# icameling/lidar_camera_calibration

Hardware: AMD Instinct MI355X
Metric: chessboard-corner frames/sec + max corner error (mm), VLP-16 cloud (higher is better)
Workload: dtype f32

## Files before the change

### include/ilcc_hip.h

```cpp
#ifndef ILCC_HIP_H_
#define ILCC_HIP_H_

#include <stdint.h>

#ifdef __cplusplus
extern "C" {
#endif

#define ILCC_MAX_CORNERS 256
#define ILCC_ABI_VERSION 5

enum {
  ILCC_OK = 0,
  ILCC_NO_ROI_POINTS = 1,
  ILCC_NO_CLUSTER = 2,
  ILCC_NO_PLANE = 3,
  ILCC_DEGENERATE_HIST = 4,
  ILCC_TOO_FEW_POINTS = 5,
  ILCC_BAD_ARGUMENT = 6,
  ILCC_CAPACITY = 7,
  ILCC_HIP_ERROR = 8,
  ILCC_IO_ERROR = 9,
  ILCC_BOARD_NOT_FOUND = 10,
  ILCC_AMBIGUOUS = 11
// ... 89 lines not shown
  uint64_t grid_cost_box_evals_sum;
  double grid_cost_kernel_ms_sum;
  double grid_cost_full_ms_sum;
  double walk_order_ms_sum;
  double grid_cost_prepass_ms_sum;
  double grid_cost_locate_ms_sum;
  uint64_t batches;
  double stage_ms_sum[7];
  double roi_count_ms_sum;
  uint64_t online_second_tier_frames;
} ilcc_timing;

int32_t ilcc_abi_version(void);
const char* ilcc_strerror(int32_t status);
const char* ilcc_last_error(const ilcc_handle* h);

void ilcc_default_params(ilcc_params* p);

int32_t ilcc_set_chessboard_param(ilcc_params* p, const char* cam_yaml);

ilcc_handle* ilcc_create(int32_t device, const ilcc_params* p, uint32_t max_frames,
                         uint64_t max_total_points);
void ilcc_destroy(ilcc_handle* h);
int32_t ilcc_set_params(ilcc_handle* h, const ilcc_params* p);
int32_t ilcc_reserve(ilcc_handle* h, uint32_t labelled_points_per_frame, uint32_t roi_points_per_frame);

int32_t ilcc_extract(ilcc_handle* h, const float* xyzi, uint32_t n, const float click[3],
                     ilcc_result* out);

int32_t ilcc_extract_batch(ilcc_handle* h, const float* xyzi, const uint64_t* offsets,
                           uint32_t n_frames, const float* clicks, ilcc_result* out);

int32_t ilcc_extract_batch_device(ilcc_handle* h, const float* d_xyzi, const uint64_t* offsets,
                                  uint32_t n_frames, const float* d_clicks, ilcc_result* out);

int32_t ilcc_submit_batch_device(ilcc_handle* h, const float* d_xyzi, const uint64_t* offsets,
                                 uint32_t n_frames, const float* d_clicks, int32_t* ticket);
int32_t ilcc_submit_batch(ilcc_handle* h, const float* xyzi, const uint64_t* offsets, uint32_t n_frames,
                          const float* clicks, int32_t* ticket);
int32_t ilcc_wait(ilcc_handle* h, int32_t ticket, ilcc_result* out);
#define ILCC_RECORD_HEADER 20
int32_t ilcc_wait_records_device(ilcc_handle* h, int32_t ticket, ilcc_result* out, void* d_records, uint32_t n_corners,
                                 uint32_t tag_base);

enum { ILCC_RESULTS_FULL = 0, ILCC_RESULTS_COMPACT = 1 };
int32_t ilcc_set_result_mode(ilcc_handle* h, int32_t mode);
int32_t ilcc_wait_compact(ilcc_handle* h, int32_t ticket, float* records, uint64_t capacity_floats);
uint32_t ilcc_record_floats(const ilcc_handle* h, int32_t ticket);
int32_t ilcc_fetch_results(ilcc_handle* h, uint32_t first, uint32_t n, ilcc_result* out);

int32_t ilcc_chessboard_by_point_batch(ilcc_handle* h, const float* xyzi, const uint64_t* offsets,
                                       uint32_t n_frames, const float* points, int32_t min_plane_points,
                                       ilcc_result* out);
int32_t ilcc_submit_chessboard_by_point(ilcc_handle* h, const float* xyzi, const uint64_t* offsets, uint32_t n_frames,
                                        const float* points, int32_t* ticket);
int32_t ilcc_wait_chessboard_by_point(ilcc_handle* h, int32_t ticket, int32_t min_plane_points, ilcc_result* out);
int64_t ilcc_fetch_classes(ilcc_handle* h, uint32_t frame, uint8_t* out_class, uint64_t cap_points);

int64_t ilcc_fetch_cloud(ilcc_handle* h, uint32_t frame, int32_t which, float* out_xyzi,
                         uint64_t cap_points);
int64_t ilcc_fetch_labelled(ilcc_handle* h, uint32_t frame, float* out_yz, uint8_t* out_label,
                            uint64_t cap_points);
int64_t ilcc_fetch_walk(ilcc_handle* h, uint32_t frame, float* out_yz, uint8_t* out_label, uint64_t cap_points,
                        uint32_t counts[2]);

int32_t ilcc_grid_cost(ilcc_handle* h, const float* yz, const uint8_t* label, uint32_t m,
                       int32_t use_oob, float* cost_out, int32_t* best_index, float* best_cost);

int32_t ilcc_grid_solve(ilcc_handle* h, const float* yz, const uint8_t* label, uint32_t m, int32_t* grid_index, float* grid_cost,
                        int32_t lat[3], int32_t* phase, int64_t* cost_q, int64_t* alt_cost_q, int32_t* rounds, int32_t* hops,
                        int32_t* flags, int32_t* ties);

int32_t ilcc_pattern_refine(ilcc_handle* h, const float* yz, const uint8_t* label, uint32_t m, int32_t lat[3],
                            int32_t* phase, int64_t* cost_q, int64_t* alt_cost_q, int32_t* rounds, int32_t* hops);

int32_t ilcc_get_theta_t(ilcc_handle* h, const float* yz, const uint8_t* label, uint32_t m,
                         int32_t topleft_white, int32_t use_oob, double theta_t[3], double* cost,
                         int32_t* iterations);

#define ILCC_TIMELINE_COLS 15
int32_t ilcc_debug_timeline_enable(ilcc_handle* h, int32_t on);
int32_t ilcc_debug_timeline_fetch(ilcc_handle* h, double* rows, uint32_t cap_rows);

void ilcc_get_timing(const ilcc_handle* h, ilcc_timing* t);
void ilcc_reset_timing(ilcc_handle* h);

int32_t ilcc_save_corners2txt(const float* corners_xyz, uint32_t n_corners, const char* filename);
int32_t ilcc_read_lidar_corners(const char* filename, uint32_t num, double* out_xyz);

#ifdef __cplusplus
}
#endif
#endif
```

### lidar_camera_calibration_amd/_native.py

```python
from __future__ import annotations

import ctypes as C
import os

import numpy as np

_HERE = os.path.dirname(os.path.abspath(__file__))
LIB_PATH = os.environ.get("ILCC_HIP_LIB") or os.path.join(_HERE, "libilcc_hip.so")
MAX_CORNERS = 256

OK, NO_ROI_POINTS, NO_CLUSTER, NO_PLANE, DEGENERATE_HIST, TOO_FEW_POINTS, BAD_ARGUMENT, CAPACITY, \
    HIP_ERROR, IO_ERROR, BOARD_NOT_FOUND, AMBIGUOUS = range(12)
FLAG_TIE_OVERFLOW, FLAG_REFINE_CAPPED, FLAG_LOW_COVERAGE, FLAG_BORDER_RISK = 1, 2, 4, 8
FLAGS_FP32_ONLY = FLAG_TIE_OVERFLOW | FLAG_BORDER_RISK
RECORD_HEADER = 20
TIMELINE_COLS = 15
COST_Q_ONE = float(1 << 40)
SOLVER_REFERENCE_LOCAL, SOLVER_GRID = 0, 1
CLOUD_ROI, CLOUD_CLUSTER, CLOUD_CHESSBOARD, CLOUD_PCA, CLOUD_OPTIM = range(5)

EXPORTS = [
    "ilcc_abi_version", "ilcc_strerror", "ilcc_last_error", "ilcc_default_params",
    "ilcc_set_chessboard_param", "ilcc_create", "ilcc_destroy", "ilcc_set_params", "ilcc_reserve", "ilcc_extract",
    "ilcc_extract_batch", "ilcc_extract_batch_device", "ilcc_submit_batch_device", "ilcc_submit_batch", "ilcc_wait", "ilcc_wait_records_device", "ilcc_fetch_cloud", "ilcc_fetch_labelled", "ilcc_fetch_walk", "ilcc_chessboard_by_point_batch", "ilcc_submit_chessboard_by_point", "ilcc_wait_chessboard_by_point", "ilcc_fetch_classes",
    "ilcc_grid_cost", "ilcc_grid_solve", "ilcc_pattern_refine", "ilcc_get_theta_t", "ilcc_get_timing", "ilcc_reset_timing",
    "ilcc_save_corners2txt", "ilcc_read_lidar_corners",
    "ilcc_set_result_mode", "ilcc_wait_compact", "ilcc_record_floats", "ilcc_fetch_results",
    "ilcc_debug_timeline_enable", "ilcc_debug_timeline_fetch",
]
ABI_VERSION = 5
RESULTS_FULL, RESULTS_COMPACT = 0, 1


class Params(C.Structure):
    _fields_ = [
        ("roi_half", C.c_double * 3),
        ("cluster_tol", C.c_double),
        ("cluster_min", C.c_int32),
        ("cluster_max", C.c_int32),
        ("ransac_thresh", C.c_double),
        ("ransac_hyp", C.c_int32),
        ("ransac_seed", C.c_uint32),
        ("hist_bins", C.c_int32),
        ("gray_rate", C.c_double),
        ("huber_delta", C.c_double),
        ("grid_length", C.c_double),
        ("board_w", C.c_int32),
        ("board_h", C.c_int32),
        ("solver", C.c_int32),
        ("phase_mode", C.c_int32),
        ("max_iterations", C.c_int32),
        ("grid_prune", C.c_int32),
        ("n_th", C.c_int32), ("n_ty", C.c_int32), ("n_tz", C.c_int32),
        ("th_min", C.c_double), ("th_step", C.c_double),
        ("ty_min", C.c_double), ("ty_step", C.c_double),
        ("tz_min", C.c_double), ("tz_step", C.c_double),
        ("refine_div", C.c_int32), ("refine_max_rounds", C.c_int32),
        ("refine_th_margin", C.c_int32), ("reserved0", C.c_int32),
        ("ambiguity_eps", C.c_double),
        ("online_cluster_tol", C.c_double),
        ("min_cell_coverage", C.c_double),
        ("ransac_probability", C.c_double),
    ]


class Result(C.Structure):
    _fields_ = [
        ("status", C.c_int32),
        ("n_points", C.c_int32),
        ("n_roi", C.c_int32), ("n_cluster", C.c_int32), ("n_plane", C.c_int32),
        ("n_black", C.c_int32), ("n_gray", C.c_int32), ("n_white", C.c_int32),
        ("n_corners", C.c_int32),
        ("phase", C.c_int32),
        ("iters_a", C.c_int32), ("iters_b", C.c_int32),
        ("grid_index", C.c_int32),
        ("found_board", C.c_int32),
        ("grid_cost", C.c_float),
        ("plane", C.c_float * 4),
        ("pca", C.c_float * 16),
        ("gray_zone", C.c_double * 2),
        ("theta_t", C.c_double * 3),
        ("cost_a", C.c_double), ("cost_b", C.c_double),
        ("sel_cost", C.c_double),
        ("basin_margin", C.c_double),
        ("flags", C.c_int32),
        ("grid_ties", C.c_int32),
        ("cells_hit", C.c_int32),
        ("n_oob", C.c_int32),
        ("corners", C.c_float * (MAX_CORNERS * 3)),
    ]

    def corners_array(self) -> np.ndarray:
        return np.ctypeslib.as_array(self.corners)[:3 * self.n_corners].reshape(-1, 3).copy()


class Timing(C.Structure):
    _fields_ = [
        ("roi_crop", C.c_float), ("cluster", C.c_float), ("ransac_plane", C.c_float),
        ("plane_frame_hist", C.c_float), ("grid_cost", C.c_float), ("refine_corners", C.c_float),
        ("total", C.c_float),
        ("grid_cost_launches", C.c_uint32),
        ("grid_cost_ms_sum", C.c_double),
        ("grid_cost_evals_sum", C.c_uint64),
        ("grid_cost_evals_nominal_sum", C.c_uint64),
        ("grid_cost_evals_interior_sum", C.c_uint64),
        ("grid_cost_box_evals_sum", C.c_uint64),
        ("grid_cost_kernel_ms_sum", C.c_double),
        ("grid_cost_full_ms_sum", C.c_double),
        ("walk_order_ms_sum", C.c_double),
        ("grid_cost_prepass_ms_sum", C.c_double),
        ("grid_cost_locate_ms_sum", C.c_double),
# ... 13 lines not shown
        if not os.path.exists(LIB_PATH):
            raise OSError(f"{LIB_PATH} not found: build it with `python -c 'import __graft_entry__ as g; "
                          "g.build()'` (hipcc --offload-arch=gfx950); there is no CPU fallback")
        L = C.CDLL(LIB_PATH)
        vp, fp = C.c_void_p, C.POINTER(C.c_float)
        pp, rp = C.POINTER(Params), C.POINTER(Result)
        L.ilcc_abi_version.restype = C.c_int32
        got = L.ilcc_abi_version()
        if got != ABI_VERSION:
            raise OSError(f"{LIB_PATH} implements ABI {got}, this package declares ABI {ABI_VERSION}: rebuild it "
                          "(python -c 'import __graft_entry__ as g; g.build()')")
        L.ilcc_strerror.argtypes = [C.c_int32]
        L.ilcc_strerror.restype = C.c_char_p
        L.ilcc_last_error.argtypes = [vp]
        L.ilcc_last_error.restype = C.c_char_p
        L.ilcc_default_params.argtypes = [pp]
        L.ilcc_set_chessboard_param.argtypes = [pp, C.c_char_p]
        L.ilcc_set_chessboard_param.restype = C.c_int32
        L.ilcc_create.argtypes = [C.c_int32, pp, C.c_uint32, C.c_uint64]
        L.ilcc_create.restype = vp
        L.ilcc_destroy.argtypes = [vp]
        L.ilcc_set_params.argtypes = [vp, pp]
        L.ilcc_set_params.restype = C.c_int32
        L.ilcc_reserve.argtypes = [vp, C.c_uint32, C.c_uint32]
        L.ilcc_reserve.restype = C.c_int32
        L.ilcc_extract.argtypes = [vp, fp, C.c_uint32, fp, rp]
        L.ilcc_extract.restype = C.c_int32
        L.ilcc_extract_batch.argtypes = [vp, fp, C.POINTER(C.c_uint64), C.c_uint32, fp, rp]
        L.ilcc_extract_batch.restype = C.c_int32
        L.ilcc_extract_batch_device.argtypes = [vp, vp, C.POINTER(C.c_uint64), C.c_uint32, vp, rp]
        L.ilcc_extract_batch_device.restype = C.c_int32
        L.ilcc_submit_batch_device.argtypes = [vp, vp, C.POINTER(C.c_uint64), C.c_uint32, vp, C.POINTER(C.c_int32)]
        L.ilcc_submit_batch_device.restype = C.c_int32
        L.ilcc_submit_batch.argtypes = [vp, vp, C.POINTER(C.c_uint64), C.c_uint32, vp, C.POINTER(C.c_int32)]
        L.ilcc_submit_batch.restype = C.c_int32
        L.ilcc_wait.argtypes = [vp, C.c_int32, rp]
        L.ilcc_wait.restype = C.c_int32
        L.ilcc_wait_records_device.argtypes = [vp, C.c_int32, rp, vp, C.c_uint32, C.c_uint32]
        L.ilcc_wait_records_device.restype = C.c_int32
        L.ilcc_chessboard_by_point_batch.argtypes = [vp, fp, C.POINTER(C.c_uint64), C.c_uint32, fp, C.c_int32, rp]
        L.ilcc_chessboard_by_point_batch.restype = C.c_int32
        L.ilcc_submit_chessboard_by_point.argtypes = [vp, C.c_void_p, C.POINTER(C.c_uint64), C.c_uint32, C.c_void_p, C.POINTER(C.c_int32)]
        L.ilcc_submit_chessboard_by_point.restype = C.c_int32
        L.ilcc_wait_chessboard_by_point.argtypes = [vp, C.c_int32, C.c_int32, rp]
        L.ilcc_wait_chessboard_by_point.restype = C.c_int32
        L.ilcc_fetch_classes.argtypes = [vp, C.c_uint32, C.POINTER(C.c_uint8), C.c_uint64]
        L.ilcc_fetch_classes.restype = C.c_int64
        L.ilcc_fetch_cloud.argtypes = [vp, C.c_uint32, C.c_int32, fp, C.c_uint64]
        L.ilcc_fetch_cloud.restype = C.c_int64
        L.ilcc_fetch_labelled.argtypes = [vp, C.c_uint32, fp, C.POINTER(C.c_uint8), C.c_uint64]
        L.ilcc_fetch_labelled.restype = C.c_int64
        L.ilcc_fetch_walk.argtypes = [vp, C.c_uint32, fp, C.POINTER(C.c_uint8), C.c_uint64, C.POINTER(C.c_uint32)]
        L.ilcc_fetch_walk.restype = C.c_int64
        L.ilcc_grid_cost.argtypes = [vp, fp, C.POINTER(C.c_uint8), C.c_uint32, C.c_int32, fp,
                                     C.POINTER(C.c_int32), fp]
        L.ilcc_grid_cost.restype = C.c_int32
        L.ilcc_grid_solve.argtypes = [vp, fp, C.POINTER(C.c_uint8), C.c_uint32, C.POINTER(C.c_int32), fp, C.POINTER(C.c_int32),
                                      C.POINTER(C.c_int32), C.POINTER(C.c_int64), C.POINTER(C.c_int64), C.POINTER(C.c_int32),
                                      C.POINTER(C.c_int32), C.POINTER(C.c_int32), C.POINTER(C.c_int32)]
        L.ilcc_grid_solve.restype = C.c_int32
        L.ilcc_pattern_refine.argtypes = [vp, fp, C.POINTER(C.c_uint8), C.c_uint32, C.POINTER(C.c_int32),
                                          C.POINTER(C.c_int32), C.POINTER(C.c_int64), C.POINTER(C.c_int64),
                                          C.POINTER(C.c_int32), C.POINTER(C.c_int32)]
        L.ilcc_pattern_refine.restype = C.c_int32
        L.ilcc_get_theta_t.argtypes = [vp, fp, C.POINTER(C.c_uint8), C.c_uint32, C.c_int32, C.c_int32,
                                       C.POINTER(C.c_double), C.POINTER(C.c_double), C.POINTER(C.c_int32)]
        L.ilcc_get_theta_t.restype = C.c_int32
        L.ilcc_get_timing.argtypes = [vp, C.POINTER(Timing)]
        L.ilcc_reset_timing.argtypes = [vp]
        L.ilcc_save_corners2txt.argtypes = [fp, C.c_uint32, C.c_char_p]
        L.ilcc_save_corners2txt.restype = C.c_int32
        L.ilcc_read_lidar_corners.argtypes = [C.c_char_p, C.c_uint32, C.POINTER(C.c_double)]
        L.ilcc_read_lidar_corners.restype = C.c_int32
        L.ilcc_set_result_mode.argtypes = [vp, C.c_int32]
        L.ilcc_set_result_mode.restype = C.c_int32
        L.ilcc_wait_compact.argtypes = [vp, C.c_int32, fp, C.c_uint64]
        L.ilcc_wait_compact.restype = C.c_int32
        L.ilcc_record_floats.argtypes = [vp, C.c_int32]
        L.ilcc_record_floats.restype = C.c_uint32
        L.ilcc_debug_timeline_enable.argtypes = [vp, C.c_int32]
        L.ilcc_debug_timeline_enable.restype = C.c_int32
        L.ilcc_debug_timeline_fetch.argtypes = [vp, C.POINTER(C.c_double), C.c_uint32]
        L.ilcc_debug_timeline_fetch.restype = C.c_int32
        L.ilcc_fetch_results.argtypes = [vp, C.c_uint32, C.c_uint32, rp]
        L.ilcc_fetch_results.restype = C.c_int32
        _lib = L
    return _lib


def default_params() -> Params:
    p = Params()
    lib().ilcc_default_params(C.byref(p))
    return p


def strerror(status: int) -> str:
    return lib().ilcc_strerror(int(status)).decode()


def fptr(a: np.ndarray):
    return a.ctypes.data_as(C.POINTER(C.c_float))
```

### lidar_camera_calibration_amd/csrc/ilcc_api.cpp

```cpp
#include <hip/hip_runtime.h>

#include <cmath>
#include <cstdio>
#include <cstdlib>
#include <cstring>
#include <fstream>
#include <mutex>
#include <new>
#include <sstream>
#include <string>
#include <vector>

#include "ilcc_internal.h"

using namespace ilcc;

#ifndef ILCC_SLOTS
#define ILCC_SLOTS 4
#endif
constexpr int kSlots = ILCC_SLOTS;
constexpr int kStreams = 3;

enum BatchEvent {
  kEvStart,
// ... 13 lines not shown
  kEvCount
};
static_assert(kEvCount == ILCC_TIMELINE_COLS - 1, "a timeline row is the slot and one time per event");

struct Slot {
  hipEvent_t ev[kEvCount]{};
  hipEvent_t done = nullptr;
  hipEvent_t late = nullptr;
  hipEvent_t k6_done = nullptr;
  bool allocated = false;
  float4* d_xyzi = nullptr;
  float* d_clicks = nullptr;
  uint64_t* d_off = nullptr;
  ilcc_result* d_res = nullptr;
  float4 *d_roi = nullptr, *d_cluster = nullptr, *d_board = nullptr, *d_pca = nullptr, *d_optim = nullptr;
  float2 *d_yz = nullptr, *d_walk_yz = nullptr;
  uint8_t* d_walk_lab = nullptr;
  uint32_t *d_walk_mi = nullptr, *d_walk_nrim = nullptr;
  uint8_t *d_lab = nullptr, *d_cls = nullptr;
  uint32_t *d_nlab = nullptr, *d_walk = nullptr, *d_counts = nullptr, *d_parent = nullptr, *d_count = nullptr;
  unsigned long long* d_masks = nullptr;
  uint32_t *d_hash_head = nullptr, *d_hash_next = nullptr;
  uint32_t *d_flags = nullptr, *d_nfinite = nullptr, *d_counts_fin = nullptr;
  uint32_t* h_online = nullptr;
  uint32_t* d_list = nullptr;
  void* d_list_frames = nullptr;
  GridPartial *d_partial = nullptr, *d_partial2 = nullptr, *d_partial3 = nullptr, *d_partial4 = nullptr;
  SolveRec* d_solverec = nullptr;
  uint32_t *d_bound = nullptr, *d_bound_sub = nullptr;
  uint32_t* d_tie_count = nullptr;
  GridPartial* d_tie_list = nullptr;
  unsigned long long* d_iters = nullptr;
  uint32_t *d_grp_alive = nullptr, *d_grp_mask = nullptr;
  size_t grp_alive_cap = 0, grp_mask_cap = 0;
  float* h_rec_dev = nullptr;
  unsigned long long* h_iters_dev = nullptr;
  float* h_rec = nullptr;
  ilcc_result* h_res = nullptr;
  unsigned long long* h_iters = nullptr;
  uint64_t* h_off = nullptr;
  std::vector<uint64_t> off;
  uint32_t n_frames = 0;
  bool busy = false, grid = false;
  bool online = false;
  bool h_res_valid = false;
  bool compact = false;
  uint32_t rec_corners = 0;
};

struct ilcc_handle {
  int device = 0;
  ilcc_params p{};
  uint32_t max_frames = 0;
  uint64_t max_points = 0;
  uint32_t max_theta = 0;
  uint32_t crop_chunks_cap = 0;
  Slot slots[kSlots];
  hipStream_t stream[kStreams]{};
  uint64_t seq = 0;
  uint64_t stream_last[kStreams]{};
  hipEvent_t entry_done = nullptr;
  int next_slot = 0;
  int last_slot = -1;
  int k6_last = -1;
  float *d_cth = nullptr, *d_sth = nullptr, *d_ay = nullptr, *d_az = nullptr;
  float *d_cth2 = nullptr, *d_sth2 = nullptr, *d_ay2 = nullptr, *d_az2 = nullptr;
  GridTables grid{}, seed_grid{};
  SeedMap seed_map{2, 12, 6};
  double2* d_th_lattice = nullptr;
  size_t th_lattice_cap = 0;
  int32_t th_lat_lo = 0, th_lat_hi = 0, hop_y = 0, hop_z = 0;
  double* d_solve = nullptr;
  RefineOut* d_refine_io = nullptr;
  uint32_t grid_lds_points = 1024;
  uint64_t group_prepass_skipped = 0;
  uint32_t cluster_lds_points = 2048;
  uint32_t cluster_cells_cap = kClusterCellsMin;
  uint32_t list_grid = 1024;
  bool poisoned = false;
  int32_t result_mode = ILCC_RESULTS_FULL;
  ilcc_timing timing{};
  hipEvent_t tl_ref = nullptr;
  bool tl_on = false;
  std::vector<double> tl_rows;
  std::string err;
};

namespace {

thread_local std::string g_err;

#define HIP_TRY(h, expr)                                                                   \
  do {                                                                                     \
    hipError_t e_ = (expr);                                                                \
    if (e_ != hipSuccess) {                                                                \
      (h)->err = std::string(#expr) + ": " + hipGetErrorString(e_);                        \
      return ILCC_HIP_ERROR;                                                               \
    }                                                                                      \
  } while (0)

int32_t near_zero_index(double vmin, double step, int32_t n) {
  long c = std::lround(-vmin / step);
  if (c < 0) c = 0;
  if (c > n - 1) c = n - 1;
  return (int32_t)c;
}

bool params_ok(const ilcc_params& p, std::string& why) {
  auto bad = [&](const char* m) {
    why = m;
    return false;
  };
  if (!(p.grid_length > 0)) return bad("grid_length must be > 0");
  if (p.board_w < 2 || p.board_h < 2 || p.board_w > p.board_h) return bad("board_w/board_h: need 2 <= w <= h");
  if ((p.board_w - 1) * (p.board_h - 1) > ILCC_MAX_CORNERS) return bad("too many corners");
  if (p.hist_bins < 1 || p.hist_bins > 4096) return bad("hist_bins out of range");
  if (!(p.gray_rate > 0) || !(p.huber_delta > 0)) return bad("gray_rate / huber_delta must be > 0");
  if (p.ransac_hyp < 1 || p.ransac_hyp > 65536) return bad("ransac_hyp out of range");
  if (!(p.ransac_probability == p.ransac_probability) || p.ransac_probability >= 1.0) return bad("ransac_probability must be < 1");
  if (!(p.cluster_tol > 0) || p.cluster_min < 1 || p.cluster_max < p.cluster_min) return bad("cluster params");
  if (p.solver != ILCC_SOLVER_REFERENCE_LOCAL && p.solver != ILCC_SOLVER_GRID) return bad("solver");
  if (p.phase_mode < 0 || p.phase_mode > 2) return bad("phase_mode");
  if (p.grid_prune != 0 && p.grid_prune != 1) return bad("grid_prune must be 0 or 1");
  if (p.max_iterations < 0 || p.max_iterations > 100000) return bad("max_iterations");
  if (p.n_th < 1 || p.n_ty < 1 || p.n_tz < 1) return bad("grid sizes must be >= 1");
  if (p.n_th > 4096 || p.n_ty > 4096 || p.n_tz > 4096) return bad("grid axes are limited to 4096 candidates");
  if (p.n_ty + p.n_tz > kGridTableMax) return bad("n_ty + n_tz exceeds the LDS table capacity of the grid kernel");
  if (p.refine_div < 0 || p.refine_div > 64 || (p.refine_div & (p.refine_div - 1)) != 0)
    return bad("refine_div must be 0 or a power of two <= 64");
  if (p.refine_max_rounds < 0 || p.refine_max_rounds > 4096) return bad("refine_max_rounds");
  if (p.refine_th_margin < 0 || p.refine_th_margin > 4096) return bad("refine_th_margin");
  if (!(p.online_cluster_tol > 0)) return bad("online_cluster_tol must be > 0");
  if (!(p.ambiguity_eps == p.ambiguity_eps)) return bad("ambiguity_eps is NaN");
  if (!(p.min_cell_coverage == p.min_cell_coverage) || p.min_cell_coverage > 1.0) return bad("min_cell_coverage must be <= 1");
  if (p.board_w * p.board_h > kCoverageCellsMax) return bad("board has more squares than the coverage mask holds");
  if ((uint64_t)p.n_th * p.n_ty * p.n_tz * 2ull >= 0xFFFFFFFFull) return bad("grid too large");
  if (!(p.th_step > 0) || !(p.ty_step > 0) || !(p.tz_step > 0)) return bad("grid steps must be > 0");
  {
    const double div = (double)(p.refine_div > 0 ? p.refine_div : 1);
    if (std::lround(p.grid_length / (p.ty_step / div)) < 1 || std::lround(p.grid_length / (p.tz_step / div)) < 1)
      return bad("ty_step / tz_step too coarse: one board square is less than half a refinement-lattice step");
  }
  return true;
}

int32_t sync_own(ilcc_handle* h, hipStream_t s) {
  HIP_TRY(h, hipEventRecord(h->entry_done, s));
  HIP_TRY(h, hipEventSynchronize(h->entry_done));
  return ILCC_OK;
}

int32_t sync_all(ilcc_handle* h) {
  for (hipStream_t s : h->stream)
    if (s) HIP_TRY(h, hipStreamSynchronize(s));
  return ILCC_OK;
}

int32_t upload_tables(ilcc_handle* h) {
  const ilcc_params& p = h->p;
  if ((uint32_t)p.n_th > h->max_theta || (uint32_t)p.n_ty > h->max_theta || (uint32_t)p.n_tz > h->max_theta) {
    h->err = "grid axis longer than the handle's table capacity";
    return ILCC_CAPACITY;
  }
  hipStream_t st = h->stream[0];
  std::vector<float> cth(p.n_th), sth(p.n_th), ay(p.n_ty), az(p.n_tz);
  const double g = p.grid_length;
// ... 339 lines not shown
#endif
#ifndef ILCC_BOX_POINTS
#define ILCC_BOX_POINTS 48
#endif
constexpr int kAnchorRadius = 1;
#ifndef ILCC_ANCHOR_ROUNDS
#define ILCC_ANCHOR_ROUNDS 2
#endif
constexpr int kAnchorRounds = ILCC_ANCHOR_ROUNDS;


GridPass whole_grid_pass(const Ctx& c, const GridTables& t, GridPartial* out) {
  GridPass g{};
  g.t = t;
  g.out = out;
  g.blocks = (uint32_t)t.n_th;
  g.bound = c.grid_bound;
  return g;
}

GridSeed full_table_records(const GridPartial* records, uint32_t blocks) { return GridSeed{records, blocks, SeedMap{1, 1, 0}}; }

GridPass seed_pass(const ilcc_handle* h, const Slot& sl, const Ctx& c) {
  GridPass g = whole_grid_pass(c, h->seed_grid, sl.d_partial2);
  g.walk_limit = (uint32_t)ILCC_SEED_POINTS;
  g.bound = c.grid_bound_sub;
  return g;
}

GridPass refine_pass(const ilcc_handle* h, const Slot& sl, const Ctx& c, int32_t refine_radius) {
  GridPass g = whole_grid_pass(c, h->grid, sl.d_partial3);
  g.seed = GridSeed{sl.d_partial2, (uint32_t)h->seed_grid.n_th, h->seed_map};
  g.window_tiles = h->seed_map.stride_t > 2 * kTileA ? 4 : 2;
  g.radius_th = (refine_radius / kRefineThetaStride) * kRefineThetaStride;
  g.step_th = kRefineThetaStride;
  g.blocks = std::min((uint32_t)(2 * (g.radius_th / kRefineThetaStride) + 1), h->max_theta);
  g.walk_limit = (uint32_t)ILCC_SEED_POINTS;
  g.bound = c.grid_bound_sub;
  return g;
}

GridPass anchor_pass(const ilcc_handle* h, const Ctx& c, const GridSeed& seed, GridPartial* out) {
  GridPass g = whole_grid_pass(c, h->grid, out);
  g.seed = seed;
  g.radius_th = kAnchorRadius;
  g.blocks = 2 * kAnchorRadius + 1;
  return g;
}

GridPass full_pass(const ilcc_handle* h, const Ctx& c, const GridSeed& seed) {
  GridPass g = whole_grid_pass(c, h->grid, c.partial);
  g.seed = seed;
  g.collect_ties = 1u;
  return g;
}

LocatePlan locate_plan(const ilcc_handle* h, const Slot& sl, const Ctx& c) {
  LocatePlan lp{};
  lp.seed = h->seed_grid;
  lp.map = h->seed_map;
  lp.refine_radius = std::max(1, h->seed_map.stride_th / ILCC_REFINE_RADIUS_DIV);
  lp.sample_min = (uint32_t)ILCC_SEED_POINTS;
  lp.sample_cap = std::max((uint32_t)ILCC_SEED_POINTS, ((c.grid_lds_points >> 3) + 63u) & ~63u);
  lp.out = sl.d_partial4;
  return lp;
}

int32_t enqueue_locate_launches(ilcc_handle* h, Slot& sl, const Ctx& c, hipStream_t s, int32_t refine_radius, GridSeed& located) {
  launch_grid_cost(c, seed_pass(h, sl, c), s, 1, nullptr, true);
  HIP_TRY(h, hipEventRecord(sl.ev[kEvSeeded], s));
  const GridPass refine = refine_pass(h, sl, c, refine_radius);
  launch_grid_cost(c, refine, s, 1, nullptr, true);
  HIP_TRY(h, hipEventRecord(sl.ev[kEvRefined], s));
  located = full_table_records(refine.out, refine.blocks);
  GridPartial* const ping[2] = {sl.d_partial4, sl.d_partial2};
  for (int round = 0; round < kAnchorRounds; ++round) {
    const GridPass anchor = anchor_pass(h, c, located, ping[round & 1]);
    launch_anchor(c, anchor, s);
    located = full_table_records(anchor.out, anchor.blocks);
  }
  return ILCC_OK;
}

int32_t enqueue_grid_search(ilcc_handle* h, Slot& sl, const Ctx& c, hipStream_t s, uint32_t n_frames, bool chain) {
  const bool prune = h->p.grid_prune != 0;
  launch_walk_order(c, s);
  HIP_TRY(h, hipEventRecord(sl.ev[kEvWalkOrdered], s));
  GridSeed located{};
  if (h->seed_grid.n_th > 0 && h->p.n_th >= 8 && h->p.n_ty >= 8 && h->p.n_tz >= 8) {
    const LocatePlan lp = locate_plan(h, sl, c);
    const bool fused = n_frames >= (uint32_t)kLocateMinFrames && lp.seed.n_th <= 16 &&
                       locate_lds_bytes(lp.sample_cap, h->grid.n_ty, h->grid.n_tz, lp.seed.n_ty, lp.seed.n_tz) <= 60u * 1024u;
    if (fused) {
      launch_locate(c, s, lp);
      HIP_TRY(h, hipEventRecord(sl.ev[kEvSeeded], s));
      HIP_TRY(h, hipEventRecord(sl.ev[kEvRefined], s));
      located = full_table_records(lp.out, 1);
    } else {
      const int32_t st = enqueue_locate_launches(h, sl, c, s, lp.refine_radius, located);
      if (st != ILCC_OK) return st;
    }
  } else {
    HIP_TRY(h, hipEventRecord(sl.ev[kEvSeeded], s));
    HIP_TRY(h, hipEventRecord(sl.ev[kEvRefined], s));
  }
  HIP_TRY(h, hipEventRecord(sl.ev[kEvAnchored], s));
  GridPass full = full_pass(h, c, located);
  const GroupPrepassPlan gp = group_prepass_plan(h->p);
  full.box_points = gp.box ? (uint32_t)ILCC_BOX_POINTS : 0u;
  if (full.box_points != 0u && gp.on && (size_t)n_frames * gp.groups <= sl.grp_alive_cap &&
      (size_t)n_frames * gp.groups * gp.words <= sl.grp_mask_cap) {
    full.grp_alive = sl.d_grp_alive;
    full.grp_mask = sl.d_grp_mask;
    full.grp_count = gp.groups;
    full.grp_words = gp.words;
    launch_group_prepass(c, full, s);
  } else if (full.box_points != 0u && gp.on) {
    if (h->group_prepass_skipped++ == 0) h->err = "note: k6_group_prepass skipped (mask buffers smaller than this batch needs): slower, results unaffected";
  }
  HIP_TRY(h, hipEventRecord(sl.ev[kEvPrepassed], s));
  const int si = (int)(&sl - h->slots);
  if (chain && h->k6_last >= 0 && h->k6_last != si && h->slots[h->k6_last].busy)
    HIP_TRY(h, hipStreamWaitEvent(s, h->slots[h->k6_last].k6_done, 0));
  HIP_TRY(h, hipEventRecord(sl.ev[kEvFullStart], s));
  launch_grid_cost(c, full, s, 1, nullptr, prune);
  if (chain) {
    HIP_TRY(h, hipEventRecord(sl.k6_done, s));
    h->k6_last = si;
  }
  return ILCC_OK;
}

int32_t enqueue_impl(ilcc_handle* h, int si, hipStream_t s, const float4* d_xyzi, const uint64_t* offsets, uint32_t n_frames,
                     const float* d_clicks, bool front_only, bool no_crop) {
  Slot& sl = h->slots[si];
  uint64_t max_n = 0;
  for (uint32_t f = 0; f < n_frames; ++f) max_n = std::max<uint64_t>(max_n, offsets[f + 1] - offsets[f]);
  uint32_t chunks = (uint32_t)((max_n + kCropChunk - 1) / kCropChunk);
  if (chunks == 0) chunks = 1;
  if ((uint64_t)chunks * n_frames > (uint64_t)h->crop_chunks_cap) {
    h->err = "crop chunk table too small for this (very ragged) batch";
    return ILCC_CAPACITY;
  }
  sl.off.assign(offsets, offsets + n_frames + 1);
  sl.n_frames = n_frames;
  std::memcpy(sl.h_off, sl.off.data(), sizeof(uint64_t) * (n_frames + 1));
  HIP_TRY(h, hipMemcpyAsync(sl.d_off, sl.h_off, sizeof(uint64_t) * (n_frames + 1), hipMemcpyHostToDevice, s));
  Ctx c = make_ctx(h, sl, d_xyzi, d_clicks, n_frames, chunks);
  HIP_TRY(h, hipEventRecord(sl.ev[kEvStart], s));
  if (!no_crop) {
    launch_roi_crop(c, s, sl.ev[kEvCropCounted]);
    HIP_TRY(h, hipEventRecord(sl.ev[kEvCropped], s));
    launch_cluster(c, s);
  } else {
    c.p.cluster_tol = c.p.online_cluster_tol;
    c.wide = 1u;
    Ctx t1 = c;
    t1.online_tier = 1u;
    t1.online_window = 1.25f;
    t1.p.roi_half[0] = t1.p.roi_half[1] = t1.p.roi_half[2] = (double)t1.online_window;
    t1.cluster_bits = cluster_bits_online();
    launch_roi_crop(t1, s, sl.ev[kEvCropCounted]);
    HIP_TRY(h, hipEventRecord(sl.ev[kEvCropped], s));
    launch_cluster(t1, s);
    Ctx t2 = c;
    t2.online_tier = 2u;
    t2.p.roi_half[0] = t2.p.roi_half[1] = t2.p.roi_half[2] = (double)INFINITY;
    launch_roi_crop(t2, s, nullptr);
    launch_cluster(t2, s);
    HIP_TRY(h, hipMemcpyAsync(sl.h_online, sl.d_flags, sizeof(uint32_t) * n_frames, hipMemcpyDeviceToHost, s));
    HIP_TRY(h, hipMemcpyAsync(sl.h_online + h->max_frames, sl.d_nfinite, sizeof(uint32_t) * n_frames, hipMemcpyDeviceToHost, s));
  }
  HIP_TRY(h, hipEventRecord(sl.ev[kEvClustered], s));
  launch_ransac_plane(c, s);
  HIP_TRY(h, hipEventRecord(sl.ev[kEvPlane], s));
  launch_plane_frame_hist(c, s);
  sl.grid = !front_only && h->p.solver == ILCC_SOLVER_GRID;
  HIP_TRY(h, hipEventRecord(sl.ev[kEvLabelled], s));
  if (sl.grid) {
    const int32_t st = enqueue_grid_search(h, sl, c, s, n_frames, true);
    if (st != ILCC_OK) return st;
  }
  HIP_TRY(h, hipEventRecord(sl.ev[kEvSearched], s));
  if (!front_only) {
    if (sl.grid) {
      launch_pattern_refine_corners(c, s);
    } else {
      launch_refine_corners(c, s);
    }
  }
  HIP_TRY(h, hipEventRecord(sl.ev[kEvEnd], s));
  HIP_TRY(h, hipGetLastError());
  sl.compact = h->result_mode == ILCC_RESULTS_COMPACT;
  sl.rec_corners = board_corners(h->p);
  if (sl.compact) {
    launch_pack_records(sl.d_res, n_frames, sl.rec_corners, 0u, sl.h_rec_dev, s);
  } else {
    HIP_TRY(h, copy_results_trimmed(sl.h_res, sl.d_res, n_frames, sl.rec_corners, s));
  }
  launch_store_to_host(sl.d_iters, sl.h_iters_dev, sizeof(unsigned long long) * kBatchWords, s);
  HIP_TRY(h, hipGetLastError());
  HIP_TRY(h, hipEventRecord(sl.done, s));
  sl.busy = true;
  sl.online = no_crop;
  return ILCC_OK;
}

int32_t run_late(ilcc_handle* h, Slot& sl, hipStream_t s) {
  HIP_TRY(h, hipEventRecord(sl.late, s));
  HIP_TRY(h, hipEventSynchronize(sl.late));
  return ILCC_OK;
}

int32_t ensure_full(ilcc_handle* h, Slot& sl) {
  if (sl.h_res_valid) return ILCC_OK;
  const hipStream_t s = late_stream(h);
  HIP_TRY(h, copy_results_trimmed(sl.h_res, sl.d_res, sl.n_frames, sl.rec_corners, s));
  const int32_t st = run_late(h, sl, s);
  if (st != ILCC_OK) return st;
  sl.h_res_valid = true;
  return ILCC_OK;
}

int32_t finish(ilcc_handle* h, int si, ilcc_result* out, float* out_compact = nullptr, float* d_records = nullptr,
               uint32_t n_corners = 0, uint32_t tag_base = 0) {
  Slot& sl = h->slots[si];
  HIP_TRY(h, hipEventSynchronize(sl.done));
  const uint32_t n_frames = sl.n_frames;
  const size_t rec_w = (size_t)ILCC_RECORD_HEADER + 3 * (size_t)sl.rec_corners;
  const bool pack_now = out_compact && !sl.compact;
  const hipStream_t ls = late_stream(h);
  if (d_records) launch_pack_records(sl.d_res, n_frames, n_corners, tag_base, d_records, ls);
  if (pack_now) launch_pack_records(sl.d_res, n_frames, sl.rec_corners, 0u, sl.h_rec_dev, ls);
  if (d_records || pack_now) {
    const int32_t st = run_late(h, sl, ls);
    if (st != ILCC_OK) return st;
  }
  sl.busy = false;
  sl.h_res_valid = !sl.compact;
  h->last_slot = si;
  if (out) {
    const int32_t st = ensure_full(h, sl);
    if (st != ILCC_OK) return st;
    const size_t row = trimmed_bytes(sl.rec_corners);
    for (uint32_t f = 0; f < n_frames; ++f) std::memcpy(&out[f], &sl.h_res[f], row);
  }
  if (out_compact) std::memcpy(out_compact, sl.h_rec, sizeof(float) * n_frames * rec_w);
  auto span = [&](BatchEvent from, BatchEvent to, float& ms_out) { return hipEventElapsedTime(&ms_out, sl.ev[from], sl.ev[to]); };
  float ms[6];
  HIP_TRY(h, span(kEvStart, kEvCropped, ms[0]));
  HIP_TRY(h, span(kEvCropped, kEvClustered, ms[1]));
  HIP_TRY(h, span(kEvClustered, kEvPlane, ms[2]));
  HIP_TRY(h, span(kEvPlane, kEvLabelled, ms[3]));
  HIP_TRY(h, span(kEvLabelled, kEvSearched, ms[4]));
  HIP_TRY(h, span(kEvSearched, kEvEnd, ms[5]));
  float k6k[6] = {0.f, 0.f, 0.f, 0.f, 0.f, 0.f};
  if (sl.grid) {
    float pre = 0.f;
    HIP_TRY(h, span(kEvLabelled, kEvPrepassed, pre));
    HIP_TRY(h, span(kEvLabelled, kEvWalkOrdered, k6k[0]));
    HIP_TRY(h, span(kEvWalkOrdered, kEvSeeded, k6k[1]));
    HIP_TRY(h, span(kEvSeeded, kEvRefined, k6k[2]));
    HIP_TRY(h, span(kEvRefined, kEvAnchored, k6k[3]));
// ... 767 lines not shown
  if (cost_q) *cost_q = (int64_t)std::llround(rec.sel * 1099511627776.0);
  if (alt_cost_q) *alt_cost_q = (int64_t)std::llround(rec.cost_b * 1099511627776.0);
  if (rounds) *rounds = rec.iters_a;
  if (hops) *hops = rec.iters_b;
  if (flags) *flags = rec.flags;
  if (ties) *ties = rec.ties;
  return ILCC_OK;
}

int32_t ilcc_get_theta_t(ilcc_handle* h, const float* yz, const uint8_t* label, uint32_t m, int32_t topleft_white,
                         int32_t use_oob, double theta_t[3], double* cost, int32_t* iterations) {
  if (!h || !theta_t) return ILCC_BAD_ARGUMENT;
  const hipStream_t s = h->stream[take_stream(h)];
  int32_t st = stage_labelled(h, s, yz, label, m);
  if (st != ILCC_OK) return st;
  Slot& sl = h->slots[0];
  HIP_TRY(h, hipMemcpyAsync(h->d_solve, theta_t, sizeof(double) * 3, hipMemcpyHostToDevice, s));
  const Ctx c = make_ctx(h, sl, nullptr, nullptr, 1, 1);
  launch_local_solve(c, s, topleft_white, use_oob, h->d_solve, h->d_solve + 3);
  HIP_TRY(h, hipGetLastError());
  double back[5];
  HIP_TRY(h, hipMemcpyAsync(back, h->d_solve, sizeof(back), hipMemcpyDeviceToHost, s));
  {
    const int32_t sst = sync_own(h, s);
    if (sst != ILCC_OK) return sst;
  }
  theta_t[0] = back[0];
  theta_t[1] = back[1];
  theta_t[2] = back[2];
  if (cost) *cost = back[3];
  if (iterations) *iterations = (int32_t)back[4];
  return ILCC_OK;
}

int32_t ilcc_pattern_refine(ilcc_handle* h, const float* yz, const uint8_t* label, uint32_t m, int32_t lat[3],
                            int32_t* phase, int64_t* cost_q, int64_t* alt_cost_q, int32_t* rounds, int32_t* hops) {
  if (!h || !lat || !phase) return ILCC_BAD_ARGUMENT;
  if (lat[0] < h->th_lat_lo || lat[0] > h->th_lat_hi || (*phase != 0 && *phase != 1)) {
    h->err = "ilcc_pattern_refine: theta lattice coordinate outside [th_min - refine_th_margin, th_max + refine_th_margin] steps";
    return ILCC_BAD_ARGUMENT;
  }
  const hipStream_t s = h->stream[take_stream(h)];
  int32_t st = stage_labelled(h, s, yz, label, m);
  if (st != ILCC_OK) return st;
  Slot& sl = h->slots[0];
  RefineOut io{};
  io.lat[0] = lat[0];
  io.lat[1] = lat[1];
  io.lat[2] = lat[2];
  io.phase = *phase;
  HIP_TRY(h, hipMemcpyAsync(h->d_refine_io, &io, sizeof(io), hipMemcpyHostToDevice, s));
  const Ctx c = make_ctx(h, sl, nullptr, nullptr, 1, 1);
  launch_pattern_refine_test(c, s, h->d_refine_io);
  HIP_TRY(h, hipGetLastError());
  HIP_TRY(h, hipMemcpyAsync(&io, h->d_refine_io, sizeof(io), hipMemcpyDeviceToHost, s));
  {
    const int32_t sst = sync_own(h, s);
    if (sst != ILCC_OK) return sst;
  }
  lat[0] = io.lat[0];
  lat[1] = io.lat[1];
  lat[2] = io.lat[2];
  *phase = io.phase;
  if (cost_q) *cost_q = io.cost_q;
  if (alt_cost_q) *alt_cost_q = io.alt_q;
  if (rounds) *rounds = io.rounds;
  if (hops) *hops = io.hops;
  return ILCC_OK;
}

int32_t ilcc_debug_timeline_enable(ilcc_handle* h, int32_t on) {
  if (!h) return ILCC_BAD_ARGUMENT;
  HIP_TRY(h, hipSetDevice(h->device));
  h->tl_rows.clear();
  h->tl_on = on != 0;
  if (h->tl_on) {
    if (!h->tl_ref) HIP_TRY(h, hipEventCreate(&h->tl_ref));
    HIP_TRY(h, hipEventRecord(h->tl_ref, h->stream[0]));
    HIP_TRY(h, hipEventSynchronize(h->tl_ref));
  }
  return ILCC_OK;
}

int32_t ilcc_debug_timeline_fetch(ilcc_handle* h, double* rows, uint32_t cap_rows) {
  if (!h || (!rows && cap_rows)) return -ILCC_BAD_ARGUMENT;
  const size_t have = h->tl_rows.size() / ILCC_TIMELINE_COLS;
  const size_t n = std::min<size_t>(have, cap_rows);
  if (n) std::memcpy(rows, h->tl_rows.data(), sizeof(double) * n * ILCC_TIMELINE_COLS);
  h->tl_rows.clear();
  return (int32_t)n;
}

void ilcc_get_timing(const ilcc_handle* h, ilcc_timing* t) {
  if (h && t) *t = h->timing;
}
void ilcc_reset_timing(ilcc_handle* h) {
  if (h) h->timing = ilcc_timing{};
}

int32_t ilcc_save_corners2txt(const float* corners_xyz, uint32_t n_corners, const char* filename) {
  if (!corners_xyz || !filename) return ILCC_BAD_ARGUMENT;
  std::ofstream outfile(filename, std::ios_base::trunc);
  if (!outfile.is_open()) return ILCC_IO_ERROR;
  for (uint32_t i = 0; i < n_corners; ++i)
    outfile << corners_xyz[3 * i] << " " << corners_xyz[3 * i + 1] << " " << corners_xyz[3 * i + 2] << std::endl;
  outfile.close();
  return outfile.fail() ? ILCC_IO_ERROR : ILCC_OK;
}

int32_t ilcc_read_lidar_corners(const char* filename, uint32_t num, double* out_xyz) {
  if (!filename || !out_xyz) return -ILCC_BAD_ARGUMENT;
  std::ifstream infile(filename);
  if (!infile.is_open()) return -ILCC_IO_ERROR;
  uint32_t counter = 0;
  while (!infile.eof() && counter < num) {
    float x = 0, y = 0, z = 0;
    infile >> x >> y >> z;
    if (infile.fail()) break;
    out_xyz[3 * counter] = x;
    out_xyz[3 * counter + 1] = y;
    out_xyz[3 * counter + 2] = z;
    ++counter;
  }
  return (int32_t)counter;
}

}
```

### lidar_camera_calibration_amd/csrc/ilcc_internal.h

```cpp
#pragma once

#include <hip/hip_runtime.h>
#include <stdint.h>

#include "ilcc_hip.h"

#define ILCC_WAVE 64

namespace ilcc {

constexpr int kCropThreads = 256;
constexpr int kCropChunk = 4096;
#ifndef ILCC_K2_THREADS
#define ILCC_K2_THREADS 256
#endif
constexpr int kFrameThreads = ILCC_K2_THREADS;
#ifndef ILCC_K3_THREADS
#define ILCC_K3_THREADS 256
#endif
#ifndef ILCC_K45_THREADS
#define ILCC_K45_THREADS 256
#endif
constexpr int kPlaneThreads = ILCC_K3_THREADS;
constexpr int kPlaneThreadsSmallBatch = 1024;
#ifndef ILCC_SMALL_BATCH
#define ILCC_SMALL_BATCH 64
#endif
constexpr int kSmallBatchFrames = ILCC_SMALL_BATCH;
constexpr int kHistThreads = ILCC_K45_THREADS;
#ifndef ILCC_K6_THREADS
#define ILCC_K6_THREADS 256
#endif
constexpr int kGridThreads = ILCC_K6_THREADS;
#ifndef ILCC_K6_THREADS_LARGE
#define ILCC_K6_THREADS_LARGE 512
#endif
constexpr int kGridThreadsLarge = ILCC_K6_THREADS_LARGE;
#ifndef ILCC_K6_LARGE_FROM
#define ILCC_K6_LARGE_FROM 2048
#endif
constexpr int kGridLargeFrom = ILCC_K6_LARGE_FROM;
constexpr int kTileA = 4;
#ifndef ILCC_TILE_B
#define ILCC_TILE_B 4
#endif
constexpr int kTileB = ILCC_TILE_B;
#ifndef ILCC_K6_GROUP
#define ILCC_K6_GROUP 7
#endif
constexpr int kThetaGroup = ILCC_K6_GROUP;
constexpr int kGridLdsPointsMax = 8192;
constexpr int kGridTableMax = 8192;
#ifndef ILCC_K7_THREADS
#define ILCC_K7_THREADS 256
#endif
constexpr int kSolveThreads = ILCC_K7_THREADS;
#ifndef ILCC_K7R_THREADS
#define ILCC_K7R_THREADS 192
#endif
constexpr int kRefineThreads = ILCC_K7R_THREADS;
constexpr int kRefineThreadsSmallBatch = 768;
constexpr int kRefineList = 32;
constexpr int kTieCap = 256;
constexpr float kTieEps = 2e-5f;
constexpr int kCoverageCellsMax = 1024;
constexpr int kIterSlots = 64;
constexpr int kBatchWords = 3 * kIterSlots + 2;
constexpr int kClusterHashSize = 1 << 17;
constexpr int kClusterLdsPointsMax = 4096;
constexpr int kClusterLdsPointsMin = 1024;
constexpr int kClusterCellsMin = 512;
constexpr int kClusterCellsMax = 6144;

struct GridPartial {
  float cost;
  uint32_t d2;
  uint32_t flat;
  uint32_t pad;
};

struct SolveRec {
  double x[3];
  double cost_a, cost_b, sel;
  double margin;
  int32_t iters_a, iters_b, phase, valid;
  int32_t flags, ties;
};

struct RefineOut {
  long long cost_q, alt_q;
  int32_t lat[3];
  int32_t phase, rounds, hops;
};

struct GridTables {
  const float* cth;
  const float* sth;
  const float* ay;
  const float* az;
  int32_t n_th, n_ty, n_tz;
  int32_t c_th, c_ty, c_tz;
};

struct SeedMap {
  int32_t stride_t, stride_th, off_th;
};

struct GridSeed {
  const GridPartial* records;
  uint32_t blocks;
  SeedMap map;
};
// ... 80 lines not shown
    }
    if (a == 1u) break;
  }
  return S >= M ? 1u : S;
}

__device__ __forceinline__ int lane_id() { return threadIdx.x & (ILCC_WAVE - 1); }
__device__ __forceinline__ int wave_id() { return threadIdx.x >> 6; }

template <typename T>
__device__ __forceinline__ T wave_sum(T v) {
#pragma unroll
  for (int o = ILCC_WAVE / 2; o > 0; o >>= 1) v += __shfl_down(v, o, ILCC_WAVE);
  return v;
}

template <typename T>
__device__ __forceinline__ T block_sum(T v, T* scratch) {
  v = wave_sum(v);
  const int nw = (blockDim.x + ILCC_WAVE - 1) / ILCC_WAVE;
  __syncthreads();
  if (lane_id() == 0) scratch[wave_id()] = v;
  __syncthreads();
  if (threadIdx.x == 0) {
    T s = scratch[0];
    for (int w = 1; w < nw; ++w) s += scratch[w];
    scratch[16] = s;
  }
  __syncthreads();
  return scratch[16];
}

template <int NV>
__device__ __forceinline__ void block_sum_n(double (&v)[NV], double* scratch ) {
#pragma unroll
  for (int k = 0; k < NV; ++k) v[k] = wave_sum(v[k]);
  const int kW = (blockDim.x + ILCC_WAVE - 1) / ILCC_WAVE;
  __syncthreads();
  if (lane_id() == 0) {
#pragma unroll
    for (int k = 0; k < NV; ++k) scratch[wave_id() * NV + k] = v[k];
  }
  __syncthreads();
#pragma unroll
  for (int k = 0; k < NV; ++k) {
    double t = scratch[k];
    for (int w = 1; w < kW; ++w) t += scratch[w * NV + k];
    v[k] = t;
  }
}

__device__ __forceinline__ uint32_t block_rank(bool flag, uint32_t* scratch, uint32_t& total) {
  const unsigned long long m = __ballot(flag);
  const int lane = lane_id();
  const uint32_t in_wave = __popcll(m & ((1ull << lane) - 1ull));
  const int nw = (blockDim.x + ILCC_WAVE - 1) / ILCC_WAVE;
  __syncthreads();
  if (lane == 0) scratch[wave_id()] = __popcll(m);
  __syncthreads();
  uint32_t base = 0, tot = 0;
  for (int w = 0; w < nw; ++w) {
    const uint32_t c = scratch[w];
    if (w < wave_id()) base += c;
    tot += c;
  }
  total = tot;
  return base + in_wave;
}

struct LocatePlan {
  GridTables seed;
  SeedMap map;
  int32_t refine_radius;
  uint32_t sample_min, sample_cap;
  GridPartial* out;
};

size_t locate_lds_bytes(uint32_t sample_cap, int n_ty, int n_tz, int n_ty2, int n_tz2);
void launch_locate(const Ctx& c, hipStream_t s, const LocatePlan& lp);
void launch_anchor(const Ctx& c, const GridPass& pass, hipStream_t s);
constexpr int kRefineThetaStride = 2;
constexpr int kLocateMinFrames = 512;

void launch_roi_crop(const Ctx& c, hipStream_t s, hipEvent_t after_count = nullptr);
void launch_cluster(const Ctx& c, hipStream_t s);
void launch_ransac_plane(const Ctx& c, hipStream_t s);
void launch_plane_frame_hist(const Ctx& c, hipStream_t s);
void launch_walk_order(const Ctx& c, hipStream_t s);
void launch_grid_cost(const Ctx& c, const GridPass& pass, hipStream_t s, int32_t use_oob, float* cost_volume , bool prune);
void launch_group_prepass(const Ctx& c, const GridPass& full, hipStream_t s);
uint32_t grid_cost_evals_per_count();
void launch_refine_corners(const Ctx& c, hipStream_t s);
void launch_pack_records(const ilcc_result* d_res, uint32_t n_frames, uint32_t n_corners, uint32_t tag_base, float* d_out,
                         hipStream_t s);
void launch_store_to_host(const void* d_src, void* h_dst, size_t bytes, hipStream_t s);
void launch_pattern_refine_corners(const Ctx& c, hipStream_t s);
void launch_pattern_refine_test(const Ctx& c, hipStream_t s, RefineOut* d_io);
hipError_t set_kernel_attributes_k2();
size_t cluster_lds_bytes(uint32_t pts_cap, uint32_t cells_cap, uint32_t bits);
uint32_t cluster_bits_default();
uint32_t cluster_bits_online();
hipError_t set_kernel_attributes_k6();
hipError_t set_kernel_attributes_k7();
void launch_local_solve(const Ctx& c, hipStream_t s, int32_t tlw, int32_t use_oob, double* theta_t,
                        double* cost_iters );

}
```

### lidar_camera_calibration_amd/csrc/k1_roi_crop.hip

```cpp
#include "ilcc_internal.h"

namespace ilcc {

typedef float f32x4 __attribute__((ext_vector_type(4)));

struct Box {
  float lo[3], hi[3];
};

__device__ __forceinline__ Box make_box(const Ctx& c, uint32_t f) {
  Box b;
#pragma unroll
  for (int a = 0; a < 3; ++a) {
    const double cl = (double)c.clicks[3 * f + a];
    b.lo[a] = (float)(cl - c.p.roi_half[a]);
    b.hi[a] = (float)(cl + c.p.roi_half[a]);
  }
  return b;
}

template <bool FINITE_BOX>
__device__ __forceinline__ bool keep_point(const float4 q, const Box& b) {
  if (FINITE_BOX)
    return q.z >= b.lo[2] && q.z <= b.hi[2] && q.x >= b.lo[0] && q.x <= b.hi[0] && q.y >= b.lo[1] && q.y <= b.hi[1];
  const bool fin = isfinite(q.x) && isfinite(q.y) && isfinite(q.z);
  const bool in = !(q.z < b.lo[2] || q.z > b.hi[2]) && !(q.x < b.lo[0] || q.x > b.hi[0]) &&
                  !(q.y < b.lo[1] || q.y > b.hi[1]);
  return fin && in;
}

__global__ __launch_bounds__(kCropThreads) void k1_roi_count(Ctx c) {
  const uint32_t f = blockIdx.y, s = blockIdx.x;
  if (c.online_tier == 2u && c.frame_flags[f] == 0u) return;
  const uint64_t beg = c.off[f], end = c.off[f + 1];
  const uint64_t n = end - beg;
  if (s == 0) {
    uint32_t* w = reinterpret_cast<uint32_t*>(&c.res[f]);
    for (uint32_t k = threadIdx.x; k < sizeof(ilcc_result) / 4; k += kCropThreads) w[k] = 0u;
    if (f == 0 && threadIdx.x < kBatchWords && c.online_tier != 2u) c.grid_iters[threadIdx.x] = 0ull;
    __syncthreads();
  }
  if (s == 0 && threadIdx.x == 0) {
    if (c.tie_count) c.tie_count[f] = 0u;
    ilcc_result* r = &c.res[f];
    r->status = ILCC_OK;
    r->n_points = (int32_t)n;
    r->n_roi = r->n_cluster = r->n_plane = 0;
    r->n_black = r->n_gray = r->n_white = 0;
    r->n_corners = 0;
    r->phase = 0;
    r->iters_a = r->iters_b = 0;
    r->grid_index = -1;
    r->cells_hit = r->n_oob = 0;
    r->grid_cost = 0.f;
    r->cost_a = r->cost_b = r->sel_cost = 0.0;
    r->theta_t[0] = r->theta_t[1] = r->theta_t[2] = 0.0;
    c.n_lab[f] = 0;
    c.grid_bound[f] = 0x7f800000u;
    c.grid_bound_sub[f] = 0x7f800000u;
    if (c.online_tier == 1u) c.frame_flags[f] = 0u;
  }
  const uint64_t cbeg = (uint64_t)s * kCropChunk;
  uint32_t cnt = 0, fin = 0;
  unsigned long long* masks = c.crop_masks + ((uint64_t)f * c.crop_chunks + s) * (kCropChunk / ILCC_WAVE);
  if (cbeg < n) {
    const Box b = make_box(c, f);
    const uint64_t cend = (cbeg + kCropChunk < n) ? cbeg + kCropChunk : n;
    const float4* __restrict__ src = c.xyzi + beg;
    constexpr int kTrips = kCropChunk / kCropThreads;
    float4 q[kTrips];
#pragma unroll
    for (int k = 0; k < kTrips; ++k) {
      const uint64_t i = cbeg + (uint64_t)k * kCropThreads + threadIdx.x;
      if (i < cend) {
        const f32x4 v = __builtin_nontemporal_load(reinterpret_cast<const f32x4*>(src + i));
        q[k] = make_float4(v.x, v.y, v.z, v.w);
      } else {
        q[k] = make_float4(0.f, 0.f, 0.f, 0.f);
      }
    }
    const bool finite_box = isfinite(b.lo[0]) && isfinite(b.hi[0]) && isfinite(b.lo[1]) && isfinite(b.hi[1]) && isfinite(b.lo[2]) && isfinite(b.hi[2]);
    const uint32_t left = (uint32_t)(cend - cbeg);
    if (finite_box && c.online_tier != 1u) {
#pragma unroll
      for (int k = 0; k < kTrips; ++k) {
        const bool keep = ((uint32_t)k * kCropThreads + threadIdx.x < left) && keep_point<true>(q[k], b);
        const unsigned long long m = __ballot(keep);
        if (lane_id() == 0) masks[k * (kCropThreads / ILCC_WAVE) + wave_id()] = m;
        cnt += keep ? 1u : 0u;
      }
    } else {
#pragma unroll
      for (int k = 0; k < kTrips; ++k) {
        const bool mine = (uint32_t)k * kCropThreads + threadIdx.x < left;
        const bool keep = mine && keep_point<false>(q[k], b);
        const unsigned long long m = __ballot(keep);
        if (lane_id() == 0) masks[k * (kCropThreads / ILCC_WAVE) + wave_id()] = m;
        cnt += keep ? 1u : 0u;
        fin += (mine && isfinite(q[k].x) && isfinite(q[k].y) && isfinite(q[k].z)) ? 1u : 0u;
      }
    }
  }
  __shared__ uint32_t sc[17];
  const uint32_t total = block_sum<uint32_t>(cnt, sc);
  if (threadIdx.x == 0) c.crop_counts[(uint64_t)f * c.crop_chunks + s] = total;
  if (c.online_tier == 1u) {
    const uint32_t total_fin = block_sum<uint32_t>(fin, sc);
    if (threadIdx.x == 0) c.crop_fin[(uint64_t)f * c.crop_chunks + s] = total_fin;
  }
}

__global__ __launch_bounds__(kCropThreads) void k1_roi_scatter(Ctx c) {
  const uint32_t f = blockIdx.y, s = blockIdx.x;
  if (c.online_tier == 2u && c.frame_flags[f] == 0u) return;
  const uint64_t beg = c.off[f], end = c.off[f + 1];
  const uint64_t n = end - beg;
  const uint32_t* counts = c.crop_counts + (uint64_t)f * c.crop_chunks;
  uint32_t base = 0, all = 0;
  for (uint32_t k = 0; k < c.crop_chunks; ++k) {
    const uint32_t v = counts[k];
    if (k < s) base += v;
    all += v;
  }
  if (s == 0 && threadIdx.x == 0 && c.online_tier == 1u) {
    uint32_t nf = 0;
    for (uint32_t k = 0; k < c.crop_chunks; ++k) nf += c.crop_fin[(uint64_t)f * c.crop_chunks + k];
    c.n_finite[f] = nf;
  }
  if (s == 0 && threadIdx.x == 0) {
    c.res[f].n_roi = (int32_t)all;
    if (all == 0) {
      if (c.online_tier == 1u)
        c.frame_flags[f] = 1u;
      else
        c.res[f].status = ILCC_NO_ROI_POINTS;
    }
  }
  const uint64_t cbeg = (uint64_t)s * kCropChunk;
  if (cbeg >= n || counts[s] == 0) return;
  const float4* __restrict__ src = c.xyzi + beg;
  float4* __restrict__ dst = c.roi + beg;
  const unsigned long long* masks = c.crop_masks + ((uint64_t)f * c.crop_chunks + s) * (kCropChunk / ILCC_WAVE);
  constexpr int kWaves = kCropThreads / ILCC_WAVE, kMasks = kCropChunk / ILCC_WAVE;
  static_assert(kMasks == ILCC_WAVE, "one keep-mask per lane of the first wavefront");
  const int lane = lane_id(), w = wave_id();
  __shared__ unsigned long long s_mask[kMasks];
  __shared__ uint32_t s_before[kMasks];
  if (w == 0) {
    const unsigned long long mk = masks[lane];
    uint32_t incl = (uint32_t)__popcll(mk);
    const uint32_t own = incl;
#pragma unroll
    for (int o = 1; o < ILCC_WAVE; o <<= 1) {
      const uint32_t t = __shfl_up(incl, o, ILCC_WAVE);
      if (lane >= o) incl += t;
    }
    s_mask[lane] = mk;
    s_before[lane] = base + incl - own;
  }
  __syncthreads();
#pragma unroll
  for (int k = 0; k < kCropChunk / kCropThreads; ++k) {
    const int mine = k * kWaves + w;
    const unsigned long long mk = s_mask[mine];
    if ((mk >> lane) & 1ull) {
      const uint64_t i = cbeg + (uint64_t)k * kCropThreads + threadIdx.x;
      dst[s_before[mine] + (uint32_t)__popcll(mk & ((1ull << lane) - 1ull))] = src[i];
    }
  }
}

void launch_roi_crop(const Ctx& c, hipStream_t s, hipEvent_t after_count) {
  const dim3 grid(c.crop_chunks, c.n_frames);
  hipLaunchKernelGGL(k1_roi_count, grid, dim3(kCropThreads), 0, s, c);
  if (after_count) (void)hipEventRecord(after_count, s);
  hipLaunchKernelGGL(k1_roi_scatter, grid, dim3(kCropThreads), 0, s, c);
}

}
```

### lidar_camera_calibration_amd/csrc/k3_ransac_plane.hip

```cpp
#include "eig3.h"
#include "ilcc_internal.h"

namespace ilcc {

__device__ __forceinline__ uint32_t hash_u32(uint32_t x) {
  x ^= x >> 16;
  x *= 0x7feb352dU;
  x ^= x >> 15;
  x *= 0x846ca68bU;
  x ^= x >> 16;
  return x;
}
__device__ __forceinline__ uint32_t sample_index(uint32_t seed, uint32_t h, uint32_t k, uint32_t m) {
  const uint32_t r = hash_u32(seed ^ hash_u32(h * 3u + k + 0x9E3779B9u));
  return (uint32_t)(((uint64_t)r * (uint64_t)m) >> 32);
}

__device__ __forceinline__ bool plane_from_3(const float4 p0, const float4 p1, const float4 p2,
                                             float pl[4]) {
  const float ax = p1.x - p0.x, ay = p1.y - p0.y, az = p1.z - p0.z;
  const float bx = p2.x - p0.x, by = p2.y - p0.y, bz = p2.z - p0.z;
  float nx = ay * bz - az * by;
  float ny = az * bx - ax * bz;
  float nz = ax * by - ay * bx;
  float n2 = nx * nx;
  n2 = n2 + ny * ny;
  n2 = n2 + nz * nz;
  if (!(n2 > 1e-12f)) return false;
  const float nrm = sqrtf(n2);
  nx = nx / nrm;
  ny = ny / nrm;
  nz = nz / nrm;
  float d = nx * p0.x;
  d = d + ny * p0.y;
  d = d + nz * p0.z;
  pl[0] = nx;
  pl[1] = ny;
  pl[2] = nz;
  pl[3] = -d;
  return true;
}

__device__ __forceinline__ float plane_dist(const float pl[4], const float4 q) {
  float s = pl[0] * q.x;
  s = s + pl[1] * q.y;
  s = s + pl[2] * q.z;
  s = s + pl[3];
  return fabsf(s);
}

constexpr int kRansacLdsPoints = 2048;

__global__ __launch_bounds__(kPlaneThreadsSmallBatch) void k3_ransac_plane(Ctx c) {
  const uint32_t kThreads = blockDim.x;
  __shared__ float4 s_P[kRansacLdsPoints];
  __shared__ uint32_t sc[64];
  __shared__ double scd[16 * 6 + 8];
  __shared__ float s_plane[4];
  const uint32_t f = blockIdx.x;
  ilcc_result* r = &c.res[f];
  if (r->status != ILCC_OK) return;
  const uint32_t M = (uint32_t)r->n_cluster;
  const uint64_t beg = c.off[f];
  const float4* __restrict__ G = c.cluster + beg;
  const uint32_t tid = threadIdx.x;
  const int lane = lane_id(), wid = wave_id();
  const float thr = (float)c.p.ransac_thresh;
  if (M < 3) {
    if (tid == 0) r->status = ILCC_NO_PLANE;
    return;
  }
  const float4* P = G;
  if (M <= (uint32_t)kRansacLdsPoints) {
    for (uint32_t i = tid; i < M; i += kThreads) s_P[i] = G[i];
    __syncthreads();
    P = s_P;
  }

  const uint32_t n_waves = kThreads / ILCC_WAVE;
  auto score = [&](uint32_t h, uint32_t beat, uint32_t& cnt) -> bool {
    const uint32_t i0 = sample_index(c.p.ransac_seed, h, 0, M);
    const uint32_t i1 = sample_index(c.p.ransac_seed, h, 1, M);
    const uint32_t i2 = sample_index(c.p.ransac_seed, h, 2, M);
    float pl[4];
    cnt = 0;
    if (i0 == i1 || i0 == i2 || i1 == i2) return false;
    if (!plane_from_3(P[i0], P[i1], P[i2], pl)) return false;
    for (uint32_t base = 0; base < M; base += ILCC_WAVE) {
      const uint32_t i = base + lane;
      const bool in = (i < M) && plane_dist(pl, P[i]) < thr;
      cnt += (uint32_t)__popcll(__ballot(in));
      if (cnt + (M - min(M, base + (uint32_t)ILCC_WAVE)) <= beat) break;
    }
    return true;
  };
  if (c.p.ransac_probability > 0.0) {
    __shared__ uint32_t s_state[5];
    __shared__ double s_k;
    if (tid == 0) {
      s_state[0] = 0u;
      s_state[1] = 0xFFFFFFFFu;
      s_state[2] = s_state[3] = s_state[4] = 0u;
      s_k = 1.0;
    }
    __syncthreads();
    const double log_probability = log(1.0 - c.p.ransac_probability);
    const double one_over_indices = 1.0 / (double)M;
    const uint32_t max_it = (uint32_t)c.p.ransac_hyp, max_skip = max_it * 10u;
    for (uint32_t h0 = 0;; h0 += n_waves) {
      uint32_t cnt;
      const bool valid = score(h0 + (uint32_t)wid, s_state[0], cnt);
      if (lane == 0) sc[wid] = valid ? cnt : 0xFFFFFFFFu;
      __syncthreads();
      if (tid == 0) {
        uint32_t best = s_state[0], best_h = s_state[1], it = s_state[2], skip = s_state[3], stop = 0u;
        double k = s_k;
        for (uint32_t j = 0; j < n_waves; ++j) {
          if (!((double)it < k && skip < max_skip)) {
            stop = 1u;
            break;
          }
          const uint32_t v = sc[j];
          if (v == 0xFFFFFFFFu) {
            ++skip;
            continue;
          }
          if (v > best) {
            best = v;
            best_h = h0 + j;
            const double w = (double)best * one_over_indices;
            double p_no_outliers = 1.0 - w * w * w;
            p_no_outliers = fmax(2.220446049250313e-16, p_no_outliers);
            p_no_outliers = fmin(1.0 - 2.220446049250313e-16, p_no_outliers);
            k = log_probability / log(p_no_outliers);
          }
          ++it;
          if (it > max_it) {
            stop = 1u;
            break;
          }
        }
        if (!((double)it < k && skip < max_skip)) stop = 1u;
        s_state[0] = best;
        s_state[1] = best_h;
        s_state[2] = it;
        s_state[3] = skip;
        s_state[4] = stop;
        s_k = k;
      }
      __syncthreads();
      if (s_state[4] != 0u) break;
    }
    if (tid == 0) {
      sc[32] = s_state[0];
      sc[33] = s_state[1];
    }
  } else {
    uint32_t best_cnt = 0, best_h = 0xFFFFFFFFu;
    for (uint32_t h = (uint32_t)wid; h < (uint32_t)c.p.ransac_hyp; h += n_waves) {
      uint32_t cnt;
      if (!score(h, best_cnt, cnt)) continue;
      if (cnt > best_cnt) {
        best_cnt = cnt;
        best_h = h;
      }
    }
    if (lane == 0) {
      sc[wid] = best_cnt;
      sc[16 + wid] = best_h;
    }
    __syncthreads();
    if (tid == 0) {
      uint32_t bc = 0, bh = 0xFFFFFFFFu;
      for (int w = 0; w < (int)n_waves; ++w)
        if (sc[w] > bc || (sc[w] == bc && sc[w] > 0 && sc[16 + w] < bh)) {
          bc = sc[w];
          bh = sc[16 + w];
        }
      sc[32] = bc;
      sc[33] = bh;
    }
  }
  if (tid == 0 && sc[32] > 0u) {
    const uint32_t bh = sc[33];
    float pl[4];
    plane_from_3(P[sample_index(c.p.ransac_seed, bh, 0, M)], P[sample_index(c.p.ransac_seed, bh, 1, M)],
                 P[sample_index(c.p.ransac_seed, bh, 2, M)], pl);
    for (int k = 0; k < 4; ++k) s_plane[k] = pl[k];
  }
  __syncthreads();
  const uint32_t bc = sc[32];
  if (bc == 0) {
    if (tid == 0) r->status = ILCC_NO_PLANE;
    return;
  }
  float pl[4] = {s_plane[0], s_plane[1], s_plane[2], s_plane[3]};

  if (bc > 3) {
    double sx = 0, sy = 0, sz = 0;
    for (uint32_t i = tid; i < M; i += kThreads) {
      const float4 q = P[i];
      if (plane_dist(pl, q) < thr) {
        sx += q.x;
        sy += q.y;
        sz += q.z;
      }
    }
    double sums3[3] = {sx, sy, sz};
    block_sum_n<3>(sums3, scd);
    const double cx = sums3[0] / bc, cy = sums3[1] / bc, cz = sums3[2] / bc;
    double cv[6] = {0, 0, 0, 0, 0, 0};
    for (uint32_t i = tid; i < M; i += kThreads) {
      const float4 q = P[i];
      if (plane_dist(pl, q) < thr) {
        const double dx = q.x - cx, dy = q.y - cy, dz = q.z - cz;
        cv[0] += dx * dx;
        cv[1] += dx * dy;
        cv[2] += dx * dz;
        cv[3] += dy * dy;
        cv[4] += dy * dz;
        cv[5] += dz * dz;
      }
    }
    __syncthreads();
    block_sum_n<6>(cv, scd);
    double cs[6];
    for (int k = 0; k < 6; ++k) cs[k] = cv[k] / bc;
    if (tid == 0) {
      const double cov[9] = {cs[0], cs[1], cs[2], cs[1], cs[3], cs[4], cs[2], cs[4], cs[5]};
      double w[3], v[3][3];
      eig3_sym(cov, w, v);
      double n[3] = {v[0][0], v[0][1], v[0][2]};
      if (n[0] * pl[0] + n[1] * pl[1] + n[2] * pl[2] < 0) {
        n[0] = -n[0];
        n[1] = -n[1];
        n[2] = -n[2];
      }
      s_plane[0] = (float)n[0];
      s_plane[1] = (float)n[1];
      s_plane[2] = (float)n[2];
      s_plane[3] = (float)(-(n[0] * cx + n[1] * cy + n[2] * cz));
    }
    __syncthreads();
    for (int k = 0; k < 4; ++k) pl[k] = s_plane[k];
  }

  float4* __restrict__ dst = c.board + beg;
  uint32_t running = 0;
  for (uint32_t base = 0; base < M; base += kThreads) {
    const uint32_t i = base + tid;
    float4 q = make_float4(0.f, 0.f, 0.f, 0.f);
    bool keep = false;
    if (i < M) {
      q = P[i];
      keep = plane_dist(pl, q) < thr;
    }
    uint32_t tot;
    const uint32_t rank = block_rank(keep, sc + 40, tot);
    if (keep) dst[running + rank] = q;
    running += tot;
  }
  if (tid == 0) {
    r->n_plane = (int32_t)running;
    for (int k = 0; k < 4; ++k) r->plane[k] = pl[k];
    if (running < 3) r->status = ILCC_NO_PLANE;
  }
}

void launch_ransac_plane(const Ctx& c, hipStream_t s) {
  const int threads = (c.n_frames <= (uint32_t)kSmallBatchFrames || c.wide) ? kPlaneThreadsSmallBatch : kPlaneThreads;
  hipLaunchKernelGGL(k3_ransac_plane, dim3(c.n_frames), dim3(threads), 0, s, c);
}

}
```

### lidar_camera_calibration_amd/csrc/k45_plane_frame_hist.hip

```cpp
#include "eig3.h"
#include "ilcc_internal.h"

namespace ilcc {

__global__ __launch_bounds__(kHistThreads) void k45_plane_frame_hist(Ctx c) {
  __shared__ uint32_t sc[64];
  __shared__ double scd[16 * 6 + 8];
  __shared__ float s_pca[16];
  __shared__ float s_mm[34];
  __shared__ double s_gz[2];
  __shared__ int s_status;
  extern __shared__ int s_hist[];

  const uint32_t f = blockIdx.x;
  ilcc_result* r = &c.res[f];
  if (r->status != ILCC_OK) return;
  const uint32_t M = (uint32_t)r->n_plane;
  const uint64_t beg = c.off[f];
  const float4* __restrict__ P = c.board + beg;
  const uint32_t tid = threadIdx.x;
  const int lane = lane_id(), wid = wave_id();
  if (M < 3) {
    if (tid == 0) r->status = ILCC_TOO_FEW_POINTS;
    return;
  }

  double sx = 0, sy = 0, sz = 0, si = 0;
  float vmin = 3.402823466e38f, vmax = -3.402823466e38f;
  for (uint32_t i = tid; i < M; i += kHistThreads) {
    const float4 q = P[i];
    sx += q.x;
    sy += q.y;
    sz += q.z;
    si += (double)q.w;
    vmin = fminf(vmin, q.w);
    vmax = fmaxf(vmax, q.w);
  }
  double s4[4] = {sx, sy, sz, si};
  block_sum_n<4>(s4, scd);
  const double cx = (double)(float)(s4[0] / M);
  const double cy = (double)(float)(s4[1] / M);
  const double cz = (double)(float)(s4[2] / M);
  const double isum = s4[3];
  double cv[6] = {0, 0, 0, 0, 0, 0};
  for (uint32_t i = tid; i < M; i += kHistThreads) {
    const float4 q = P[i];
    const double dx = q.x - cx, dy = q.y - cy, dz = q.z - cz;
    cv[0] += dx * dx;
    cv[1] += dx * dy;
    cv[2] += dx * dz;
    cv[3] += dy * dy;
    cv[4] += dy * dz;
    cv[5] += dz * dz;
  }
  __syncthreads();
  block_sum_n<6>(cv, scd);
  double cs[6];
  for (int k = 0; k < 6; ++k) cs[k] = cv[k] / M;
#pragma unroll
  for (int o = 32; o > 0; o >>= 1) {
    vmin = fminf(vmin, __shfl_down(vmin, o, ILCC_WAVE));
    vmax = fmaxf(vmax, __shfl_down(vmax, o, ILCC_WAVE));
  }
  if (lane == 0) {
    s_mm[wid] = vmin;
    s_mm[16 + wid] = vmax;
  }
  __syncthreads();
  if (tid == 0) {
    const double cov[9] = {cs[0], cs[1], cs[2], cs[1], cs[3], cs[4], cs[2], cs[4], cs[5]};
    double w[3], v[3][3];
    eig3_sym(cov, w, v);
    double e0[3] = {v[0][0], v[0][1], v[0][2]};
    double e1[3] = {v[1][0], v[1][1], v[1][2]};
    if (e0[0] * cx + e0[1] * cy + e0[2] * cz > 0) {
      e0[0] = -e0[0];
      e0[1] = -e0[1];
      e0[2] = -e0[2];
    }
    int big = 0;
    for (int a = 1; a < 3; ++a)
      if (fabs(e1[a]) > fabs(e1[big])) big = a;
    if (e1[big] < 0) {
      e1[0] = -e1[0];
      e1[1] = -e1[1];
      e1[2] = -e1[2];
    }
    float f0[3], f1[3], f2[3];
    for (int a = 0; a < 3; ++a) {
      f0[a] = (float)e0[a];
      f1[a] = (float)e1[a];
    }
    f2[0] = f0[1] * f1[2] - f0[2] * f1[1];
    f2[1] = f0[2] * f1[0] - f0[0] * f1[2];
    f2[2] = f0[0] * f1[1] - f0[1] * f1[0];
    const float cf[3] = {(float)cx, (float)cy, (float)cz};
    const float* rows[3] = {f0, f1, f2};
    for (int rr = 0; rr < 3; ++rr) {
      for (int a = 0; a < 3; ++a) s_pca[4 * rr + a] = rows[rr][a];
      float t = rows[rr][0] * cf[0];
      t = t + rows[rr][1] * cf[1];
      t = t + rows[rr][2] * cf[2];
      s_pca[4 * rr + 3] = -1.0f * t;
    }
    s_pca[12] = s_pca[13] = s_pca[14] = 0.f;
    s_pca[15] = 1.f;
    for (int k = 0; k < 16; ++k) r->pca[k] = s_pca[k];
    float mn = s_mm[0], mx = s_mm[16];
    for (int w2 = 1; w2 < kHistThreads / ILCC_WAVE; ++w2) {
      mn = fminf(mn, s_mm[w2]);
      mx = fmaxf(mx, s_mm[16 + w2]);
    }
    s_mm[32] = mn;
    s_mm[33] = mx;
  }
  const int HL = c.p.hist_bins;
  for (int b = (int)tid; b <= HL; b += kHistThreads) s_hist[b] = 0;
  __syncthreads();

  float4* __restrict__ Q = c.pca + beg;
  const double mn = (double)s_mm[32], mx = (double)s_mm[33];
  const bool flat = !(mx > mn);
  const double factor = flat ? 0.0 : HL / (mx - mn);
  for (uint32_t i = tid; i < M; i += kHistThreads) {
    const float4 q = P[i];
    float o[3];
#pragma unroll
    for (int rr = 0; rr < 3; ++rr) {
      float s = s_pca[4 * rr] * q.x;
      s = s + s_pca[4 * rr + 1] * q.y;
      s = s + s_pca[4 * rr + 2] * q.z;
      s = s + s_pca[4 * rr + 3];
      o[rr] = s;
    }
    Q[i] = make_float4(o[0], o[1], o[2], q.w);
    if (!flat) {
      const double sample = (double)q.w - mn;
      int bin = (int)round(sample * factor);
      bin = bin < 0 ? 0 : (bin > HL ? HL : bin);
      atomicAdd(&s_hist[bin], 1);
    }
  }
  __syncthreads();

  __shared__ unsigned long long s_top[2];
  if (tid == 0) s_top[0] = s_top[1] = 0ull;
  __syncthreads();
  const bool hist_ok = !(flat || HL <= 0);
  const double mean = isum / M;
  const double bin_width = (mx - mn) / HL;
  if (hist_ok) {
    for (int bb = (int)tid; bb < HL; bb += kHistThreads) {
      const int cb = s_hist[bb];
      bool first = true;
      for (int b2 = 0; b2 < bb; ++b2) first = first && (s_hist[b2] != cb);
      if (!first) continue;
      const double edge = bin_width * (double)bb + mn;
      const int side = edge > mean ? 1 : (edge < mean ? 0 : -1);
      if (side >= 0) atomicMax(&s_top[side], ((unsigned long long)(uint32_t)(cb + 1) << 32) | (unsigned long long)(uint32_t)bb);
    }
  }
  __syncthreads();
  if (tid == 0) {
    int status = ILCC_OK;
    if (!hist_ok || s_top[0] == 0ull || s_top[1] == 0ull) {
      status = ILCC_DEGENERATE_HIST;
    } else {
      const double low = bin_width * (double)(uint32_t)(s_top[0] & 0xFFFFFFFFull) + mn;
      const double high = bin_width * (double)(uint32_t)(s_top[1] & 0xFFFFFFFFull) + mn;
      const double rate = c.p.gray_rate;
      s_gz[0] = ((rate - 1) * low + high) / rate;
      s_gz[1] = (low + (rate - 1) * high) / rate;
      r->gray_zone[0] = s_gz[0];
      r->gray_zone[1] = s_gz[1];
    }
    s_status = status;
    if (status != ILCC_OK) r->status = status;
  }
  __syncthreads();
  if (s_status != ILCC_OK) return;

  const double gz0 = s_gz[0], gz1 = s_gz[1];
  float2* __restrict__ YZ = c.yz + beg;
  uint8_t* __restrict__ LB = c.lab + beg;
  uint8_t* __restrict__ CL = c.cls + beg;
  uint32_t running = 0, nb = 0, nw = 0;
  for (uint32_t base = 0; base < M; base += kHistThreads) {
    const uint32_t i = base + tid;
    bool keep = false;
    uint8_t l = 0;
    float4 q = make_float4(0.f, 0.f, 0.f, 0.f);
    if (i < M) {
      q = Q[i];
      if ((double)q.w < gz0) {
        keep = true;
        l = 0;
      } else if ((double)q.w > gz1) {
        keep = true;
        l = 1;
      }
      CL[i] = keep ? (uint8_t)(2 * l) : (uint8_t)1;
    }
    uint32_t tot, totw;
    const uint32_t rank = block_rank(keep, sc, tot);
    (void)block_rank(keep && l == 1, sc + 20, totw);
    if (keep) {
      YZ[running + rank] = make_float2(q.y, q.z);
      LB[running + rank] = l;
    }
    running += tot;
    nw += totw;
    nb += tot - totw;
  }
  if (tid == 0) {
    r->n_black = (int32_t)nb;
    r->n_white = (int32_t)nw;
    r->n_gray = (int32_t)(M - running);
    c.n_lab[f] = running;
    c.walk_stride[f] = walk_stride(running);
  }
}

void launch_plane_frame_hist(const Ctx& c, hipStream_t s) {
  const size_t lds = sizeof(int) * (size_t)(c.p.hist_bins + 1);
  hipLaunchKernelGGL(k45_plane_frame_hist, dim3(c.n_frames), dim3(kHistThreads), lds, s, c);
}

}
```

### lidar_camera_calibration_amd/csrc/k6_grid_cost.hip

```cpp
#include "ilcc_internal.h"
#include <type_traits>
#ifdef ILCC_K6_TIMING
#include <algorithm>
#include <vector>
#endif

namespace ilcc {

#ifdef ILCC_K6_TIMING
constexpr int kProfWaves = 1 << 17, kProfWords = 16;
__device__ unsigned long long k6_prof[kProfWaves * kProfWords];
#define K6_NOW() __builtin_readcyclecounter()
#else
#define K6_NOW() 0ull
#endif
#ifndef ILCC_SEED_SHIFT
#define ILCC_SEED_SHIFT 4
#endif
constexpr int kSeedShift = ILCC_SEED_SHIFT;
constexpr int kTile = 4;
constexpr int kSlices = 4;
constexpr int kUnroll = 2;
constexpr int kStep = kSlices * kUnroll;
constexpr int kBoxShiftSmall = 3;
constexpr int kBoxShiftLarge = 2;
#ifndef ILCC_GROUP_SHIFT_SMALL
#define ILCC_GROUP_SHIFT_SMALL 2
#endif
#ifndef ILCC_GROUP_SHIFT_LARGE
#define ILCC_GROUP_SHIFT_LARGE 1
#endif
constexpr int kGroupShiftSmall = ILCC_GROUP_SHIFT_SMALL, kGroupShiftLarge = ILCC_GROUP_SHIFT_LARGE;
static_assert(kGroupShiftSmall >= 1 && kGroupShiftLarge >= 1,
              "k6_group_prepass stages M >> kGroupShift <= M / 2 points: launch_group_prepass sizes its LDS for that");
constexpr int kBoxFirstRound = 32;
constexpr int kBoxFirstRoundFrom = 8;
template <int THREADS>
constexpr int kBoxSegment = THREADS <= 256 ? 256 : 1024;
constexpr int kBoxTilesMax = 4096;
constexpr float kBoxSafety = 1.f - 0x1p-12f;
constexpr int kBoundRefresh = 256;

__device__ __forceinline__ float quad_sum(float v) {
  v += __uint_as_float(__builtin_amdgcn_update_dpp(0u, __float_as_uint(v), 0xB1 , 0xf, 0xf, false));
  v += __uint_as_float(__builtin_amdgcn_update_dpp(0u, __float_as_uint(v), 0x4E , 0xf, 0xf, false));
  return v;
}

__device__ __forceinline__ float lanes_sum(float v, uint32_t P) {
  v += __uint_as_float(__builtin_amdgcn_update_dpp(0u, __float_as_uint(v), 0xB1 , 0xf, 0xf, false));
  if (P > 2u) v += __uint_as_float(__builtin_amdgcn_update_dpp(0u, __float_as_uint(v), 0x4E , 0xf, 0xf, false));
  if (P > 4u) v += __uint_as_float(__builtin_amdgcn_update_dpp(0u, __float_as_uint(v), 0x141 , 0xf, 0xf, false));
  if (P > 8u) v += __uint_as_float(__builtin_amdgcn_update_dpp(0u, __float_as_uint(v), 0x140 , 0xf, 0xf, false));
  if (P > 16u) v += __shfl_xor(v, 16);
  if (P > 32u) v += __shfl_xor(v, 32);
  return v;
}

struct Best {
  float cost;
  uint32_t d2;
  uint32_t flat;
};
__device__ __forceinline__ bool better(float c, uint32_t d2, uint32_t flat, const Best& b) {
  return c < b.cost || (c == b.cost && (d2 < b.d2 || (d2 == b.d2 && flat < b.flat)));
}

template <bool AB>
__device__ __forceinline__ Best wave_argmin(Best best, uint32_t& ab) {
#pragma unroll
  for (int o = ILCC_WAVE / 2; o > 0; o >>= 1) {
    Best t;
    t.cost = __shfl_down(best.cost, o, ILCC_WAVE);
    t.d2 = __shfl_down(best.d2, o, ILCC_WAVE);
    t.flat = __shfl_down(best.flat, o, ILCC_WAVE);
    const uint32_t tab = AB ? __shfl_down(ab, o, ILCC_WAVE) : 0u;
    if (better(t.cost, t.d2, t.flat, best)) {
      best = t;
      if (AB) ab = tab;
    }
  }
  return best;
}
__device__ __forceinline__ Best wave_argmin(Best best) {
  uint32_t none = 0;
  return wave_argmin<false>(best, none);
}

template <int WAVES>
__device__ __forceinline__ Best block_argmin(const Best* s_best, const uint32_t* s_ab, uint32_t& ab) {
  Best b = s_best[0];
  if (s_ab) ab = s_ab[0];
  for (int w = 1; w < WAVES; ++w)
    if (better(s_best[w].cost, s_best[w].d2, s_best[w].flat, b)) {
      b = s_best[w];
      if (s_ab) ab = s_ab[w];
    }
  return b;
}

__device__ __forceinline__ float wave_min(float v) {
#pragma unroll
  for (int o = ILCC_WAVE / 2; o > 0; o >>= 1) v = fminf(v, __shfl_xor(v, o, ILCC_WAVE));
  return v;
}

__device__ __forceinline__ void score(float c0, float c1, int k, int ia, int ib, int n_ty, int n_tz, int c_th, int c_ty, int c_tz, Best& best,
                                      uint32_t& ab) {
  const uint32_t cell = ((uint32_t)k * (uint32_t)n_ty + (uint32_t)ia) * (uint32_t)n_tz + (uint32_t)ib;
  const uint32_t d2 = (uint32_t)((k - c_th) * (k - c_th) + (ia - c_ty) * (ia - c_ty) + (ib - c_tz) * (ib - c_tz));
  const uint32_t cab = ((uint32_t)ia << 16) | (uint32_t)ib;
  if (better(c0, d2, 2u * cell, best)) {
    best = Best{c0, d2, 2u * cell};
    ab = cab;
  }
  if (better(c1, d2, 2u * cell + 1u, best)) {
    best = Best{c1, d2, 2u * cell + 1u};
    ab = cab;
  }
}

__device__ __forceinline__ void no_candidate(GridPartial* out) { *out = GridPartial{__builtin_inff(), 0xFFFFFFFFu, 0xFFFFFFFFu, 0u}; }

enum EvalCounter { kEvalsAll = 0, kEvalsInterior = 1, kEvalsBox = 2 };
__device__ __forceinline__ void count_evals(unsigned long long* grid_iters, uint32_t f, EvalCounter which, unsigned long long n) {
  atomicAdd(grid_iters + (int)which * kIterSlots + (f & (kIterSlots - 1)), n);
}

__device__ __forceinline__ int window_origin(int centre, int before, int n, int width) {
  return min(max(centre - before, 0), max(n - width, 0));
}

__device__ __forceinline__ float2 rotate(float2 v, float cth, float sth) {
  return make_float2(fmaf(-sth, v.y, cth * v.x), fmaf(cth, v.y, sth * v.x));
}

__device__ __forceinline__ uint32_t walk_sample(uint32_t M, uint32_t at_least) { return min(M, max(at_least, M >> kSeedShift)); }
__device__ __forceinline__ void walk_prefix(uint32_t Ms, uint32_t M, uint32_t Mi_all, uint32_t n_rim_all, uint32_t& n_in, uint32_t& n_rm) {
  n_in = Mi_all;
  n_rm = n_rim_all;
  if (Ms < M) {
    n_in = (uint32_t)(((uint64_t)Mi_all * Ms) / M);
    n_rm = (uint32_t)(((uint64_t)n_rim_all * Ms) / M);
  }
}
__device__ __forceinline__ uint32_t layout_source(uint32_t sl, uint32_t n_in, uint32_t n_rm, uint32_t M, uint32_t Mi_all, uint32_t n_rim_all) {
  const uint32_t src = sl < n_in ? sl : sl < n_in + n_rm ? Mi_all + (sl - n_in) : Mi_all + n_rim_all + (sl - n_in - n_rm);
  return min(src, M - 1u);
}
struct FrameWalk {
  const float2* __restrict__ yz;
  const uint8_t* __restrict__ lab;
  uint32_t M, S, Mi_all, n_rim_all;
  bool layout;
  __device__ __forceinline__ FrameWalk(const Ctx& c, uint32_t f) : M(c.n_lab[f]), layout(M <= (uint32_t)kGridLdsPointsMax) {
    const uint64_t beg = c.off[f];
    yz = (layout ? c.walk_yz : c.yz) + beg;
    lab = (layout ? c.walk_lab : c.lab) + beg;
    S = (!layout && M) ? c.walk_stride[f] : 1u;
    Mi_all = layout ? c.walk_mi[f] : 0u;
    n_rim_all = layout ? c.walk_nrim[f] : 0u;
  }
  __device__ __forceinline__ uint32_t sample(uint32_t at_least) const { return walk_sample(M, at_least); }
  __device__ __forceinline__ void prefix(uint32_t Ms, uint32_t& n_in, uint32_t& n_rm) const { walk_prefix(Ms, M, Mi_all, n_rim_all, n_in, n_rm); }
  __device__ __forceinline__ uint32_t source(uint32_t sl, uint32_t n_in, uint32_t n_rm) const {
    return layout ? layout_source(sl, n_in, n_rm, M, Mi_all, n_rim_all) : (uint32_t)(((uint64_t)sl * S) % M);
  }
};

struct PointTerms {
  float pi, pj, hw;
};

template <bool OOB>
__device__ __forceinline__ void accumulate(const PointTerms& p, float ay, float az, float Wh, float Hh, float delta,
                                           float& A0, float& A1) {
  const float i = p.pi + ay, j = p.pj + az;
  const float fi = floorf(i), fj = floorf(j);
  const float ai = (i - fi) - 0.5f, aj = (j - fj) - 0.5f;
  const float Rin = 1.f - (fabsf(ai) + fabsf(aj));
  const float mf = __builtin_amdgcn_fractf(fmaf(0.5f, fi + fj, p.hw));
  const float nmf = 0.5f - mf;
  const float ui = fabsf(i - Wh) - Wh, uj = fabsf(j - Hh) - Hh;
  const bool oob = fmaxf(ui, uj) >= 0.f;
  auto sel = [&](float if_oob, float otherwise) -> float { return oob ? if_oob : otherwise; };
  float R, w0, w1;
  if (OOB) {
    R = sel(fabsf(ui) + fabsf(uj), Rin);
    w0 = sel(0.5f, mf);
    w1 = sel(0.5f, nmf);
  } else {
    R = sel(0.f, Rin);
    w0 = mf;
    w1 = nmf;
  }
  const float Q = fminf(R, delta);
  const float T = Q * fmaf(-0.5f, Q, R);
  A0 = fmaf(T, w0, A0);
  A1 = fmaf(T, w1, A1);
}

__device__ __forceinline__ void accumulate_interior(const PointTerms& p, float ay, float az, float delta, float& A0, float& A1) {
  const float i = p.pi + ay, j = p.pj + az;
  const float fi = floorf(i), fj = floorf(j);
  const float ai = (i - fi) - 0.5f, aj = (j - fj) - 0.5f;
  const float R = 1.f - (fabsf(ai) + fabsf(aj));
  const float mf = __builtin_amdgcn_fractf(fmaf(0.5f, fi + fj, p.hw));
  const float nmf = 0.5f - mf;
  const float Q = fminf(R, delta);
  const float T = Q * fmaf(-0.5f, Q, R);
  A0 = fmaf(T, mf, A0);
  A1 = fmaf(T, nmf, A1);
}


__device__ __forceinline__ void box_term(float pi_lo, float pi_hi, float pj_lo, float pj_hi, float alo, float ahi, float zlo, float zhi,
                                         float Wh, float Hh, float delta, float& lb, bool count = true) {
  const float i_lo = pi_lo + alo, i_hi = pi_hi + ahi, j_lo = pj_lo + zlo, j_hi = pj_hi + zhi;
  const float ui_lo = fabsf(i_lo - Wh) - Wh, ui_hi = fabsf(i_hi - Wh) - Wh;
// ... 991 lines not shown
    const int kr = (int)((s_pick[0] >> 1) / (uint32_t)(n_ty * n_tz));
    const int ra = min((int)(s_pick[1] >> 16), n_ty - 1), rb = min((int)(s_pick[1] & 0xFFFFu), n_tz - 1);
    const int a_org = window_origin(ra, 1, n_ty, kTile), b_org = window_origin(rb, 1, n_tz, kTile);
    const int k0 = kr - kAnchorThetas / 2;
    if (wid < kAnchorThetas * kAnchorParts) {
      const int t = wid % kAnchorThetas, part = wid / kAnchorThetas;
      anchor_walk(c.p, full, fw, min(max(k0 + t, 0), n_th - 1), a_org, b_org, s_ay, s_az, (uint32_t)part, kAnchorParts, s_part[t * kAnchorParts + part],
                  pts_done, pts_in);
    }
    __syncthreads();
    if (wid == 0) anchor_publish<kAnchorThetas, kAnchorParts>(full, c.grid_bound + f, s_part, k0, a_org, b_org, out);
  }
  if (lane == 0) {
    s_iters[wid] = pts_done;
    s_iters_in[wid] = pts_in;
  }
  __syncthreads();
  if (threadIdx.x == 0) {
    uint32_t it_sum = 0, in_sum = 0;
    for (int w = 0; w < kLocateWaves; ++w) {
      it_sum += s_iters[w];
      in_sum += s_iters_in[w];
    }
    count_evals(c.grid_iters, f, kEvalsAll, it_sum);
    count_evals(c.grid_iters, f, kEvalsInterior, in_sum);
  }
}

constexpr int kAnchorThreads = 512;
constexpr int kAnchorWaves = kAnchorThreads / ILCC_WAVE;
__global__ __launch_bounds__(kAnchorThreads) void k6_anchor(Ctx c, GridPass pass) {
  __shared__ float s_part[kAnchorWaves][16][2];
  __shared__ uint32_t s_iters[kAnchorWaves], s_iters_in[kAnchorWaves];
  const uint32_t f = blockIdx.y, kblk = blockIdx.x;
  GridPartial* out = &pass.out[(uint64_t)f * pass.blocks + kblk];
  const int lane = lane_id();
  const int wid = __builtin_amdgcn_readfirstlane(wave_id());
  uint32_t k2u = 0, ab = 0;
  Best sb{__builtin_inff(), 0xFFFFFFFFu, 0xFFFFFFFFu};
  if (c.res[f].status == ILCC_OK) sb = seed_argmin(pass.seed, f, k2u, ab);
  if (sb.flat == 0xFFFFFFFFu) {
    if (threadIdx.x == 0) no_candidate(out);
    return;
  }
  const int n_ty = pass.t.n_ty, n_tz = pass.t.n_tz;
  const int kr = (int)((sb.flat >> 1) / (uint32_t)(n_ty * n_tz));
  const int k0 = kr + (int)kblk - pass.radius_th;
  const int ra = min((int)(ab >> 16), n_ty - 1), rb = min((int)(ab & 0xFFFFu), n_tz - 1);
  const int a_org = window_origin(ra, 1, n_ty, kTile), b_org = window_origin(rb, 1, n_tz, kTile);
  uint32_t pts_done = 0, pts_in = 0;
  anchor_walk(c.p, pass.t, FrameWalk(c, f), min(max(k0, 0), pass.t.n_th - 1), a_org, b_org, pass.t.ay, pass.t.az, (uint32_t)wid, kAnchorWaves, s_part[wid], pts_done,
              pts_in);
  if (lane == 0) {
    s_iters[wid] = pts_done;
    s_iters_in[wid] = pts_in;
  }
  __syncthreads();
  if (wid == 0) anchor_publish<1, kAnchorWaves>(pass.t, pass.bound + f, s_part, k0, a_org, b_org, out);
  if (threadIdx.x == 0) {
    uint32_t it_sum = 0, in_sum = 0;
    for (int w = 0; w < kAnchorWaves; ++w) {
      it_sum += s_iters[w];
      in_sum += s_iters_in[w];
    }
    count_evals(c.grid_iters, f, kEvalsAll, it_sum);
    count_evals(c.grid_iters, f, kEvalsInterior, in_sum);
  }
}

void launch_anchor(const Ctx& c, const GridPass& pass, hipStream_t s) {
  hipLaunchKernelGGL(k6_anchor, dim3(pass.blocks, c.n_frames), dim3(kAnchorThreads), 0, s, c, pass);
}

size_t locate_lds_bytes(uint32_t sample_cap, int n_ty, int n_tz, int n_ty2, int n_tz2) {
  return (sizeof(float2) + sizeof(float)) * (size_t)sample_cap + sizeof(float2) * (size_t)kLocateThetasMax * sample_cap +
         sizeof(float) * (size_t)(n_ty + n_tz + n_ty2 + n_tz2);
}

void launch_locate(const Ctx& c, hipStream_t s, const LocatePlan& lp) {
  const size_t lds = locate_lds_bytes(lp.sample_cap, c.grid.n_ty, c.grid.n_tz, lp.seed.n_ty, lp.seed.n_tz);
  hipLaunchKernelGGL(k6_locate, dim3(c.n_frames), dim3(kLocateThreads), lds, s, c, lp);
}

constexpr int kRimMilli = 300;
constexpr int kWalkThreads = 256;
__global__ __launch_bounds__(kWalkThreads) void k5w_walk_order(Ctx c) {
  __shared__ uint8_t s_cls[kGridLdsPointsMax];
  __shared__ uint32_t s_in[kWalkThreads / ILCC_WAVE], s_rim[kWalkThreads / ILCC_WAVE], s_oth[kWalkThreads / ILCC_WAVE];
  const uint32_t f = blockIdx.x;
  if (c.res[f].status != ILCC_OK) return;
  const uint32_t M = c.n_lab[f];
  if (M == 0u || M > (uint32_t)kGridLdsPointsMax) {
    if (threadIdx.x == 0) {
      c.walk_mi[f] = 0u;
      c.walk_nrim[f] = 0u;
    }
    return;
  }
  const int lane = lane_id();
  const int wid = wave_id();
  const uint64_t beg = c.off[f];
  const float2* __restrict__ gyz = c.yz + beg;
  const uint8_t* __restrict__ glab = c.lab + beg;
  const uint32_t S = c.walk_stride[f];
  const float Wh = 0.5f * (float)c.p.board_w, Hh = 0.5f * (float)c.p.board_h;
  const GridTables& t = c.grid;
  const float ay_lo = t.ay[0], ay_hi = t.ay[t.n_ty - 1], az_lo = t.az[0], az_hi = t.az[t.n_tz - 1];
  const float ay_c = t.ay[t.c_ty], az_c = t.az[t.c_tz];
  const float rim_thr = -(float)kRimMilli * 1e-3f;
  const int n_th = t.n_th;
  float cmax = 0.f, smax = 0.f;
  for (int k = 0; k < n_th; ++k) {
    cmax = fmaxf(cmax, fabsf(t.cth[k]));
    smax = fmaxf(smax, fabsf(t.sth[k]));
  }
  const float room_i = fminf(fminf(ay_lo, ay_hi), 2.f * Wh - fmaxf(ay_lo, ay_hi)), room_j = fminf(fminf(az_lo, az_hi), 2.f * Hh - fmaxf(az_lo, az_hi));
  uint32_t cnt_in = 0, cnt_rim = 0;
  for (uint32_t sl = threadIdx.x; sl < M; sl += kWalkThreads) {
    const float2 v = gyz[(uint32_t)(((uint64_t)sl * S) % M)];
    const float bi = fmaf(fabsf(v.y), smax, fabsf(v.x) * cmax), bj = fmaf(fabsf(v.y), cmax, fabsf(v.x) * smax);
    const bool inside_always = bi + 1e-4f < room_i && bj + 1e-4f < room_j;
    int cl = 0;
    if (!inside_always) {
      const float2 p = rotate(v, t.cth[t.c_th], t.sth[t.c_th]);
      const float uc = fabsf((p.x + ay_c) - Wh) - Wh, wc = fabsf((p.y + az_c) - Hh) - Hh;
      cl = (fmaxf(uc, wc) > rim_thr) ? 2 : 1;
    }
    s_cls[sl] = (uint8_t)cl;
    cnt_in += cl == 0;
    cnt_rim += cl == 2;
  }
  cnt_in = wave_sum(cnt_in);
  cnt_rim = wave_sum(cnt_rim);
  if (lane == 0) {
    s_in[wid] = cnt_in;
    s_rim[wid] = cnt_rim;
  }
  __syncthreads();
  uint32_t Mi = 0, n_rim = 0;
  for (int w = 0; w < kWalkThreads / ILCC_WAVE; ++w) {
    Mi += s_in[w];
    n_rim += s_rim[w];
  }
  __syncthreads();
  if (threadIdx.x == 0) {
    c.walk_mi[f] = Mi;
    c.walk_nrim[f] = n_rim;
  }
  float2* __restrict__ wyz = c.walk_yz + beg;
  uint8_t* __restrict__ wlab = c.walk_lab + beg;
  uint32_t base_in = 0, base_rim = Mi, base_oth = Mi + n_rim;
  for (uint32_t c0 = 0; c0 < M; c0 += kWalkThreads) {
    const uint32_t sl = c0 + threadIdx.x;
    const int cl = sl < M ? (int)s_cls[sl] : -1;
    const unsigned long long m_in = __ballot(cl == 0), m_oth = __ballot(cl == 1), m_rim = __ballot(cl == 2);
    const unsigned long long below = (1ull << lane) - 1ull;
    if (lane == 0) {
      s_in[wid] = (uint32_t)__popcll(m_in);
      s_rim[wid] = (uint32_t)__popcll(m_rim);
      s_oth[wid] = (uint32_t)__popcll(m_oth);
    }
    __syncthreads();
    uint32_t pre_in = 0, pre_rim = 0, pre_oth = 0, tot_in = 0, tot_rim = 0, tot_oth = 0;
    for (int w = 0; w < kWalkThreads / ILCC_WAVE; ++w) {
      const uint32_t a = s_in[w], r = s_rim[w], o = s_oth[w];
      if (w < wid) {
        pre_in += a;
        pre_rim += r;
        pre_oth += o;
      }
      tot_in += a;
      tot_rim += r;
      tot_oth += o;
    }
    if (cl >= 0) {
      const uint32_t at = cl == 0   ? base_in + pre_in + (uint32_t)__popcll(m_in & below)
                          : cl == 2 ? base_rim + pre_rim + (uint32_t)__popcll(m_rim & below)
                                    : base_oth + pre_oth + (uint32_t)__popcll(m_oth & below);
      const uint32_t i = (uint32_t)(((uint64_t)sl * S) % M);
      wyz[at] = gyz[i];
      wlab[at] = glab[i];
    }
    base_in += tot_in;
    base_rim += tot_rim;
    base_oth += tot_oth;
    __syncthreads();
  }
}

void launch_walk_order(const Ctx& c, hipStream_t s) {
  hipLaunchKernelGGL(k5w_walk_order, dim3(c.n_frames), dim3(kWalkThreads), 0, s, c);
}

#ifdef ILCC_K6_ISA_PROBE
template <int N, bool BORDER>
__global__ void k6_isa_probe(const float* __restrict__ pts, float ay, float az, float Wh, float Hh, float delta, float* out) {
  float A0 = 0.f, A1 = 0.f;
  const float lay = ay + (float)threadIdx.x, laz = az - (float)threadIdx.x;
#pragma unroll
  for (int k = 0; k < N; ++k) {
    const PointTerms p{pts[3 * k], pts[3 * k + 1], pts[3 * k + 2]};
    if (BORDER)
      accumulate<true>(p, lay, laz, Wh, Hh, delta, A0, A1);
    else
      accumulate_interior(p, lay, laz, delta, A0, A1);
  }
  out[2 * threadIdx.x] = A0;
  out[2 * threadIdx.x + 1] = A1;
}
template <int N>
__global__ void k6_isa_probe_box(const float* __restrict__ pts, float alo, float ahi, float zlo, float zhi, float Wh, float Hh, float delta,
                                 float* out) {
  float lb = 0.f;
  const float t = (float)threadIdx.x;
#pragma unroll
  for (int k = 0; k < N; ++k) box_term(pts[2 * k], pts[2 * k], pts[2 * k + 1], pts[2 * k + 1], alo + t, ahi + t, zlo - t, zhi - t, Wh, Hh, delta, lb);
  out[threadIdx.x] = lb;
}
template __global__ void k6_isa_probe_box<1>(const float*, float, float, float, float, float, float, float, float*);
template __global__ void k6_isa_probe_box<3>(const float*, float, float, float, float, float, float, float, float*);
template __global__ void k6_isa_probe<1, true>(const float*, float, float, float, float, float, float*);
template __global__ void k6_isa_probe<3, true>(const float*, float, float, float, float, float, float*);
template __global__ void k6_isa_probe<1, false>(const float*, float, float, float, float, float, float*);
template __global__ void k6_isa_probe<3, false>(const float*, float, float, float, float, float, float*);
#endif

#ifdef ILCC_K6_TIMING
extern "C" int ilcc_debug_k6_profile(unsigned long long* out16, int clear) {
  static std::vector<unsigned long long> host((size_t)kProfWaves * kProfWords);
  if (hipMemcpyFromSymbol(host.data(), HIP_SYMBOL(k6_prof), host.size() * sizeof(unsigned long long)) != hipSuccess) return -1;
  for (int k = 0; k < 16; ++k) out16[k] = 0;
  for (size_t w = 0; w < (size_t)kProfWaves; ++w)
    for (int k = 0; k < kProfWords; ++k) out16[k] += host[w * kProfWords + k];
  if (clear) {
    std::fill(host.begin(), host.end(), 0ull);
    if (hipMemcpyToSymbol(HIP_SYMBOL(k6_prof), host.data(), host.size() * sizeof(unsigned long long)) != hipSuccess) return -1;
  }
  return 0;
}
#endif

uint32_t grid_cost_evals_per_count() { return kTile * kTile; }

hipError_t set_kernel_attributes_k6() {
  const void* fns[] = {(const void*)k6_grid_cost<true, true, false, kGridThreads>,  (const void*)k6_grid_cost<true, false, false, kGridThreads>,
                       (const void*)k6_grid_cost<false, true, false, kGridThreads>, (const void*)k6_grid_cost<false, false, false, kGridThreads>,
                       (const void*)k6_grid_cost<true, false, true, kGridThreads>,  (const void*)k6_grid_cost<false, false, true, kGridThreads>,
                       (const void*)k6_grid_cost<true, false, true, kGridThreadsLarge>,
                       (const void*)k6_group_prepass<kGridThreads>, (const void*)k6_group_prepass<kGridThreadsLarge>, (const void*)k6_locate};
  const int cap = (int)((sizeof(float2) + sizeof(float)) * (size_t)kGridLdsPointsMax + sizeof(float) * (size_t)kGridTableMax);
  for (const void* fn : fns) {
    const hipError_t e = hipFuncSetAttribute(fn, hipFuncAttributeMaxDynamicSharedMemorySize, cap);
    if (e != hipSuccess) return e;
  }
  return hipSuccess;
}

void launch_grid_cost(const Ctx& c, const GridPass& pass, hipStream_t s, int32_t use_oob, float* cost_volume, bool prune) {
  const dim3 grid(pass.blocks, c.n_frames), block(kGridThreads);
  const size_t lds = (sizeof(float2) + sizeof(float)) * (size_t)c.grid_lds_points + sizeof(float) * (size_t)(pass.t.n_ty + pass.t.n_tz);
  if (cost_volume) {
    if (use_oob)
      hipLaunchKernelGGL((k6_grid_cost<true, true, false, kGridThreads>), grid, block, lds, s, c, pass, cost_volume);
    else
      hipLaunchKernelGGL((k6_grid_cost<false, true, false, kGridThreads>), grid, block, lds, s, c, pass, cost_volume);
  } else if (prune) {
    if (use_oob && c.grid_lds_points > (uint32_t)kGridLargeFrom)
      hipLaunchKernelGGL((k6_grid_cost<true, false, true, kGridThreadsLarge>), grid, dim3(kGridThreadsLarge), lds, s, c, pass, cost_volume);
    else if (use_oob)
      hipLaunchKernelGGL((k6_grid_cost<true, false, true, kGridThreads>), grid, block, lds, s, c, pass, cost_volume);
// ... 12 lines not shown
```

### lidar_camera_calibration_amd/lidar_corners_est.py

```python
from __future__ import annotations

import ctypes as C
from typing import Optional, Sequence

import numpy as np

from . import _native as N


class IlccError(RuntimeError):
    def __init__(self, status: int, detail: str = ""):
        self.status = int(status)
        msg = N.strerror(status)
        super().__init__(f"{msg}: {detail}" if detail else msg)


class LidarCornersEst:

    def __init__(self, device: int = -1, max_frames: int = 1, max_points_per_frame: int = 150_000,
                 params: Optional[N.Params] = None):
        self._lib = N.lib()
        self.params = params if params is not None else N.default_params()
        self._device = device
        self._max_frames = int(max_frames)
# ... 103 lines not shown
    def color_by_gray_zone(self) -> np.ndarray:
        n = self._lib.ilcc_fetch_classes(self._h, 0, None, 0)
        if n < 0:
            raise IlccError(-n)
        cl = np.zeros(max(n, 1), dtype=np.uint8)
        self._lib.ilcc_fetch_classes(self._h, 0, cl.ctypes.data_as(C.POINTER(C.c_uint8)), n)
        lut = np.array([[10, 10, 10], [255, 0, 0], [255, 255, 255]], dtype=np.uint8)
        return lut[cl[:n]]

    def EuclideanCluster(self) -> bool:
        res = self._run()
        self.m_cloud_ROI = self._fetch(N.CLOUD_ROI)
        if res.status in (N.NO_ROI_POINTS, N.NO_CLUSTER, N.NO_PLANE):
            return False
        self.m_cloud_chessboard = self._fetch(N.CLOUD_CHESSBOARD)
        print("chessboard plane size:", len(self.m_cloud_chessboard))
        return True

    def PCA(self):
        res = self._run()
        self.m_cloud_PCA = self._fetch(N.CLOUD_PCA)
        self.pca_matrix = np.array(res.pca, dtype=np.float32).reshape(4, 4)
        self.m_gray_zone = np.array(res.gray_zone)

    def get_corners(self, corners: list) -> bool:
        res = self._run()
        if res.status == N.AMBIGUOUS and not self.accept_ambiguous:
            print("reject this scan (ambiguous: basin margin %.3g)" % res.basin_margin)
            return False
        if res.status not in (N.OK, N.AMBIGUOUS):
            print("reject this scan")
            return False
        if (res.flags & N.FLAG_LOW_COVERAGE) and not self.accept_low_coverage:
            print("reject this scan (pattern under-sampled: %d of %d squares hold points)"
                  % (res.cells_hit, self.params.board_w * self.params.board_h))
            return False
        c = res.corners_array()
        self.m_cloud_optim = self._fetch(N.CLOUD_OPTIM)
        self.m_cloud_corners = np.concatenate([c, np.full((len(c), 1), 50.0, np.float32)], 1)
        corners.extend(map(tuple, c.astype(np.float64)))
        return True

    @property
    def result(self) -> Optional[N.Result]:
        return self._result


class LidarCornersBatch:

    def __init__(self, max_frames: int, max_points_per_frame: int, params: Optional[N.Params] = None,
                 device: int = -1):
        self._lib = N.lib()
        self.params = params if params is not None else N.default_params()
        self._h = self._lib.ilcc_create(device, C.byref(self.params), int(max_frames),
                                        int(max_frames) * int(max_points_per_frame))
        if not self._h:
            raise IlccError(N.HIP_ERROR, self._lib.ilcc_last_error(None).decode())

    def close(self):
        if self._h:
            self._lib.ilcc_destroy(self._h)
            self._h = None

    def __del__(self):
        try:
            self.close()
        except Exception:
            pass

    def _err(self):
        return self._lib.ilcc_last_error(self._h).decode()

    def set_params(self, params: N.Params):
        self.params = params
        st = self._lib.ilcc_set_params(self._h, C.byref(params))
        if st != N.OK:
            raise IlccError(st, self._err())

    def set_result_mode(self, mode: int):
        st = self._lib.ilcc_set_result_mode(self._h, int(mode))
        if st != N.OK:
            raise IlccError(st, self._err())

    def wait_compact(self, ticket) -> np.ndarray:
        t, n_frames = ticket
        width = int(self._lib.ilcc_record_floats(self._h, t))
        if width == 0:
            raise IlccError(N.BAD_ARGUMENT, "wait_compact: no batch in flight under this ticket")
        rec = np.empty((n_frames, width), dtype=np.float32)
        st = self._lib.ilcc_wait_compact(self._h, t, N.fptr(rec), rec.size)
        if st != N.OK:
            raise IlccError(st, self._err())
        return rec

    def fetch_results(self, first: int, n: int):
        res = (N.Result * n)()
        st = self._lib.ilcc_fetch_results(self._h, int(first), int(n), res)
        if st != N.OK:
            raise IlccError(st, self._err())
        return res

    def reserve(self, labelled_points_per_frame: int, roi_points_per_frame: int):
        st = self._lib.ilcc_reserve(self._h, int(labelled_points_per_frame), int(roi_points_per_frame))
        if st != N.OK:
            raise IlccError(st, self._err())

    def extract(self, clouds: np.ndarray, clicks: np.ndarray, offsets: Optional[np.ndarray] = None):
        clouds = np.ascontiguousarray(clouds, dtype=np.float32)
        clicks = np.ascontiguousarray(clicks, dtype=np.float32).reshape(-1, 3)
        f = len(clicks)
        if offsets is None:
            n = clouds.shape[-2]
            offsets = np.arange(f + 1, dtype=np.uint64) * np.uint64(n)
        offsets = np.ascontiguousarray(offsets, dtype=np.uint64)
        res = (N.Result * f)()
        st = self._lib.ilcc_extract_batch(self._h, N.fptr(clouds), offsets.ctypes.data_as(C.POINTER(C.c_uint64)),
                                          f, N.fptr(clicks), res)
        if st != N.OK:
            raise IlccError(st, self._err())
        return res

    def extract_device(self, d_xyzi_ptr: int, n_frames: int, n_points: int, d_clicks_ptr: int):
        offsets = np.arange(n_frames + 1, dtype=np.uint64) * np.uint64(n_points)
        res = (N.Result * n_frames)()
        st = self._lib.ilcc_extract_batch_device(self._h, C.c_void_p(d_xyzi_ptr),
                                                 offsets.ctypes.data_as(C.POINTER(C.c_uint64)), n_frames,
                                                 C.c_void_p(d_clicks_ptr), res)
        if st != N.OK:
            raise IlccError(st, self._err())
        return res

    def submit_device(self, d_xyzi_ptr: int, n_frames: int, n_points: int, d_clicks_ptr: int):
        offsets = np.arange(n_frames + 1, dtype=np.uint64) * np.uint64(n_points)
        ticket = C.c_int32(-1)
        st = self._lib.ilcc_submit_batch_device(self._h, C.c_void_p(d_xyzi_ptr),
                                                offsets.ctypes.data_as(C.POINTER(C.c_uint64)), n_frames,
                                                C.c_void_p(d_clicks_ptr), C.byref(ticket))
        if st != N.OK:
            raise IlccError(st, self._err())
        return ticket.value, n_frames

    def submit_host(self, xyzi_ptr: int, n_frames: int, n_points: int, clicks_ptr: int):
        offsets = np.arange(n_frames + 1, dtype=np.uint64) * np.uint64(n_points)
        ticket = C.c_int32(-1)
        st = self._lib.ilcc_submit_batch(self._h, C.c_void_p(xyzi_ptr), offsets.ctypes.data_as(C.POINTER(C.c_uint64)),
                                         n_frames, C.c_void_p(clicks_ptr), C.byref(ticket))
        if st != N.OK:
            raise IlccError(st, self._err())
        return ticket.value, n_frames

    def wait(self, ticket, d_records_ptr: Optional[int] = None, n_corners: int = 0, tag_base: int = 0,
             want_results: bool = True):
        t, n_frames = ticket
        res = (N.Result * n_frames)() if (want_results or d_records_ptr is None) else None
        if d_records_ptr is not None:
            st = self._lib.ilcc_wait_records_device(self._h, t, res, C.c_void_p(d_records_ptr), n_corners,
                                                    int(tag_base) & 0xFFFFFFFF)
        else:
            st = self._lib.ilcc_wait(self._h, t, res)
        if st != N.OK:
            raise IlccError(st, self._err())
        return res

    def fetch_cloud(self, frame: int, which: int) -> np.ndarray:
        n = self._lib.ilcc_fetch_cloud(self._h, frame, which, None, 0)
        if n < 0:
# ... 141 lines not shown
```

Before: 1.278 million.

## Fuse RANSAC, histogram and walk-order into one front-end kernel; one-pass ROI crop

Merges the RANSAC plane, plane-frame histogram and walk-order kernels into a single per-frame kernel. It keeps cluster points staged in LDS across the stages so the labelled points are not reloaded from global memory, and it removes two launches. For large batches it also adds a one-block-per-frame ROI crop that counts and compacts in a single pass, replacing the count-then-scatter pair. A debug switch restores separate launches. Risks include larger LDS use and lower occupancy in the fused kernel, and one block per frame can leave the GPU underused on big frames.

```diff
diff --git a/include/ilcc_hip.h b/include/ilcc_hip.h
--- a/include/ilcc_hip.h
+++ b/include/ilcc_hip.h
@@ -195,6 +195,8 @@
 int32_t ilcc_debug_timeline_enable(ilcc_handle* h, int32_t on);
 int32_t ilcc_debug_timeline_fetch(ilcc_handle* h, double* rows, uint32_t cap_rows);
 
+int32_t ilcc_debug_separate_launches(ilcc_handle* h, int32_t on);
+
 void ilcc_get_timing(const ilcc_handle* h, ilcc_timing* t);
 void ilcc_reset_timing(ilcc_handle* h);
 
diff --git a/lidar_camera_calibration_amd/_native.py b/lidar_camera_calibration_amd/_native.py
--- a/lidar_camera_calibration_amd/_native.py
+++ b/lidar_camera_calibration_amd/_native.py
@@ -26,7 +26,7 @@
     "ilcc_grid_cost", "ilcc_grid_solve", "ilcc_pattern_refine", "ilcc_get_theta_t", "ilcc_get_timing", "ilcc_reset_timing",
     "ilcc_save_corners2txt", "ilcc_read_lidar_corners",
     "ilcc_set_result_mode", "ilcc_wait_compact", "ilcc_record_floats", "ilcc_fetch_results",
-    "ilcc_debug_timeline_enable", "ilcc_debug_timeline_fetch",
+    "ilcc_debug_timeline_enable", "ilcc_debug_timeline_fetch", "ilcc_debug_separate_launches",
 ]
 ABI_VERSION = 5
 RESULTS_FULL, RESULTS_COMPACT = 0, 1
@@ -206,6 +206,9 @@
         L.ilcc_debug_timeline_enable.restype = C.c_int32
         L.ilcc_debug_timeline_fetch.argtypes = [vp, C.POINTER(C.c_double), C.c_uint32]
         L.ilcc_debug_timeline_fetch.restype = C.c_int32
+        if hasattr(L, "ilcc_debug_separate_launches"):
+            L.ilcc_debug_separate_launches.argtypes = [vp, C.c_int32]
+            L.ilcc_debug_separate_launches.restype = C.c_int32
         L.ilcc_fetch_results.argtypes = [vp, C.c_uint32, C.c_uint32, rp]
         L.ilcc_fetch_results.restype = C.c_int32
         _lib = L
diff --git a/lidar_camera_calibration_amd/csrc/ilcc_api.cpp b/lidar_camera_calibration_amd/csrc/ilcc_api.cpp
--- a/lidar_camera_calibration_amd/csrc/ilcc_api.cpp
+++ b/lidar_camera_calibration_amd/csrc/ilcc_api.cpp
@@ -119,6 +119,7 @@
   ilcc_timing timing{};
   hipEvent_t tl_ref = nullptr;
   bool tl_on = false;
+  bool separate_launches = false;
   std::vector<double> tl_rows;
   std::string err;
 };
@@ -624,9 +625,9 @@
   return ILCC_OK;
 }
 
-int32_t enqueue_grid_search(ilcc_handle* h, Slot& sl, const Ctx& c, hipStream_t s, uint32_t n_frames, bool chain) {
+int32_t enqueue_grid_search(ilcc_handle* h, Slot& sl, const Ctx& c, hipStream_t s, uint32_t n_frames, bool chain, bool walk_laid_out = false) {
   const bool prune = h->p.grid_prune != 0;
-  launch_walk_order(c, s);
+  if (!walk_laid_out) launch_walk_order(c, s);
   HIP_TRY(h, hipEventRecord(sl.ev[kEvWalkOrdered], s));
   GridSeed located{};
   if (h->seed_grid.n_th > 0 && h->p.n_th >= 8 && h->p.n_ty >= 8 && h->p.n_tz >= 8) {
@@ -691,7 +692,7 @@
   Ctx c = make_ctx(h, sl, d_xyzi, d_clicks, n_frames, chunks);
   HIP_TRY(h, hipEventRecord(sl.ev[kEvStart], s));
   if (!no_crop) {
-    launch_roi_crop(c, s, sl.ev[kEvCropCounted]);
+    launch_roi_crop(c, s, sl.ev[kEvCropCounted], !h->separate_launches && n_frames >= (uint32_t)kCropFrameMinFrames);
     HIP_TRY(h, hipEventRecord(sl.ev[kEvCropped], s));
     launch_cluster(c, s);
   } else {
@@ -714,13 +715,19 @@
     HIP_TRY(h, hipMemcpyAsync(sl.h_online + h->max_frames, sl.d_nfinite, sizeof(uint32_t) * n_frames, hipMemcpyDeviceToHost, s));
   }
   HIP_TRY(h, hipEventRecord(sl.ev[kEvClustered], s));
-  launch_ransac_plane(c, s);
-  HIP_TRY(h, hipEventRecord(sl.ev[kEvPlane], s));
-  launch_plane_frame_hist(c, s);
   sl.grid = !front_only && h->p.solver == ILCC_SOLVER_GRID;
+  const bool one_launch = !h->separate_launches && front_end_fusable(c);
+  if (one_launch) {
+    launch_front_end(c, s, sl.grid);
+    HIP_TRY(h, hipEventRecord(sl.ev[kEvPlane], s));
+  } else {
+    launch_ransac_plane(c, s);
+    HIP_TRY(h, hipEventRecord(sl.ev[kEvPlane], s));
+    launch_plane_frame_hist(c, s);
+  }
   HIP_TRY(h, hipEventRecord(sl.ev[kEvLabelled], s));
   if (sl.grid) {
-    const int32_t st = enqueue_grid_search(h, sl, c, s, n_frames, true);
+    const int32_t st = enqueue_grid_search(h, sl, c, s, n_frames, true, one_launch);
     if (st != ILCC_OK) return st;
   }
   HIP_TRY(h, hipEventRecord(sl.ev[kEvSearched], s));
@@ -1654,6 +1661,18 @@
   return ILCC_OK;
 }
 
+int32_t ilcc_debug_separate_launches(ilcc_handle* h, int32_t on) {
+  if (!h) return ILCC_BAD_ARGUMENT;
+  for (const Slot& sl : h->slots) {
+    if (sl.busy) {
+      h->err = "ilcc_debug_separate_launches with a batch in flight: ilcc_wait first";
+      return ILCC_BAD_ARGUMENT;
+    }
+  }
+  h->separate_launches = on != 0;
+  return ILCC_OK;
+}
+
 int32_t ilcc_debug_timeline_fetch(ilcc_handle* h, double* rows, uint32_t cap_rows) {
   if (!h || (!rows && cap_rows)) return -ILCC_BAD_ARGUMENT;
   const size_t have = h->tl_rows.size() / ILCC_TIMELINE_COLS;
diff --git a/lidar_camera_calibration_amd/csrc/ilcc_internal.h b/lidar_camera_calibration_amd/csrc/ilcc_internal.h
--- a/lidar_camera_calibration_amd/csrc/ilcc_internal.h
+++ b/lidar_camera_calibration_amd/csrc/ilcc_internal.h
@@ -28,6 +28,7 @@
 #endif
 constexpr int kSmallBatchFrames = ILCC_SMALL_BATCH;
 constexpr int kHistThreads = ILCC_K45_THREADS;
+constexpr int kWalkThreads = 256;
 #ifndef ILCC_K6_THREADS
 #define ILCC_K6_THREADS 256
 #endif
@@ -274,10 +275,15 @@
 constexpr int kRefineThetaStride = 2;
 constexpr int kLocateMinFrames = 512;
 
-void launch_roi_crop(const Ctx& c, hipStream_t s, hipEvent_t after_count = nullptr);
+void launch_roi_crop(const Ctx& c, hipStream_t s, hipEvent_t after_count = nullptr, bool one_pass = false);
+constexpr int kCropFrameMinFrames = 512;
 void launch_cluster(const Ctx& c, hipStream_t s);
 void launch_ransac_plane(const Ctx& c, hipStream_t s);
 void launch_plane_frame_hist(const Ctx& c, hipStream_t s);
+void launch_front_end(const Ctx& c, hipStream_t s, bool walk_layout);
+inline bool front_end_fusable(const Ctx& c) {
+  return kPlaneThreads == kHistThreads && kHistThreads == kWalkThreads && c.n_frames > (uint32_t)kSmallBatchFrames && !c.wide;
+}
 void launch_walk_order(const Ctx& c, hipStream_t s);
 void launch_grid_cost(const Ctx& c, const GridPass& pass, hipStream_t s, int32_t use_oob, float* cost_volume , bool prune);
 void launch_group_prepass(const Ctx& c, const GridPass& full, hipStream_t s);
diff --git a/lidar_camera_calibration_amd/csrc/k1_roi_crop.hip b/lidar_camera_calibration_amd/csrc/k1_roi_crop.hip
--- a/lidar_camera_calibration_amd/csrc/k1_roi_crop.hip
+++ b/lidar_camera_calibration_amd/csrc/k1_roi_crop.hip
@@ -29,18 +29,12 @@
   return fin && in;
 }
 
-__global__ __launch_bounds__(kCropThreads) void k1_roi_count(Ctx c) {
-  const uint32_t f = blockIdx.y, s = blockIdx.x;
-  if (c.online_tier == 2u && c.frame_flags[f] == 0u) return;
-  const uint64_t beg = c.off[f], end = c.off[f + 1];
-  const uint64_t n = end - beg;
-  if (s == 0) {
-    uint32_t* w = reinterpret_cast<uint32_t*>(&c.res[f]);
-    for (uint32_t k = threadIdx.x; k < sizeof(ilcc_result) / 4; k += kCropThreads) w[k] = 0u;
-    if (f == 0 && threadIdx.x < kBatchWords && c.online_tier != 2u) c.grid_iters[threadIdx.x] = 0ull;
-    __syncthreads();
-  }
-  if (s == 0 && threadIdx.x == 0) {
+__device__ __forceinline__ void reset_frame(const Ctx& c, const uint32_t f, const uint64_t n) {
+  uint32_t* w = reinterpret_cast<uint32_t*>(&c.res[f]);
+  for (uint32_t k = threadIdx.x; k < sizeof(ilcc_result) / 4; k += kCropThreads) w[k] = 0u;
+  if (f == 0 && threadIdx.x < kBatchWords && c.online_tier != 2u) c.grid_iters[threadIdx.x] = 0ull;
+  __syncthreads();
+  if (threadIdx.x == 0) {
     if (c.tie_count) c.tie_count[f] = 0u;
     ilcc_result* r = &c.res[f];
     r->status = ILCC_OK;
@@ -60,6 +54,14 @@
     c.grid_bound_sub[f] = 0x7f800000u;
     if (c.online_tier == 1u) c.frame_flags[f] = 0u;
   }
+}
+
+__global__ __launch_bounds__(kCropThreads) void k1_roi_count(Ctx c) {
+  const uint32_t f = blockIdx.y, s = blockIdx.x;
+  if (c.online_tier == 2u && c.frame_flags[f] == 0u) return;
+  const uint64_t beg = c.off[f], end = c.off[f + 1];
+  const uint64_t n = end - beg;
+  if (s == 0) reset_frame(c, f, n);
   const uint64_t cbeg = (uint64_t)s * kCropChunk;
   uint32_t cnt = 0, fin = 0;
   unsigned long long* masks = c.crop_masks + ((uint64_t)f * c.crop_chunks + s) * (kCropChunk / ILCC_WAVE);
@@ -170,7 +172,82 @@
   }
 }
 
-void launch_roi_crop(const Ctx& c, hipStream_t s, hipEvent_t after_count) {
+constexpr int kCropFrameTrips = 8;
+constexpr int kCropFrameChunk = kCropFrameTrips * kCropThreads;
+constexpr int kCropFrameCounts = kCropFrameTrips * (kCropThreads / ILCC_WAVE);
+static_assert(kCropFrameCounts <= ILCC_WAVE, "one popcount per lane");
+
+template <bool FINITE_BOX>
+__device__ __forceinline__ uint32_t crop_frame(const float4* __restrict__ src, float4* __restrict__ dst, const uint64_t n, const Box& b,
+                                               uint32_t (*s_cnt)[kCropFrameCounts]) {
+  const int lane = lane_id(), w = wave_id();
+  constexpr int kWaves = kCropThreads / ILCC_WAVE;
+  if (n == 0) return 0u;
+  auto load_chunk = [&](float4 (&q)[kCropFrameTrips], const uint64_t cbeg) {
+#pragma unroll
+    for (int k = 0; k < kCropFrameTrips; ++k) {
+      const uint64_t i = cbeg + (uint64_t)k * kCropThreads + threadIdx.x;
+      const f32x4 v = __builtin_nontemporal_load(reinterpret_cast<const f32x4*>(src + (i < n ? i : n - 1)));
+      q[k] = make_float4(v.x, v.y, v.z, v.w);
+    }
+  };
+  uint32_t running = 0;
+  auto chunk = [&](float4 (&cur)[kCropFrameTrips], float4 (&nxt)[kCropFrameTrips], const uint64_t cbeg, const int pb) {
+    load_chunk(nxt, cbeg + kCropFrameChunk);
+    unsigned long long mk[kCropFrameTrips];
+#pragma unroll
+    for (int k = 0; k < kCropFrameTrips; ++k) {
+      const bool keep = (cbeg + (uint64_t)k * kCropThreads + threadIdx.x < n) && keep_point<FINITE_BOX>(cur[k], b);
+      mk[k] = __ballot(keep);
+      if (lane == 0) s_cnt[pb][k * kWaves + w] = (uint32_t)__popcll(mk[k]);
+    }
+    __syncthreads();
+    uint32_t incl = lane < kCropFrameCounts ? s_cnt[pb][lane] : 0u;
+    const uint32_t own = incl;
+#pragma unroll
+    for (int o = 1; o < ILCC_WAVE; o <<= 1) {
+      const uint32_t t = __shfl_up(incl, o, ILCC_WAVE);
+      if (lane >= o) incl += t;
+    }
+    const uint32_t excl = incl - own;
+#pragma unroll
+    for (int k = 0; k < kCropFrameTrips; ++k) {
+      const uint32_t before = __shfl(excl, k * kWaves + w, ILCC_WAVE);
+      if ((mk[k] >> lane) & 1ull) dst[running + before + (uint32_t)__popcll(mk[k] & ((1ull << lane) - 1ull))] = cur[k];
+    }
+    running += __shfl(incl, ILCC_WAVE - 1, ILCC_WAVE);
+  };
+  float4 qa[kCropFrameTrips], qb[kCropFrameTrips];
+  load_chunk(qa, 0);
+  for (uint64_t cbeg = 0; cbeg < n; cbeg += 2 * kCropFrameChunk) {
+    chunk(qa, qb, cbeg, 0);
+    if (cbeg + kCropFrameChunk >= n) break;
+    chunk(qb, qa, cbeg + kCropFrameChunk, 1);
+  }
+  return running;
+}
+
+__global__ __launch_bounds__(kCropThreads, 4) void k1_roi_crop_frame(Ctx c) {
+  const uint32_t f = blockIdx.x;
+  const uint64_t beg = c.off[f], end = c.off[f + 1];
+  const uint64_t n = end - beg;
+  reset_frame(c, f, n);
+  __shared__ uint32_t s_cnt[2][kCropFrameCounts];
+  const Box b = make_box(c, f);
+  const bool finite_box = isfinite(b.lo[0]) && isfinite(b.hi[0]) && isfinite(b.lo[1]) && isfinite(b.hi[1]) && isfinite(b.lo[2]) && isfinite(b.hi[2]);
+  const uint32_t all = finite_box ? crop_frame<true>(c.xyzi + beg, c.roi + beg, n, b, s_cnt) : crop_frame<false>(c.xyzi + beg, c.roi + beg, n, b, s_cnt);
+  if (threadIdx.x == 0) {
+    c.res[f].n_roi = (int32_t)all;
+    if (all == 0) c.res[f].status = ILCC_NO_ROI_POINTS;
+  }
+}
+
+void launch_roi_crop(const Ctx& c, hipStream_t s, hipEvent_t after_count, bool one_pass) {
+  if (one_pass && c.online_tier == 0u) {
+    hipLaunchKernelGGL(k1_roi_crop_frame, dim3(c.n_frames), dim3(kCropThreads), 0, s, c);
+    if (after_count) (void)hipEventRecord(after_count, s);
+    return;
+  }
   const dim3 grid(c.crop_chunks, c.n_frames);
   hipLaunchKernelGGL(k1_roi_count, grid, dim3(kCropThreads), 0, s, c);
   if (after_count) (void)hipEventRecord(after_count, s);
diff --git a/lidar_camera_calibration_amd/csrc/k345_front_end.hip b/lidar_camera_calibration_amd/csrc/k345_front_end.hip
--- /dev/null
+++ b/lidar_camera_calibration_amd/csrc/k345_front_end.hip
@@ -0,0 +1,37 @@
+#include "k3_ransac_plane.h"
+#include "k45_plane_frame_hist.h"
+#include "k5w_walk_order.h"
+
+namespace ilcc {
+
+constexpr int kFrontThreads = kPlaneThreads;
+static_assert(kRansacLdsPoints * sizeof(float4) >= (size_t)kGridLdsPointsMax, "K5w's classes fit the unused staging");
+
+__global__ __launch_bounds__(kFrontThreads) void k345_front_end(Ctx c, uint32_t walk_layout) {
+  __shared__ float4 s_P[kRansacLdsPoints];
+  __shared__ uint32_t sc[64];
+  __shared__ double scd[16 * 6 + 8];
+  extern __shared__ int s_hist[];
+  const uint32_t f = blockIdx.x;
+  if (c.res[f].status != ILCC_OK) return;
+  const uint64_t beg = c.off[f];
+  uint32_t n_plane, n_lab, S;
+  bool staged;
+  if (!ransac_plane_frame(c, f, s_P, sc, scd, true, n_plane, staged)) return;
+  if (staged) {
+    if (!plane_frame_hist_frame(c, f, s_P, n_plane, sc, scd, s_hist, s_P, n_lab, S) || !walk_layout) return;
+    uint8_t* bytes = reinterpret_cast<uint8_t*>(s_P);
+    walk_order_frame(c, f, n_lab, S, WalkSource{reinterpret_cast<const float*>(s_P), 4u, bytes + 8, 16u}, bytes + 12, 16u, sc);
+  } else {
+    if (!plane_frame_hist_frame(c, f, c.board + beg, n_plane, sc, scd, s_hist, nullptr, n_lab, S) || !walk_layout) return;
+    walk_order_frame(c, f, n_lab, S, WalkSource{reinterpret_cast<const float*>(c.yz + beg), 2u, c.lab + beg, 1u},
+                     reinterpret_cast<uint8_t*>(s_P), 1u, sc);
+  }
+}
+
+void launch_front_end(const Ctx& c, hipStream_t s, bool walk_layout) {
+  const size_t lds = sizeof(int) * (size_t)(c.p.hist_bins + 1);
+  hipLaunchKernelGGL(k345_front_end, dim3(c.n_frames), dim3(kFrontThreads), lds, s, c, walk_layout ? 1u : 0u);
+}
+
+}
diff --git a/lidar_camera_calibration_amd/csrc/k3_ransac_plane.h b/lidar_camera_calibration_amd/csrc/k3_ransac_plane.h
--- /dev/null
+++ b/lidar_camera_calibration_amd/csrc/k3_ransac_plane.h
@@ -0,0 +1,278 @@
+#pragma once
+
+#include "eig3.h"
+#include "ilcc_internal.h"
+
+namespace ilcc {
+
+__device__ __forceinline__ uint32_t hash_u32(uint32_t x) {
+  x ^= x >> 16;
+  x *= 0x7feb352dU;
+  x ^= x >> 15;
+  x *= 0x846ca68bU;
+  x ^= x >> 16;
+  return x;
+}
+__device__ __forceinline__ uint32_t sample_index(uint32_t seed, uint32_t h, uint32_t k, uint32_t m) {
+  const uint32_t r = hash_u32(seed ^ hash_u32(h * 3u + k + 0x9E3779B9u));
+  return (uint32_t)(((uint64_t)r * (uint64_t)m) >> 32);
+}
+
+__device__ __forceinline__ bool plane_from_3(const float4 p0, const float4 p1, const float4 p2,
+                                             float pl[4]) {
+  const float ax = p1.x - p0.x, ay = p1.y - p0.y, az = p1.z - p0.z;
+  const float bx = p2.x - p0.x, by = p2.y - p0.y, bz = p2.z - p0.z;
+  float nx = ay * bz - az * by;
+  float ny = az * bx - ax * bz;
+  float nz = ax * by - ay * bx;
+  float n2 = nx * nx;
+  n2 = n2 + ny * ny;
+  n2 = n2 + nz * nz;
+  if (!(n2 > 1e-12f)) return false;
+  const float nrm = sqrtf(n2);
+  nx = nx / nrm;
+  ny = ny / nrm;
+  nz = nz / nrm;
+  float d = nx * p0.x;
+  d = d + ny * p0.y;
+  d = d + nz * p0.z;
+  pl[0] = nx;
+  pl[1] = ny;
+  pl[2] = nz;
+  pl[3] = -d;
+  return true;
+}
+
+__device__ __forceinline__ float plane_dist(const float pl[4], const float4 q) {
+  float s = pl[0] * q.x;
+  s = s + pl[1] * q.y;
+  s = s + pl[2] * q.z;
+  s = s + pl[3];
+  return fabsf(s);
+}
+
+constexpr int kRansacLdsPoints = 2048;
+
+__device__ __forceinline__ bool ransac_plane_frame(const Ctx& c, const uint32_t f, float4* s_P, uint32_t* sc, double* scd,
+                                                   const bool keep_in_lds, uint32_t& n_plane, bool& staged) {
+  const uint32_t kThreads = blockDim.x;
+  __shared__ float s_plane[4];
+  ilcc_result* r = &c.res[f];
+  n_plane = 0u;
+  staged = false;
+  const uint32_t M = (uint32_t)r->n_cluster;
+  const uint64_t beg = c.off[f];
+  const float4* __restrict__ G = c.cluster + beg;
+  const uint32_t tid = threadIdx.x;
+  const int lane = lane_id(), wid = wave_id();
+  const float thr = (float)c.p.ransac_thresh;
+  if (M < 3) {
+    if (tid == 0) r->status = ILCC_NO_PLANE;
+    return false;
+  }
+  const float4* P = G;
+  if (M <= (uint32_t)kRansacLdsPoints) {
+    for (uint32_t i = tid; i < M; i += kThreads) s_P[i] = G[i];
+    __syncthreads();
+    P = s_P;
+    staged = true;
+  }
+
+  const uint32_t n_waves = kThreads / ILCC_WAVE;
+  auto score = [&](uint32_t h, uint32_t beat, uint32_t& cnt) -> bool {
+    const uint32_t i0 = sample_index(c.p.ransac_seed, h, 0, M);
+    const uint32_t i1 = sample_index(c.p.ransac_seed, h, 1, M);
+    const uint32_t i2 = sample_index(c.p.ransac_seed, h, 2, M);
+    float pl[4];
+    cnt = 0;
+    if (i0 == i1 || i0 == i2 || i1 == i2) return false;
+    if (!plane_from_3(P[i0], P[i1], P[i2], pl)) return false;
+    for (uint32_t base = 0; base < M; base += ILCC_WAVE) {
+      const uint32_t i = base + lane;
+      const bool in = (i < M) && plane_dist(pl, P[i]) < thr;
+      cnt += (uint32_t)__popcll(__ballot(in));
+      if (cnt + (M - min(M, base + (uint32_t)ILCC_WAVE)) <= beat) break;
+    }
+    return true;
+  };
+  if (c.p.ransac_probability > 0.0) {
+    __shared__ uint32_t s_state[5];
+    __shared__ double s_k;
+    if (tid == 0) {
+      s_state[0] = 0u;
+      s_state[1] = 0xFFFFFFFFu;
+      s_state[2] = s_state[3] = s_state[4] = 0u;
+      s_k = 1.0;
+    }
+    __syncthreads();
+    const double log_probability = log(1.0 - c.p.ransac_probability);
+    const double one_over_indices = 1.0 / (double)M;
+    const uint32_t max_it = (uint32_t)c.p.ransac_hyp, max_skip = max_it * 10u;
+    for (uint32_t h0 = 0;; h0 += n_waves) {
+      uint32_t cnt;
+      const bool valid = score(h0 + (uint32_t)wid, s_state[0], cnt);
+      if (lane == 0) sc[wid] = valid ? cnt : 0xFFFFFFFFu;
+      __syncthreads();
+      if (tid == 0) {
+        uint32_t best = s_state[0], best_h = s_state[1], it = s_state[2], skip = s_state[3], stop = 0u;
+        double k = s_k;
+        for (uint32_t j = 0; j < n_waves; ++j) {
+          if (!((double)it < k && skip < max_skip)) {
+            stop = 1u;
+            break;
+          }
+          const uint32_t v = sc[j];
+          if (v == 0xFFFFFFFFu) {
+            ++skip;
+            continue;
+          }
+          if (v > best) {
+            best = v;
+            best_h = h0 + j;
+            const double w = (double)best * one_over_indices;
+            double p_no_outliers = 1.0 - w * w * w;
+            p_no_outliers = fmax(2.220446049250313e-16, p_no_outliers);
+            p_no_outliers = fmin(1.0 - 2.220446049250313e-16, p_no_outliers);
+            k = log_probability / log(p_no_outliers);
+          }
+          ++it;
+          if (it > max_it) {
+            stop = 1u;
+            break;
+          }
+        }
+        if (!((double)it < k && skip < max_skip)) stop = 1u;
+        s_state[0] = best;
+        s_state[1] = best_h;
+        s_state[2] = it;
+        s_state[3] = skip;
+        s_state[4] = stop;
+        s_k = k;
+      }
+      __syncthreads();
+      if (s_state[4] != 0u) break;
+    }
+    if (tid == 0) {
+      sc[32] = s_state[0];
+      sc[33] = s_state[1];
+    }
+  } else {
+    uint32_t best_cnt = 0, best_h = 0xFFFFFFFFu;
+    for (uint32_t h = (uint32_t)wid; h < (uint32_t)c.p.ransac_hyp; h += n_waves) {
+      uint32_t cnt;
+      if (!score(h, best_cnt, cnt)) continue;
+      if (cnt > best_cnt) {
+        best_cnt = cnt;
+        best_h = h;
+      }
+    }
+    if (lane == 0) {
+      sc[wid] = best_cnt;
+      sc[16 + wid] = best_h;
+    }
+    __syncthreads();
+    if (tid == 0) {
+      uint32_t bc = 0, bh = 0xFFFFFFFFu;
+      for (int w = 0; w < (int)n_waves; ++w)
+        if (sc[w] > bc || (sc[w] == bc && sc[w] > 0 && sc[16 + w] < bh)) {
+          bc = sc[w];
+          bh = sc[16 + w];
+        }
+      sc[32] = bc;
+      sc[33] = bh;
+    }
+  }
+  if (tid == 0 && sc[32] > 0u) {
+    const uint32_t bh = sc[33];
+    float pl[4];
+    plane_from_3(P[sample_index(c.p.ransac_seed, bh, 0, M)], P[sample_index(c.p.ransac_seed, bh, 1, M)],
+                 P[sample_index(c.p.ransac_seed, bh, 2, M)], pl);
+    for (int k = 0; k < 4; ++k) s_plane[k] = pl[k];
+  }
+  __syncthreads();
+  const uint32_t bc = sc[32];
+  if (bc == 0) {
+    if (tid == 0) r->status = ILCC_NO_PLANE;
+    return false;
+  }
+  float pl[4] = {s_plane[0], s_plane[1], s_plane[2], s_plane[3]};
+
+  if (bc > 3) {
+    double sx = 0, sy = 0, sz = 0;
+    for (uint32_t i = tid; i < M; i += kThreads) {
+      const float4 q = P[i];
+      if (plane_dist(pl, q) < thr) {
+        sx += q.x;
+        sy += q.y;
+        sz += q.z;
+      }
+    }
+    double sums3[3] = {sx, sy, sz};
+    block_sum_n<3>(sums3, scd);
+    const double cx = sums3[0] / bc, cy = sums3[1] / bc, cz = sums3[2] / bc;
+    double cv[6] = {0, 0, 0, 0, 0, 0};
+    for (uint32_t i = tid; i < M; i += kThreads) {
+      const float4 q = P[i];
+      if (plane_dist(pl, q) < thr) {
+        const double dx = q.x - cx, dy = q.y - cy, dz = q.z - cz;
+        cv[0] += dx * dx;
+        cv[1] += dx * dy;
+        cv[2] += dx * dz;
+        cv[3] += dy * dy;
+        cv[4] += dy * dz;
+        cv[5] += dz * dz;
+      }
+    }
+    __syncthreads();
+    block_sum_n<6>(cv, scd);
+    double cs[6];
+    for (int k = 0; k < 6; ++k) cs[k] = cv[k] / bc;
+    if (tid == 0) {
+      const double cov[9] = {cs[0], cs[1], cs[2], cs[1], cs[3], cs[4], cs[2], cs[4], cs[5]};
+      double w[3], v[3][3];
+      eig3_sym(cov, w, v);
+      double n[3] = {v[0][0], v[0][1], v[0][2]};
+      if (n[0] * pl[0] + n[1] * pl[1] + n[2] * pl[2] < 0) {
+        n[0] = -n[0];
+        n[1] = -n[1];
+        n[2] = -n[2];
+      }
+      s_plane[0] = (float)n[0];
+      s_plane[1] = (float)n[1];
+      s_plane[2] = (float)n[2];
+      s_plane[3] = (float)(-(n[0] * cx + n[1] * cy + n[2] * cz));
+    }
+    __syncthreads();
+    for (int k = 0; k < 4; ++k) pl[k] = s_plane[k];
+  }
+
+  const bool compact = keep_in_lds && staged;
+  float4* __restrict__ dst = c.board + beg;
+  uint32_t running = 0;
+  for (uint32_t base = 0; base < M; base += kThreads) {
+    const uint32_t i = base + tid;
+    float4 q = make_float4(0.f, 0.f, 0.f, 0.f);
+    bool keep = false;
+    if (i < M) {
+      q = P[i];
+      keep = plane_dist(pl, q) < thr;
+    }
+    uint32_t tot;
+    const uint32_t rank = block_rank(keep, sc + 40, tot);
+    if (keep) {
+      dst[running + rank] = q;
+      if (compact) s_P[running + rank] = q;
+    }
+    running += tot;
+  }
+  if (tid == 0) {
+    r->n_plane = (int32_t)running;
+    for (int k = 0; k < 4; ++k) r->plane[k] = pl[k];
+    if (running < 3) r->status = ILCC_NO_PLANE;
+  }
+  __syncthreads();
+  n_plane = running;
+  return running >= 3;
+}
+
+}
diff --git a/lidar_camera_calibration_amd/csrc/k3_ransac_plane.hip b/lidar_camera_calibration_amd/csrc/k3_ransac_plane.hip
--- a/lidar_camera_calibration_amd/csrc/k3_ransac_plane.hip
+++ b/lidar_camera_calibration_amd/csrc/k3_ransac_plane.hip
@@ -1,270 +1,16 @@
-#include "eig3.h"
-#include "ilcc_internal.h"
+#include "k3_ransac_plane.h"
 
 namespace ilcc {
 
-__device__ __forceinline__ uint32_t hash_u32(uint32_t x) {
-  x ^= x >> 16;
-  x *= 0x7feb352dU;
-  x ^= x >> 15;
-  x *= 0x846ca68bU;
-  x ^= x >> 16;
-  return x;
-}
-__device__ __forceinline__ uint32_t sample_index(uint32_t seed, uint32_t h, uint32_t k, uint32_t m) {
-  const uint32_t r = hash_u32(seed ^ hash_u32(h * 3u + k + 0x9E3779B9u));
-  return (uint32_t)(((uint64_t)r * (uint64_t)m) >> 32);
-}
-
-__device__ __forceinline__ bool plane_from_3(const float4 p0, const float4 p1, const float4 p2,
-                                             float pl[4]) {
-  const float ax = p1.x - p0.x, ay = p1.y - p0.y, az = p1.z - p0.z;
-  const float bx = p2.x - p0.x, by = p2.y - p0.y, bz = p2.z - p0.z;
-  float nx = ay * bz - az * by;
-  float ny = az * bx - ax * bz;
-  float nz = ax * by - ay * bx;
-  float n2 = nx * nx;
-  n2 = n2 + ny * ny;
-  n2 = n2 + nz * nz;
-  if (!(n2 > 1e-12f)) return false;
-  const float nrm = sqrtf(n2);
-  nx = nx / nrm;
-  ny = ny / nrm;
-  nz = nz / nrm;
-  float d = nx * p0.x;
-  d = d + ny * p0.y;
-  d = d + nz * p0.z;
-  pl[0] = nx;
-  pl[1] = ny;
-  pl[2] = nz;
-  pl[3] = -d;
-  return true;
-}
-
-__device__ __forceinline__ float plane_dist(const float pl[4], const float4 q) {
-  float s = pl[0] * q.x;
-  s = s + pl[1] * q.y;
-  s = s + pl[2] * q.z;
-  s = s + pl[3];
-  return fabsf(s);
-}
-
-constexpr int kRansacLdsPoints = 2048;
-
 __global__ __launch_bounds__(kPlaneThreadsSmallBatch) void k3_ransac_plane(Ctx c) {
-  const uint32_t kThreads = blockDim.x;
   __shared__ float4 s_P[kRansacLdsPoints];
   __shared__ uint32_t sc[64];
   __shared__ double scd[16 * 6 + 8];
-  __shared__ float s_plane[4];
   const uint32_t f = blockIdx.x;
-  ilcc_result* r = &c.res[f];
-  if (r->status != ILCC_OK) return;
-  const uint32_t M = (uint32_t)r->n_cluster;
-  const uint64_t beg = c.off[f];
-  const float4* __restrict__ G = c.cluster + beg;
-  const uint32_t tid = threadIdx.x;
-  const int lane = lane_id(), wid = wave_id();
-  const float thr = (float)c.p.ransac_thresh;
-  if (M < 3) {
-    if (tid == 0) r->status = ILCC_NO_PLANE;
-    return;
-  }
-  const float4* P = G;
-  if (M <= (uint32_t)kRansacLdsPoints) {
-    for (uint32_t i = tid; i < M; i += kThreads) s_P[i] = G[i];
-    __syncthreads();
-    P = s_P;
-  }
-
-  const uint32_t n_waves = kThreads / ILCC_WAVE;
-  auto score = [&](uint32_t h, uint32_t beat, uint32_t& cnt) -> bool {
-    const uint32_t i0 = sample_index(c.p.ransac_seed, h, 0, M);
-    const uint32_t i1 = sample_index(c.p.ransac_seed, h, 1, M);
-    const uint32_t i2 = sample_index(c.p.ransac_seed, h, 2, M);
-    float pl[4];
-    cnt = 0;
-    if (i0 == i1 || i0 == i2 || i1 == i2) return false;
-    if (!plane_from_3(P[i0], P[i1], P[i2], pl)) return false;
-    for (uint32_t base = 0; base < M; base += ILCC_WAVE) {
-      const uint32_t i = base + lane;
-      const bool in = (i < M) && plane_dist(pl, P[i]) < thr;
-      cnt += (uint32_t)__popcll(__ballot(in));
-      if (cnt + (M - min(M, base + (uint32_t)ILCC_WAVE)) <= beat) break;
-    }
-    return true;
-  };
-  if (c.p.ransac_probability > 0.0) {
-    __shared__ uint32_t s_state[5];
-    __shared__ double s_k;
-    if (tid == 0) {
-      s_state[0] = 0u;
-      s_state[1] = 0xFFFFFFFFu;
-      s_state[2] = s_state[3] = s_state[4] = 0u;
-      s_k = 1.0;
-    }
-    __syncthreads();
-    const double log_probability = log(1.0 - c.p.ransac_probability);
-    const double one_over_indices = 1.0 / (double)M;
-    const uint32_t max_it = (uint32_t)c.p.ransac_hyp, max_skip = max_it * 10u;
-    for (uint32_t h0 = 0;; h0 += n_waves) {
-      uint32_t cnt;
-      const bool valid = score(h0 + (uint32_t)wid, s_state[0], cnt);
-      if (lane == 0) sc[wid] = valid ? cnt : 0xFFFFFFFFu;
-      __syncthreads();
-      if (tid == 0) {
-        uint32_t best = s_state[0], best_h = s_state[1], it = s_state[2], skip = s_state[3], stop = 0u;
-        double k = s_k;
-        for (uint32_t j = 0; j < n_waves; ++j) {
-          if (!((double)it < k && skip < max_skip)) {
-            stop = 1u;
-            break;
-          }
-          const uint32_t v = sc[j];
-          if (v == 0xFFFFFFFFu) {
-            ++skip;
-            continue;
-          }
-          if (v > best) {
-            best = v;
-            best_h = h0 + j;
-            const double w = (double)best * one_over_indices;
-            double p_no_outliers = 1.0 - w * w * w;
-            p_no_outliers = fmax(2.220446049250313e-16, p_no_outliers);
-            p_no_outliers = fmin(1.0 - 2.220446049250313e-16, p_no_outliers);
-            k = log_probability / log(p_no_outliers);
-          }
-          ++it;
-          if (it > max_it) {
-            stop = 1u;
-            break;
-          }
-        }
-        if (!((double)it < k && skip < max_skip)) stop = 1u;
-        s_state[0] = best;
-        s_state[1] = best_h;
-        s_state[2] = it;
-        s_state[3] = skip;
-        s_state[4] = stop;
-        s_k = k;
-      }
-      __syncthreads();
-      if (s_state[4] != 0u) break;
-    }
-    if (tid == 0) {
-      sc[32] = s_state[0];
-      sc[33] = s_state[1];
-    }
-  } else {
-    uint32_t best_cnt = 0, best_h = 0xFFFFFFFFu;
-    for (uint32_t h = (uint32_t)wid; h < (uint32_t)c.p.ransac_hyp; h += n_waves) {
-      uint32_t cnt;
-      if (!score(h, best_cnt, cnt)) continue;
-      if (cnt > best_cnt) {
-        best_cnt = cnt;
-        best_h = h;
-      }
-    }
-    if (lane == 0) {
-      sc[wid] = best_cnt;
-      sc[16 + wid] = best_h;
-    }
-    __syncthreads();
-    if (tid == 0) {
-      uint32_t bc = 0, bh = 0xFFFFFFFFu;
-      for (int w = 0; w < (int)n_waves; ++w)
-        if (sc[w] > bc || (sc[w] == bc && sc[w] > 0 && sc[16 + w] < bh)) {
-          bc = sc[w];
-          bh = sc[16 + w];
-        }
-      sc[32] = bc;
-      sc[33] = bh;
-    }
-  }
-  if (tid == 0 && sc[32] > 0u) {
-    const uint32_t bh = sc[33];
-    float pl[4];
-    plane_from_3(P[sample_index(c.p.ransac_seed, bh, 0, M)], P[sample_index(c.p.ransac_seed, bh, 1, M)],
-                 P[sample_index(c.p.ransac_seed, bh, 2, M)], pl);
-    for (int k = 0; k < 4; ++k) s_plane[k] = pl[k];
-  }
-  __syncthreads();
-  const uint32_t bc = sc[32];
-  if (bc == 0) {
-    if (tid == 0) r->status = ILCC_NO_PLANE;
-    return;
-  }
-  float pl[4] = {s_plane[0], s_plane[1], s_plane[2], s_plane[3]};
-
-  if (bc > 3) {
-    double sx = 0, sy = 0, sz = 0;
-    for (uint32_t i = tid; i < M; i += kThreads) {
-      const float4 q = P[i];
-      if (plane_dist(pl, q) < thr) {
-        sx += q.x;
-        sy += q.y;
-        sz += q.z;
-      }
-    }
-    double sums3[3] = {sx, sy, sz};
-    block_sum_n<3>(sums3, scd);
-    const double cx = sums3[0] / bc, cy = sums3[1] / bc, cz = sums3[2] / bc;
-    double cv[6] = {0, 0, 0, 0, 0, 0};
-    for (uint32_t i = tid; i < M; i += kThreads) {
-      const float4 q = P[i];
-      if (plane_dist(pl, q) < thr) {
-        const double dx = q.x - cx, dy = q.y - cy, dz = q.z - cz;
-        cv[0] += dx * dx;
-        cv[1] += dx * dy;
-        cv[2] += dx * dz;
-        cv[3] += dy * dy;
-        cv[4] += dy * dz;
-        cv[5] += dz * dz;
-      }
-    }
-    __syncthreads();
-    block_sum_n<6>(cv, scd);
-    double cs[6];
-    for (int k = 0; k < 6; ++k) cs[k] = cv[k] / bc;
-    if (tid == 0) {
-      const double cov[9] = {cs[0], cs[1], cs[2], cs[1], cs[3], cs[4], cs[2], cs[4], cs[5]};
-      double w[3], v[3][3];
-      eig3_sym(cov, w, v);
-      double n[3] = {v[0][0], v[0][1], v[0][2]};
-      if (n[0] * pl[0] + n[1] * pl[1] + n[2] * pl[2] < 0) {
-        n[0] = -n[0];
-        n[1] = -n[1];
-        n[2] = -n[2];
-      }
-      s_plane[0] = (float)n[0];
-      s_plane[1] = (float)n[1];
-      s_plane[2] = (float)n[2];
-      s_plane[3] = (float)(-(n[0] * cx + n[1] * cy + n[2] * cz));
-    }
-    __syncthreads();
-    for (int k = 0; k < 4; ++k) pl[k] = s_plane[k];
-  }
-
-  float4* __restrict__ dst = c.board + beg;
-  uint32_t running = 0;
-  for (uint32_t base = 0; base < M; base += kThreads) {
-    const uint32_t i = base + tid;
-    float4 q = make_float4(0.f, 0.f, 0.f, 0.f);
-    bool keep = false;
-    if (i < M) {
-      q = P[i];
-      keep = plane_dist(pl, q) < thr;
-    }
-    uint32_t tot;
-    const uint32_t rank = block_rank(keep, sc + 40, tot);
-    if (keep) dst[running + rank] = q;
-    running += tot;
-  }
-  if (tid == 0) {
-    r->n_plane = (int32_t)running;
-    for (int k = 0; k < 4; ++k) r->plane[k] = pl[k];
-    if (running < 3) r->status = ILCC_NO_PLANE;
-  }
+  if (c.res[f].status != ILCC_OK) return;
+  uint32_t n_plane;
+  bool staged;
+  (void)ransac_plane_frame(c, f, s_P, sc, scd, false, n_plane, staged);
 }
 
 void launch_ransac_plane(const Ctx& c, hipStream_t s) {
diff --git a/lidar_camera_calibration_amd/csrc/k45_plane_frame_hist.h b/lidar_camera_calibration_amd/csrc/k45_plane_frame_hist.h
--- /dev/null
+++ b/lidar_camera_calibration_amd/csrc/k45_plane_frame_hist.h
@@ -0,0 +1,230 @@
+#pragma once
+
+#include "eig3.h"
+#include "ilcc_internal.h"
+
+namespace ilcc {
+
+__device__ __forceinline__ bool plane_frame_hist_frame(const Ctx& c, const uint32_t f, const float4* P, const uint32_t M, uint32_t* sc,
+                                                       double* scd, int* s_hist, float4* s_keep, uint32_t& n_lab, uint32_t& S) {
+  __shared__ float s_pca[16];
+  __shared__ float s_mm[34];
+  __shared__ double s_gz[2];
+  __shared__ int s_status;
+  __shared__ uint32_t s_stride;
+
+  ilcc_result* r = &c.res[f];
+  n_lab = 0u;
+  S = 1u;
+  const uint64_t beg = c.off[f];
+  const uint32_t tid = threadIdx.x;
+  const int lane = lane_id(), wid = wave_id();
+  if (M < 3) {
+    if (tid == 0) r->status = ILCC_TOO_FEW_POINTS;
+    return false;
+  }
+
+  double sx = 0, sy = 0, sz = 0, si = 0;
+  float vmin = 3.402823466e38f, vmax = -3.402823466e38f;
+  for (uint32_t i = tid; i < M; i += kHistThreads) {
+    const float4 q = P[i];
+    sx += q.x;
+    sy += q.y;
+    sz += q.z;
+    si += (double)q.w;
+    vmin = fminf(vmin, q.w);
+    vmax = fmaxf(vmax, q.w);
+  }
+  double s4[4] = {sx, sy, sz, si};
+  block_sum_n<4>(s4, scd);
+  const double cx = (double)(float)(s4[0] / M);
+  const double cy = (double)(float)(s4[1] / M);
+  const double cz = (double)(float)(s4[2] / M);
+  const double isum = s4[3];
+  double cv[6] = {0, 0, 0, 0, 0, 0};
+  for (uint32_t i = tid; i < M; i += kHistThreads) {
+    const float4 q = P[i];
+    const double dx = q.x - cx, dy = q.y - cy, dz = q.z - cz;
+    cv[0] += dx * dx;
+    cv[1] += dx * dy;
+    cv[2] += dx * dz;
+    cv[3] += dy * dy;
+    cv[4] += dy * dz;
+    cv[5] += dz * dz;
+  }
+  __syncthreads();
+  block_sum_n<6>(cv, scd);
+  double cs[6];
+  for (int k = 0; k < 6; ++k) cs[k] = cv[k] / M;
+#pragma unroll
+  for (int o = 32; o > 0; o >>= 1) {
+    vmin = fminf(vmin, __shfl_down(vmin, o, ILCC_WAVE));
+    vmax = fmaxf(vmax, __shfl_down(vmax, o, ILCC_WAVE));
+  }
+  if (lane == 0) {
+    s_mm[wid] = vmin;
+    s_mm[16 + wid] = vmax;
+  }
+  __syncthreads();
+  if (tid == 0) {
+    const double cov[9] = {cs[0], cs[1], cs[2], cs[1], cs[3], cs[4], cs[2], cs[4], cs[5]};
+    double w[3], v[3][3];
+    eig3_sym(cov, w, v);
+    double e0[3] = {v[0][0], v[0][1], v[0][2]};
+    double e1[3] = {v[1][0], v[1][1], v[1][2]};
+    if (e0[0] * cx + e0[1] * cy + e0[2] * cz > 0) {
+      e0[0] = -e0[0];
+      e0[1] = -e0[1];
+      e0[2] = -e0[2];
+    }
+    int big = 0;
+    for (int a = 1; a < 3; ++a)
+      if (fabs(e1[a]) > fabs(e1[big])) big = a;
+    if (e1[big] < 0) {
+      e1[0] = -e1[0];
+      e1[1] = -e1[1];
+      e1[2] = -e1[2];
+    }
+    float f0[3], f1[3], f2[3];
+    for (int a = 0; a < 3; ++a) {
+      f0[a] = (float)e0[a];
+      f1[a] = (float)e1[a];
+    }
+    f2[0] = f0[1] * f1[2] - f0[2] * f1[1];
+    f2[1] = f0[2] * f1[0] - f0[0] * f1[2];
+    f2[2] = f0[0] * f1[1] - f0[1] * f1[0];
+    const float cf[3] = {(float)cx, (float)cy, (float)cz};
+    const float* rows[3] = {f0, f1, f2};
+    for (int rr = 0; rr < 3; ++rr) {
+      for (int a = 0; a < 3; ++a) s_pca[4 * rr + a] = rows[rr][a];
+      float t = rows[rr][0] * cf[0];
+      t = t + rows[rr][1] * cf[1];
+      t = t + rows[rr][2] * cf[2];
+      s_pca[4 * rr + 3] = -1.0f * t;
+    }
+    s_pca[12] = s_pca[13] = s_pca[14] = 0.f;
+    s_pca[15] = 1.f;
+    for (int k = 0; k < 16; ++k) r->pca[k] = s_pca[k];
+    float mn = s_mm[0], mx = s_mm[16];
+    for (int w2 = 1; w2 < kHistThreads / ILCC_WAVE; ++w2) {
+      mn = fminf(mn, s_mm[w2]);
+      mx = fmaxf(mx, s_mm[16 + w2]);
+    }
+    s_mm[32] = mn;
+    s_mm[33] = mx;
+  }
+  const int HL = c.p.hist_bins;
+  for (int b = (int)tid; b <= HL; b += kHistThreads) s_hist[b] = 0;
+  __syncthreads();
+
+  float4* __restrict__ Q = c.pca + beg;
+  const double mn = (double)s_mm[32], mx = (double)s_mm[33];
+  const bool flat = !(mx > mn);
+  const double factor = flat ? 0.0 : HL / (mx - mn);
+  for (uint32_t i = tid; i < M; i += kHistThreads) {
+    const float4 q = P[i];
+    float o[3];
+#pragma unroll
+    for (int rr = 0; rr < 3; ++rr) {
+      float s = s_pca[4 * rr] * q.x;
+      s = s + s_pca[4 * rr + 1] * q.y;
+      s = s + s_pca[4 * rr + 2] * q.z;
+      s = s + s_pca[4 * rr + 3];
+      o[rr] = s;
+    }
+    Q[i] = make_float4(o[0], o[1], o[2], q.w);
+    if (s_keep) s_keep[i] = make_float4(o[0], o[1], o[2], q.w);
+    if (!flat) {
+      const double sample = (double)q.w - mn;
+      int bin = (int)round(sample * factor);
+      bin = bin < 0 ? 0 : (bin > HL ? HL : bin);
+      atomicAdd(&s_hist[bin], 1);
+    }
+  }
+  __syncthreads();
+
+  __shared__ unsigned long long s_top[2];
+  if (tid == 0) s_top[0] = s_top[1] = 0ull;
+  __syncthreads();
+  const bool hist_ok = !(flat || HL <= 0);
+  const double mean = isum / M;
+  const double bin_width = (mx - mn) / HL;
+  if (hist_ok) {
+    for (int bb = (int)tid; bb < HL; bb += kHistThreads) {
+      const int cb = s_hist[bb];
+      bool first = true;
+      for (int b2 = 0; b2 < bb; ++b2) first = first && (s_hist[b2] != cb);
+      if (!first) continue;
+      const double edge = bin_width * (double)bb + mn;
+      const int side = edge > mean ? 1 : (edge < mean ? 0 : -1);
+      if (side >= 0) atomicMax(&s_top[side], ((unsigned long long)(uint32_t)(cb + 1) << 32) | (unsigned long long)(uint32_t)bb);
+    }
+  }
+  __syncthreads();
+  if (tid == 0) {
+    int status = ILCC_OK;
+    if (!hist_ok || s_top[0] == 0ull || s_top[1] == 0ull) {
+      status = ILCC_DEGENERATE_HIST;
+    } else {
+      const double low = bin_width * (double)(uint32_t)(s_top[0] & 0xFFFFFFFFull) + mn;
+      const double high = bin_width * (double)(uint32_t)(s_top[1] & 0xFFFFFFFFull) + mn;
+      const double rate = c.p.gray_rate;
+      s_gz[0] = ((rate - 1) * low + high) / rate;
+      s_gz[1] = (low + (rate - 1) * high) / rate;
+      r->gray_zone[0] = s_gz[0];
+      r->gray_zone[1] = s_gz[1];
+    }
+    s_status = status;
+    if (status != ILCC_OK) r->status = status;
+  }
+  __syncthreads();
+  if (s_status != ILCC_OK) return false;
+
+  const double gz0 = s_gz[0], gz1 = s_gz[1];
+  float2* __restrict__ YZ = c.yz + beg;
+  uint8_t* __restrict__ LB = c.lab + beg;
+  uint8_t* __restrict__ CL = c.cls + beg;
+  uint32_t running = 0, nb = 0, nw = 0;
+  for (uint32_t base = 0; base < M; base += kHistThreads) {
+    const uint32_t i = base + tid;
+    bool keep = false;
+    uint8_t l = 0;
+    float4 q = make_float4(0.f, 0.f, 0.f, 0.f);
+    if (i < M) {
+      q = s_keep ? s_keep[i] : Q[i];
+      if ((double)q.w < gz0) {
+        keep = true;
+        l = 0;
+      } else if ((double)q.w > gz1) {
+        keep = true;
+        l = 1;
+      }
+      CL[i] = keep ? (uint8_t)(2 * l) : (uint8_t)1;
+    }
+    uint32_t tot, totw;
+    const uint32_t rank = block_rank(keep, sc, tot);
+    (void)block_rank(keep && l == 1, sc + 20, totw);
+    if (keep) {
+      YZ[running + rank] = make_float2(q.y, q.z);
+      LB[running + rank] = l;
+      if (s_keep) s_keep[running + rank] = make_float4(q.y, q.z, __uint_as_float((uint32_t)l), 0.f);
+    }
+    running += tot;
+    nw += totw;
+    nb += tot - totw;
+  }
+  if (tid == 0) {
+    r->n_black = (int32_t)nb;
+    r->n_white = (int32_t)nw;
+    r->n_gray = (int32_t)(M - running);
+    c.n_lab[f] = running;
+    s_stride = walk_stride(running);
+    c.walk_stride[f] = s_stride;
+  }
+  __syncthreads();
+  n_lab = running;
+  S = s_stride;
+  return true;
+}
+
+}
diff --git a/lidar_camera_calibration_amd/csrc/k45_plane_frame_hist.hip b/lidar_camera_calibration_amd/csrc/k45_plane_frame_hist.hip
--- a/lidar_camera_calibration_amd/csrc/k45_plane_frame_hist.hip
+++ b/lidar_camera_calibration_amd/csrc/k45_plane_frame_hist.hip
@@ -1,224 +1,16 @@
-#include "eig3.h"
-#include "ilcc_internal.h"
+#include "k45_plane_frame_hist.h"
 
 namespace ilcc {
 
 __global__ __launch_bounds__(kHistThreads) void k45_plane_frame_hist(Ctx c) {
   __shared__ uint32_t sc[64];
   __shared__ double scd[16 * 6 + 8];
-  __shared__ float s_pca[16];
-  __shared__ float s_mm[34];
-  __shared__ double s_gz[2];
-  __shared__ int s_status;
   extern __shared__ int s_hist[];
-
   const uint32_t f = blockIdx.x;
-  ilcc_result* r = &c.res[f];
-  if (r->status != ILCC_OK) return;
-  const uint32_t M = (uint32_t)r->n_plane;
-  const uint64_t beg = c.off[f];
-  const float4* __restrict__ P = c.board + beg;
-  const uint32_t tid = threadIdx.x;
-  const int lane = lane_id(), wid = wave_id();
-  if (M < 3) {
-    if (tid == 0) r->status = ILCC_TOO_FEW_POINTS;
-    return;
-  }
-
-  double sx = 0, sy = 0, sz = 0, si = 0;
-  float vmin = 3.402823466e38f, vmax = -3.402823466e38f;
-  for (uint32_t i = tid; i < M; i += kHistThreads) {
-    const float4 q = P[i];
-    sx += q.x;
-    sy += q.y;
-    sz += q.z;
-    si += (double)q.w;
-    vmin = fminf(vmin, q.w);
-    vmax = fmaxf(vmax, q.w);
-  }
-  double s4[4] = {sx, sy, sz, si};
-  block_sum_n<4>(s4, scd);
-  const double cx = (double)(float)(s4[0] / M);
-  const double cy = (double)(float)(s4[1] / M);
-  const double cz = (double)(float)(s4[2] / M);
-  const double isum = s4[3];
-  double cv[6] = {0, 0, 0, 0, 0, 0};
-  for (uint32_t i = tid; i < M; i += kHistThreads) {
-    const float4 q = P[i];
-    const double dx = q.x - cx, dy = q.y - cy, dz = q.z - cz;
-    cv[0] += dx * dx;
-    cv[1] += dx * dy;
-    cv[2] += dx * dz;
-    cv[3] += dy * dy;
-    cv[4] += dy * dz;
-    cv[5] += dz * dz;
-  }
-  __syncthreads();
-  block_sum_n<6>(cv, scd);
-  double cs[6];
-  for (int k = 0; k < 6; ++k) cs[k] = cv[k] / M;
-#pragma unroll
-  for (int o = 32; o > 0; o >>= 1) {
-    vmin = fminf(vmin, __shfl_down(vmin, o, ILCC_WAVE));
-    vmax = fmaxf(vmax, __shfl_down(vmax, o, ILCC_WAVE));
-  }
-  if (lane == 0) {
-    s_mm[wid] = vmin;
-    s_mm[16 + wid] = vmax;
-  }
-  __syncthreads();
-  if (tid == 0) {
-    const double cov[9] = {cs[0], cs[1], cs[2], cs[1], cs[3], cs[4], cs[2], cs[4], cs[5]};
-    double w[3], v[3][3];
-    eig3_sym(cov, w, v);
-    double e0[3] = {v[0][0], v[0][1], v[0][2]};
-    double e1[3] = {v[1][0], v[1][1], v[1][2]};
-    if (e0[0] * cx + e0[1] * cy + e0[2] * cz > 0) {
-      e0[0] = -e0[0];
-      e0[1] = -e0[1];
-      e0[2] = -e0[2];
-    }
-    int big = 0;
-    for (int a = 1; a < 3; ++a)
-      if (fabs(e1[a]) > fabs(e1[big])) big = a;
-    if (e1[big] < 0) {
-      e1[0] = -e1[0];
-      e1[1] = -e1[1];
-      e1[2] = -e1[2];
-    }
-    float f0[3], f1[3], f2[3];
-    for (int a = 0; a < 3; ++a) {
-      f0[a] = (float)e0[a];
-      f1[a] = (float)e1[a];
-    }
-    f2[0] = f0[1] * f1[2] - f0[2] * f1[1];
-    f2[1] = f0[2] * f1[0] - f0[0] * f1[2];
-    f2[2] = f0[0] * f1[1] - f0[1] * f1[0];
-    const float cf[3] = {(float)cx, (float)cy, (float)cz};
-    const float* rows[3] = {f0, f1, f2};
-    for (int rr = 0; rr < 3; ++rr) {
-      for (int a = 0; a < 3; ++a) s_pca[4 * rr + a] = rows[rr][a];
-      float t = rows[rr][0] * cf[0];
-      t = t + rows[rr][1] * cf[1];
-      t = t + rows[rr][2] * cf[2];
-      s_pca[4 * rr + 3] = -1.0f * t;
-    }
-    s_pca[12] = s_pca[13] = s_pca[14] = 0.f;
-    s_pca[15] = 1.f;
-    for (int k = 0; k < 16; ++k) r->pca[k] = s_pca[k];
-    float mn = s_mm[0], mx = s_mm[16];
-    for (int w2 = 1; w2 < kHistThreads / ILCC_WAVE; ++w2) {
-      mn = fminf(mn, s_mm[w2]);
-      mx = fmaxf(mx, s_mm[16 + w2]);
-    }
-    s_mm[32] = mn;
-    s_mm[33] = mx;
-  }
-  const int HL = c.p.hist_bins;
-  for (int b = (int)tid; b <= HL; b += kHistThreads) s_hist[b] = 0;
-  __syncthreads();
-
-  float4* __restrict__ Q = c.pca + beg;
-  const double mn = (double)s_mm[32], mx = (double)s_mm[33];
-  const bool flat = !(mx > mn);
-  const double factor = flat ? 0.0 : HL / (mx - mn);
-  for (uint32_t i = tid; i < M; i += kHistThreads) {
-    const float4 q = P[i];
-    float o[3];
-#pragma unroll
-    for (int rr = 0; rr < 3; ++rr) {
-      float s = s_pca[4 * rr] * q.x;
-      s = s + s_pca[4 * rr + 1] * q.y;
-      s = s + s_pca[4 * rr + 2] * q.z;
-      s = s + s_pca[4 * rr + 3];
-      o[rr] = s;
-    }
-    Q[i] = make_float4(o[0], o[1], o[2], q.w);
-    if (!flat) {
-      const double sample = (double)q.w - mn;
-      int bin = (int)round(sample * factor);
-      bin = bin < 0 ? 0 : (bin > HL ? HL : bin);
-      atomicAdd(&s_hist[bin], 1);
-    }
-  }
-  __syncthreads();
-
-  __shared__ unsigned long long s_top[2];
-  if (tid == 0) s_top[0] = s_top[1] = 0ull;
-  __syncthreads();
-  const bool hist_ok = !(flat || HL <= 0);
-  const double mean = isum / M;
-  const double bin_width = (mx - mn) / HL;
-  if (hist_ok) {
-    for (int bb = (int)tid; bb < HL; bb += kHistThreads) {
-      const int cb = s_hist[bb];
-      bool first = true;
-      for (int b2 = 0; b2 < bb; ++b2) first = first && (s_hist[b2] != cb);
-      if (!first) continue;
-      const double edge = bin_width * (double)bb + mn;
-      const int side = edge > mean ? 1 : (edge < mean ? 0 : -1);
-      if (side >= 0) atomicMax(&s_top[side], ((unsigned long long)(uint32_t)(cb + 1) << 32) | (unsigned long long)(uint32_t)bb);
-    }
-  }
-  __syncthreads();
-  if (tid == 0) {
-    int status = ILCC_OK;
-    if (!hist_ok || s_top[0] == 0ull || s_top[1] == 0ull) {
-      status = ILCC_DEGENERATE_HIST;
-    } else {
-      const double low = bin_width * (double)(uint32_t)(s_top[0] & 0xFFFFFFFFull) + mn;
-      const double high = bin_width * (double)(uint32_t)(s_top[1] & 0xFFFFFFFFull) + mn;
-      const double rate = c.p.gray_rate;
-      s_gz[0] = ((rate - 1) * low + high) / rate;
-      s_gz[1] = (low + (rate - 1) * high) / rate;
-      r->gray_zone[0] = s_gz[0];
-      r->gray_zone[1] = s_gz[1];
-    }
-    s_status = status;
-    if (status != ILCC_OK) r->status = status;
-  }
-  __syncthreads();
-  if (s_status != ILCC_OK) return;
-
-  const double gz0 = s_gz[0], gz1 = s_gz[1];
-  float2* __restrict__ YZ = c.yz + beg;
-  uint8_t* __restrict__ LB = c.lab + beg;
-  uint8_t* __restrict__ CL = c.cls + beg;
-  uint32_t running = 0, nb = 0, nw = 0;
-  for (uint32_t base = 0; base < M; base += kHistThreads) {
-    const uint32_t i = base + tid;
-    bool keep = false;
-    uint8_t l = 0;
-    float4 q = make_float4(0.f, 0.f, 0.f, 0.f);
-    if (i < M) {
-      q = Q[i];
-      if ((double)q.w < gz0) {
-        keep = true;
-        l = 0;
-      } else if ((double)q.w > gz1) {
-        keep = true;
-        l = 1;
-      }
-      CL[i] = keep ? (uint8_t)(2 * l) : (uint8_t)1;
-    }
-    uint32_t tot, totw;
-    const uint32_t rank = block_rank(keep, sc, tot);
-    (void)block_rank(keep && l == 1, sc + 20, totw);
-    if (keep) {
-      YZ[running + rank] = make_float2(q.y, q.z);
-      LB[running + rank] = l;
-    }
-    running += tot;
-    nw += totw;
-    nb += tot - totw;
-  }
-  if (tid == 0) {
-    r->n_black = (int32_t)nb;
-    r->n_white = (int32_t)nw;
-    r->n_gray = (int32_t)(M - running);
-    c.n_lab[f] = running;
-    c.walk_stride[f] = walk_stride(running);
-  }
+  if (c.res[f].status != ILCC_OK) return;
+  const float4* __restrict__ P = c.board + c.off[f];
+  uint32_t n_lab, S;
+  (void)plane_frame_hist_frame(c, f, P, (uint32_t)c.res[f].n_plane, sc, scd, s_hist, nullptr, n_lab, S);
 }
 
 void launch_plane_frame_hist(const Ctx& c, hipStream_t s) {
diff --git a/lidar_camera_calibration_amd/csrc/k5w_walk_order.h b/lidar_camera_calibration_amd/csrc/k5w_walk_order.h
--- /dev/null
+++ b/lidar_camera_calibration_amd/csrc/k5w_walk_order.h
@@ -0,0 +1,117 @@
+#pragma once
+
+#include "ilcc_internal.h"
+
+namespace ilcc {
+
+__device__ __forceinline__ float2 rotate(float2 v, float cth, float sth) {
+  return make_float2(fmaf(-sth, v.y, cth * v.x), fmaf(cth, v.y, sth * v.x));
+}
+
+constexpr int kRimMilli = 300;
+struct WalkSource {
+  const float* yz;
+  uint32_t yz_stride;
+  const uint8_t* lab;
+  uint32_t lab_stride;
+};
+__device__ __forceinline__ void walk_order_frame(const Ctx& c, const uint32_t f, const uint32_t M, const uint32_t S, const WalkSource src,
+                                                 uint8_t* s_cls, const uint32_t cls_stride, uint32_t* s_cnt) {
+  uint32_t *s_in = s_cnt, *s_rim = s_cnt + kWalkThreads / ILCC_WAVE, *s_oth = s_cnt + 2 * (kWalkThreads / ILCC_WAVE);
+  if (M == 0u || M > (uint32_t)kGridLdsPointsMax) {
+    if (threadIdx.x == 0) {
+      c.walk_mi[f] = 0u;
+      c.walk_nrim[f] = 0u;
+    }
+    return;
+  }
+  const int lane = lane_id();
+  const int wid = wave_id();
+  const uint64_t beg = c.off[f];
+  auto point = [&](uint32_t i) { return make_float2(src.yz[(size_t)i * src.yz_stride], src.yz[(size_t)i * src.yz_stride + 1]); };
+  const float Wh = 0.5f * (float)c.p.board_w, Hh = 0.5f * (float)c.p.board_h;
+  const GridTables& t = c.grid;
+  const float ay_lo = t.ay[0], ay_hi = t.ay[t.n_ty - 1], az_lo = t.az[0], az_hi = t.az[t.n_tz - 1];
+  const float ay_c = t.ay[t.c_ty], az_c = t.az[t.c_tz];
+  const float rim_thr = -(float)kRimMilli * 1e-3f;
+  const int n_th = t.n_th;
+  float cmax = 0.f, smax = 0.f;
+  for (int k = 0; k < n_th; ++k) {
+    cmax = fmaxf(cmax, fabsf(t.cth[k]));
+    smax = fmaxf(smax, fabsf(t.sth[k]));
+  }
+  const float room_i = fminf(fminf(ay_lo, ay_hi), 2.f * Wh - fmaxf(ay_lo, ay_hi)), room_j = fminf(fminf(az_lo, az_hi), 2.f * Hh - fmaxf(az_lo, az_hi));
+  uint32_t cnt_in = 0, cnt_rim = 0;
+  for (uint32_t sl = threadIdx.x; sl < M; sl += kWalkThreads) {
+    const float2 v = point((uint32_t)(((uint64_t)sl * S) % M));
+    const float bi = fmaf(fabsf(v.y), smax, fabsf(v.x) * cmax), bj = fmaf(fabsf(v.y), cmax, fabsf(v.x) * smax);
+    const bool inside_always = bi + 1e-4f < room_i && bj + 1e-4f < room_j;
+    int cl = 0;
+    if (!inside_always) {
+      const float2 p = rotate(v, t.cth[t.c_th], t.sth[t.c_th]);
+      const float uc = fabsf((p.x + ay_c) - Wh) - Wh, wc = fabsf((p.y + az_c) - Hh) - Hh;
+      cl = (fmaxf(uc, wc) > rim_thr) ? 2 : 1;
+    }
+    s_cls[(size_t)sl * cls_stride] = (uint8_t)cl;
+    cnt_in += cl == 0;
+    cnt_rim += cl == 2;
+  }
+  cnt_in = wave_sum(cnt_in);
+  cnt_rim = wave_sum(cnt_rim);
+  if (lane == 0) {
+    s_in[wid] = cnt_in;
+    s_rim[wid] = cnt_rim;
+  }
+  __syncthreads();
+  uint32_t Mi = 0, n_rim = 0;
+  for (int w = 0; w < kWalkThreads / ILCC_WAVE; ++w) {
+    Mi += s_in[w];
+    n_rim += s_rim[w];
+  }
+  __syncthreads();
+  if (threadIdx.x == 0) {
+    c.walk_mi[f] = Mi;
+    c.walk_nrim[f] = n_rim;
+  }
+  float2* __restrict__ wyz = c.walk_yz + beg;
+  uint8_t* __restrict__ wlab = c.walk_lab + beg;
+  uint32_t base_in = 0, base_rim = Mi, base_oth = Mi + n_rim;
+  for (uint32_t c0 = 0; c0 < M; c0 += kWalkThreads) {
+    const uint32_t sl = c0 + threadIdx.x;
+    const int cl = sl < M ? (int)s_cls[(size_t)sl * cls_stride] : -1;
+    const unsigned long long m_in = __ballot(cl == 0), m_oth = __ballot(cl == 1), m_rim = __ballot(cl == 2);
+    const unsigned long long below = (1ull << lane) - 1ull;
+    if (lane == 0) {
+      s_in[wid] = (uint32_t)__popcll(m_in);
+      s_rim[wid] = (uint32_t)__popcll(m_rim);
+      s_oth[wid] = (uint32_t)__popcll(m_oth);
+    }
+    __syncthreads();
+    uint32_t pre_in = 0, pre_rim = 0, pre_oth = 0, tot_in = 0, tot_rim = 0, tot_oth = 0;
+    for (int w = 0; w < kWalkThreads / ILCC_WAVE; ++w) {
+      const uint32_t a = s_in[w], r = s_rim[w], o = s_oth[w];
+      if (w < wid) {
+        pre_in += a;
+        pre_rim += r;
+        pre_oth += o;
+      }
+      tot_in += a;
+      tot_rim += r;
+      tot_oth += o;
+    }
+    if (cl >= 0) {
+      const uint32_t at = cl == 0   ? base_in + pre_in + (uint32_t)__popcll(m_in & below)
+                          : cl == 2 ? base_rim + pre_rim + (uint32_t)__popcll(m_rim & below)
+                                    : base_oth + pre_oth + (uint32_t)__popcll(m_oth & below);
+      const uint32_t i = (uint32_t)(((uint64_t)sl * S) % M);
+      wyz[at] = point(i);
+      wlab[at] = src.lab[(size_t)i * src.lab_stride];
+    }
+    base_in += tot_in;
+    base_rim += tot_rim;
+    base_oth += tot_oth;
+    __syncthreads();
+  }
+}
+
+}
diff --git a/lidar_camera_calibration_amd/csrc/k6_grid_cost.hip b/lidar_camera_calibration_amd/csrc/k6_grid_cost.hip
--- a/lidar_camera_calibration_amd/csrc/k6_grid_cost.hip
+++ b/lidar_camera_calibration_amd/csrc/k6_grid_cost.hip
@@ -1,4 +1,5 @@
 #include "ilcc_internal.h"
+#include "k5w_walk_order.h"
 #include <type_traits>
 #ifdef ILCC_K6_TIMING
 #include <algorithm>
@@ -131,10 +132,6 @@
   return min(max(centre - before, 0), max(n - width, 0));
 }
 
-__device__ __forceinline__ float2 rotate(float2 v, float cth, float sth) {
-  return make_float2(fmaf(-sth, v.y, cth * v.x), fmaf(cth, v.y, sth * v.x));
-}
-
 __device__ __forceinline__ uint32_t walk_sample(uint32_t M, uint32_t at_least) { return min(M, max(at_least, M >> kSeedShift)); }
 __device__ __forceinline__ void walk_prefix(uint32_t Ms, uint32_t M, uint32_t Mi_all, uint32_t n_rim_all, uint32_t& n_in, uint32_t& n_rm) {
   n_in = Mi_all;
@@ -1292,110 +1289,13 @@
   hipLaunchKernelGGL(k6_locate, dim3(c.n_frames), dim3(kLocateThreads), lds, s, c, lp);
 }
 
-constexpr int kRimMilli = 300;
-constexpr int kWalkThreads = 256;
 __global__ __launch_bounds__(kWalkThreads) void k5w_walk_order(Ctx c) {
   __shared__ uint8_t s_cls[kGridLdsPointsMax];
-  __shared__ uint32_t s_in[kWalkThreads / ILCC_WAVE], s_rim[kWalkThreads / ILCC_WAVE], s_oth[kWalkThreads / ILCC_WAVE];
+  __shared__ uint32_t s_cnt[3 * (kWalkThreads / ILCC_WAVE)];
   const uint32_t f = blockIdx.x;
   if (c.res[f].status != ILCC_OK) return;
-  const uint32_t M = c.n_lab[f];
-  if (M == 0u || M > (uint32_t)kGridLdsPointsMax) {
-    if (threadIdx.x == 0) {
-      c.walk_mi[f] = 0u;
-      c.walk_nrim[f] = 0u;
-    }
-    return;
-  }
-  const int lane = lane_id();
-  const int wid = wave_id();
   const uint64_t beg = c.off[f];
-  const float2* __restrict__ gyz = c.yz + beg;
-  const uint8_t* __restrict__ glab = c.lab + beg;
-  const uint32_t S = c.walk_stride[f];
-  const float Wh = 0.5f * (float)c.p.board_w, Hh = 0.5f * (float)c.p.board_h;
-  const GridTables& t = c.grid;
-  const float ay_lo = t.ay[0], ay_hi = t.ay[t.n_ty - 1], az_lo = t.az[0], az_hi = t.az[t.n_tz - 1];
-  const float ay_c = t.ay[t.c_ty], az_c = t.az[t.c_tz];
-  const float rim_thr = -(float)kRimMilli * 1e-3f;
-  const int n_th = t.n_th;
-  float cmax = 0.f, smax = 0.f;
-  for (int k = 0; k < n_th; ++k) {
-    cmax = fmaxf(cmax, fabsf(t.cth[k]));
-    smax = fmaxf(smax, fabsf(t.sth[k]));
-  }
-  const float room_i = fminf(fminf(ay_lo, ay_hi), 2.f * Wh - fmaxf(ay_lo, ay_hi)), room_j = fminf(fminf(az_lo, az_hi), 2.f * Hh - fmaxf(az_lo, az_hi));
-  uint32_t cnt_in = 0, cnt_rim = 0;
-  for (uint32_t sl = threadIdx.x; sl < M; sl += kWalkThreads) {
-    const float2 v = gyz[(uint32_t)(((uint64_t)sl * S) % M)];
-    const float bi = fmaf(fabsf(v.y), smax, fabsf(v.x) * cmax), bj = fmaf(fabsf(v.y), cmax, fabsf(v.x) * smax);
-    const bool inside_always = bi + 1e-4f < room_i && bj + 1e-4f < room_j;
-    int cl = 0;
-    if (!inside_always) {
-      const float2 p = rotate(v, t.cth[t.c_th], t.sth[t.c_th]);
-      const float uc = fabsf((p.x + ay_c) - Wh) - Wh, wc = fabsf((p.y + az_c) - Hh) - Hh;
-      cl = (fmaxf(uc, wc) > rim_thr) ? 2 : 1;
-    }
-    s_cls[sl] = (uint8_t)cl;
-    cnt_in += cl == 0;
-    cnt_rim += cl == 2;
-  }
-  cnt_in = wave_sum(cnt_in);
-  cnt_rim = wave_sum(cnt_rim);
-  if (lane == 0) {
-    s_in[wid] = cnt_in;
-    s_rim[wid] = cnt_rim;
-  }
-  __syncthreads();
-  uint32_t Mi = 0, n_rim = 0;
-  for (int w = 0; w < kWalkThreads / ILCC_WAVE; ++w) {
-    Mi += s_in[w];
-    n_rim += s_rim[w];
-  }
-  __syncthreads();
-  if (threadIdx.x == 0) {
-    c.walk_mi[f] = Mi;
-    c.walk_nrim[f] = n_rim;
-  }
-  float2* __restrict__ wyz = c.walk_yz + beg;
-  uint8_t* __restrict__ wlab = c.walk_lab + beg;
-  uint32_t base_in = 0, base_rim = Mi, base_oth = Mi + n_rim;
-  for (uint32_t c0 = 0; c0 < M; c0 += kWalkThreads) {
-    const uint32_t sl = c0 + threadIdx.x;
-    const int cl = sl < M ? (int)s_cls[sl] : -1;
-    const unsigned long long m_in = __ballot(cl == 0), m_oth = __ballot(cl == 1), m_rim = __ballot(cl == 2);
-    const unsigned long long below = (1ull << lane) - 1ull;
-    if (lane == 0) {
-      s_in[wid] = (uint32_t)__popcll(m_in);
-      s_rim[wid] = (uint32_t)__popcll(m_rim);
-      s_oth[wid] = (uint32_t)__popcll(m_oth);
-    }
-    __syncthreads();
-    uint32_t pre_in = 0, pre_rim = 0, pre_oth = 0, tot_in = 0, tot_rim = 0, tot_oth = 0;
-    for (int w = 0; w < kWalkThreads / ILCC_WAVE; ++w) {
-      const uint32_t a = s_in[w], r = s_rim[w], o = s_oth[w];
-      if (w < wid) {
-        pre_in += a;
-        pre_rim += r;
-        pre_oth += o;
-      }
-      tot_in += a;
-      tot_rim += r;
-      tot_oth += o;
-    }
-    if (cl >= 0) {
-      const uint32_t at = cl == 0   ? base_in + pre_in + (uint32_t)__popcll(m_in & below)
-                          : cl == 2 ? base_rim + pre_rim + (uint32_t)__popcll(m_rim & below)
-                                    : base_oth + pre_oth + (uint32_t)__popcll(m_oth & below);
-      const uint32_t i = (uint32_t)(((uint64_t)sl * S) % M);
-      wyz[at] = gyz[i];
-      wlab[at] = glab[i];
-    }
-    base_in += tot_in;
-    base_rim += tot_rim;
-    base_oth += tot_oth;
-    __syncthreads();
-  }
+  walk_order_frame(c, f, c.n_lab[f], c.walk_stride[f], WalkSource{reinterpret_cast<const float*>(c.yz + beg), 2u, c.lab + beg, 1u}, s_cls, 1u, s_cnt);
 }
 
 void launch_walk_order(const Ctx& c, hipStream_t s) {
diff --git a/lidar_camera_calibration_amd/lidar_corners_est.py b/lidar_camera_calibration_amd/lidar_corners_est.py
--- a/lidar_camera_calibration_amd/lidar_corners_est.py
+++ b/lidar_camera_calibration_amd/lidar_corners_est.py
@@ -209,6 +209,11 @@
         if st != N.OK:
             raise IlccError(st, self._err())
 
+    def debug_separate_launches(self, on: bool):
+        st = self._lib.ilcc_debug_separate_launches(self._h, 1 if on else 0)
+        if st != N.OK:
+            raise IlccError(st, self._err())
+
     def wait_compact(self, ticket) -> np.ndarray:
         t, n_frames = ticket
         width = int(self._lib.ilcc_record_floats(self._h, t))
```

After: 1.303 million (median of 6 runs). +2.0%, better.
